# METHODS-Group/ProximalGalerkin

Measured on AMD Instinct MI355X. Metric: proximal-Newton iterations/sec, 2048^2 P1 obstacle (LVPP Newton inner loop), higher is better.
Workload: dtype f64; 1 GPU; 2048x2048 right-diagonal P1 obstacle problem on [-1,1]^2, phi_set obstacle, f=0, settings B: alpha double_exponential, alpha_max 100, tol 0.0001; snes_rtol 1e-6, Newton linear solves to true relative residual 1e-10; mixed_unknowns=8396802, step=one full LVPP solve from the zero state, parallelism=single

## Files before the change

include/pgx.h:

```cpp
#ifndef PGX_H
#define PGX_H

#include <stdint.h>

#ifdef __cplusplus
extern "C" {
#endif

#define PGX_OK 0
#define PGX_EINVAL (-1)
#define PGX_EHIP (-2)
#define PGX_ENODEV (-3)
#define PGX_ENOMEM (-4)
#define PGX_ESTATE (-5)
#define PGX_ECOMM (-6)

#define PGX_SNES_CONVERGED_FNORM_ABS 2
#define PGX_SNES_CONVERGED_FNORM_RELATIVE 3
#define PGX_SNES_CONVERGED_SNORM_RELATIVE 4
#define PGX_SNES_DIVERGED_LINEAR_SOLVE (-3)
#define PGX_SNES_DIVERGED_FNORM_NAN (-4)
#define PGX_SNES_DIVERGED_MAX_IT (-5)
#define PGX_SNES_DIVERGED_DTOL (-9)

typedef struct pgx_handle pgx_handle;

typedef struct {
  int32_t n_vertices;
  int32_t n_cells;
  const double* coords;
  const int32_t* cells;
  int32_t structured_nx;
  int32_t structured_ny;
  const int32_t* cell_dofs;
  int32_t n_dofs;
} pgx_mesh;

typedef struct {
  int32_t degree;
  int32_t nq;
  const double* qpts;
  const double* qwts;
  const double* phi_q;
  double f;
  int32_t n_bc;
  const int32_t* bc_dofs;
  const double* bc_vals;
} pgx_problem;

typedef struct {
  double snes_rtol;
  double snes_atol;
  double snes_stol;
  double snes_divtol;
  int32_t snes_max_it;
  double ksp_rtol;
  int32_t ksp_max_it;
  int32_t ksp_restart;
  int32_t mg_nu;
  double mg_omega;
  int32_t monitor;
  int32_t pc_type;
  int32_t linesearch;
} pgx_snes_opts;

void pgx_default_opts(pgx_snes_opts* o);

int pgx_create(const pgx_mesh* mesh, const pgx_problem* prob, int device, pgx_handle** out);
int pgx_create_curved(const pgx_mesh* mesh, const pgx_problem* prob, const double* geoq, int device, pgx_handle** out);
void pgx_destroy(pgx_handle* h);
const char* pgx_last_error(const pgx_handle* h);

int pgx_num_dofs(const pgx_handle* h, int64_t* ndofs);
int pgx_set_state(pgx_handle* h, const double* x);
int pgx_get_state(pgx_handle* h, double* x);
int pgx_set_prev(pgx_handle* h, const double* xk);
int pgx_get_prev(pgx_handle* h, double* xk);
int pgx_advance_prev(pgx_handle* h);
int pgx_zero_state(pgx_handle* h);
int pgx_set_alpha(pgx_handle* h, double alpha);

int pgx_residual(pgx_handle* h, const double* x, double* F, double* fnorm);
int pgx_jacobian_fill(pgx_handle* h, const double* x);

int pgx_csr_export(pgx_handle* h, int64_t* nrows, int64_t* nnz, int32_t* rowptr, int32_t* col,
                   double* K, double* M, double* D);

int pgx_spmv(pgx_handle* h, const double* x, double* y);
int pgx_spmv_bench(pgx_handle* h, int reps, double* avg_ms, double* algorithmic_bytes);
int pgx_spmv_bench_cold(pgx_handle* h, int reps, double* avg_ms, double* algorithmic_bytes);
int pgx_comm_counts(pgx_handle* h, int64_t out[4], int reset);
int pgx_spmv_select(pgx_handle* h, int kind, int* active);
int pgx_p2_stencil_info(pgx_handle* h, int32_t out[5]);
int pgx_smoother_bench(pgx_handle* h, int reps, double* avg_ms, double* algorithmic_bytes);

int pgx_tuning_set(const char* key, const char* value);
int pgx_vcycle_bench(pgx_handle* h, int level, int reps, double* avg_ms, int* n_level);

int pgx_mg_level_export(pgx_handle* h, int level, int32_t* nx, int32_t* ny, double* Dh4, float* Dq4, uint8_t* mask, int32_t* f32,
                        int32_t* dbf16);
int pgx_vcycle_apply(pgx_handle* h, int level, int nu, double omega, int in_form, int out_form, double scale, const double* b,
                     double* z);

int pgx_newton_solve(pgx_handle* h, const pgx_snes_opts* opts, int* reason, int* its, int* lin_its);
int pgx_observables(pgx_handle* h, double out[6]);

int pgx_profile_enable(pgx_handle* h, int on);
int pgx_profile_get(pgx_handle* h, double ms[8], int reset);

typedef struct pgx_comm pgx_comm;

typedef struct pgx_partition {
  int32_t rank, size;
  int32_t global_ny;
  int32_t dist_levels;
} pgx_partition;

int pgx_partition_rows(pgx_partition* part, int32_t* row0, int32_t* nrows, int32_t* own0, int32_t* nown);

int pgx_comm_rccl_unique_id(char id[128]);
int pgx_comm_rccl_init(const char id[128], int rank, int size, int device, pgx_comm** out);
int pgx_comm_local_group(int size, pgx_comm** out );
int pgx_comm_shm_init(const char* name, int rank, int size, uint64_t slot_bytes, int host_mode, pgx_comm** out);
int pgx_comm_allreduce(pgx_comm* c, double* buf, uint64_t n);
int pgx_comm_halo(pgx_comm* c, double* f0, double* f1, uint64_t send_lo, uint64_t n_send_lo, uint64_t recv_lo, uint64_t n_recv_lo,
                  uint64_t send_hi, uint64_t n_send_hi, uint64_t recv_hi, uint64_t n_recv_hi);
int pgx_comm_gather0(pgx_comm* c, const double* send, uint64_t n, double* recv0);
int pgx_comm_scatter0(pgx_comm* c, const double* send0, uint64_t n, double* recv);
int pgx_comm_selfcheck(pgx_comm* c, int host, double timeout_s);
void pgx_comm_free(pgx_comm* c);
const char* pgx_comm_last_error(void);

int pgx_create_sharded(const pgx_mesh* local_mesh, const pgx_problem* local_prob, const pgx_partition* part,
                       pgx_comm* comm, int device, pgx_handle** out);
int pgx_create_lu_dist(const pgx_mesh* mesh, const pgx_problem* prob, pgx_comm* comm, int device, pgx_handle** out);
int pgx_owned_range(const pgx_handle* h, int64_t* offset, int64_t* count);
int pgx_owned_edge_range(const pgx_handle* h, int64_t* offset, int64_t* count);
int pgx_sync_ghosts(pgx_handle* h);

#ifdef __cplusplus
}
#endif
#endif
```

proximalgalerkin_amd/_lib.py:

```python
from __future__ import annotations

import ctypes as C
import pathlib

import numpy as np

_HERE = pathlib.Path(__file__).resolve().parent
import os as _os

LIB_PATH = pathlib.Path(_os.environ.get("PGX_LIB", _HERE / "libpgx.so"))

c_double_p = C.POINTER(C.c_double)
c_int32_p = C.POINTER(C.c_int32)
c_int64_p = C.POINTER(C.c_int64)


class PgxError(RuntimeError):
    pass


class pgx_mesh(C.Structure):
    _fields_ = [
        ("n_vertices", C.c_int32),
        ("n_cells", C.c_int32),
# ... 264 lines not shown


class pgx_ma_problem(C.Structure):
    _fields_ = [
        ("nv", C.c_int32), ("nc", C.c_int32),
        ("coords", C.POINTER(C.c_double)),
        ("cells", C.POINTER(C.c_int32)),
        ("degree", C.c_int32),
        ("nu", C.c_int32), ("np", C.c_int32),
        ("cell_dofs_u", C.POINTER(C.c_int32)),
        ("cell_dofs_p", C.POINTER(C.c_int32)),
        ("nq", C.c_int32),
        ("qwts", C.POINTER(C.c_double)),
        ("tab_u", C.POINTER(C.c_double)),
        ("dtab_u", C.POINTER(C.c_double)),
        ("tab_p", C.POINTER(C.c_double)),
        ("dtab_p", C.POINTER(C.c_double)),
        ("ln_rho", C.POINTER(C.c_double)),
        ("n_bc", C.c_int32),
        ("bc_dofs", C.POINTER(C.c_int32)),
        ("g", C.POINTER(C.c_double)),
    ]


class pgx_ek_problem(C.Structure):
    _fields_ = [
        ("nc", C.c_int32),
        ("geo_order", C.c_int32),
        ("cell_nodes", c_double_p),
        ("n1", C.c_int32), ("n2", C.c_int32),
        ("cell_dofs_u", c_int32_p),
        ("cell_dofs_p", c_int32_p),
        ("nq", C.c_int32),
        ("qpts", c_double_p),
        ("qwts", c_double_p),
        ("f", C.c_double), ("phi", C.c_double),
    ]


class pgx_partition(C.Structure):
    _fields_ = [
        ("rank", C.c_int32),
        ("size", C.c_int32),
        ("global_ny", C.c_int32),
        ("dist_levels", C.c_int32),
    ]


_H = C.c_void_p
_COMM = C.c_void_p
SYMBOLS = [
    ("pgx_default_opts", None, [C.POINTER(pgx_snes_opts)]),
    ("pgx_create", C.c_int, [C.POINTER(pgx_mesh), C.POINTER(pgx_problem), C.c_int, C.POINTER(_H)]),
    ("pgx_create_curved", C.c_int, [C.POINTER(pgx_mesh), C.POINTER(pgx_problem), c_double_p, C.c_int, C.POINTER(_H)]),
    ("pgx_destroy", None, [_H]),
    ("pgx_last_error", C.c_char_p, [_H]),
    ("pgx_num_dofs", C.c_int, [_H, C.POINTER(C.c_int64)]),
    ("pgx_set_state", C.c_int, [_H, c_double_p]),
    ("pgx_get_state", C.c_int, [_H, c_double_p]),
    ("pgx_set_prev", C.c_int, [_H, c_double_p]),
    ("pgx_get_prev", C.c_int, [_H, c_double_p]),
    ("pgx_advance_prev", C.c_int, [_H]),
    ("pgx_zero_state", C.c_int, [_H]),
    ("pgx_set_alpha", C.c_int, [_H, C.c_double]),
    ("pgx_residual", C.c_int, [_H, c_double_p, c_double_p, c_double_p]),
    ("pgx_jacobian_fill", C.c_int, [_H, c_double_p]),
    ("pgx_csr_export", C.c_int,
     [_H, C.POINTER(C.c_int64), C.POINTER(C.c_int64), c_int32_p, c_int32_p, c_double_p, c_double_p, c_double_p]),
    ("pgx_spmv", C.c_int, [_H, c_double_p, c_double_p]),
    ("pgx_spmv_bench", C.c_int, [_H, C.c_int, c_double_p, c_double_p]),
    ("pgx_spmv_bench_cold", C.c_int, [_H, C.c_int, c_double_p, c_double_p]),
    ("pgx_tuning_set", C.c_int, [C.c_char_p, C.c_char_p]),
    ("pgx_smoother_bench", C.c_int, [_H, C.c_int, c_double_p, c_double_p]),
    ("pgx_vcycle_bench", C.c_int, [_H, C.c_int, C.c_int, c_double_p, C.POINTER(C.c_int)]),
    ("pgx_mg_level_export", C.c_int,
     [_H, C.c_int, c_int32_p, c_int32_p, c_double_p, C.POINTER(C.c_float), C.POINTER(C.c_uint8), c_int32_p, c_int32_p]),
    ("pgx_vcycle_apply", C.c_int, [_H, C.c_int, C.c_int, C.c_double, C.c_int, C.c_int, C.c_double, c_double_p, c_double_p]),
    ("pgx_spmv_select", C.c_int, [_H, C.c_int, C.POINTER(C.c_int)]),
    ("pgx_p2_stencil_info", C.c_int, [_H, C.POINTER(C.c_int32)]),
    ("pgx_comm_counts", C.c_int, [_H, C.POINTER(C.c_int64), C.c_int]),
    ("pgx_newton_solve", C.c_int,
     [_H, C.POINTER(pgx_snes_opts), C.POINTER(C.c_int), C.POINTER(C.c_int), C.POINTER(C.c_int)]),
    ("pgx_observables", C.c_int, [_H, c_double_p]),
    ("pgx_profile_enable", C.c_int, [_H, C.c_int]),
    ("pgx_profile_get", C.c_int, [_H, c_double_p, C.c_int]),
    ("pgx_partition_rows", C.c_int,
     [C.POINTER(pgx_partition), c_int32_p, c_int32_p, c_int32_p, c_int32_p]),
    ("pgx_comm_rccl_unique_id", C.c_int, [C.c_char_p]),
    ("pgx_comm_rccl_init", C.c_int, [C.c_char_p, C.c_int, C.c_int, C.c_int, C.POINTER(_COMM)]),
    ("pgx_comm_local_group", C.c_int, [C.c_int, C.POINTER(_COMM)]),
    ("pgx_comm_shm_init", C.c_int, [C.c_char_p, C.c_int, C.c_int, C.c_uint64, C.c_int, C.POINTER(_COMM)]),
    ("pgx_comm_allreduce", C.c_int, [_COMM, c_double_p, C.c_uint64]),
    ("pgx_comm_halo", C.c_int, [_COMM, c_double_p, c_double_p] + [C.c_uint64] * 8),
    ("pgx_comm_gather0", C.c_int, [_COMM, c_double_p, C.c_uint64, c_double_p]),
    ("pgx_comm_scatter0", C.c_int, [_COMM, c_double_p, C.c_uint64, c_double_p]),
    ("pgx_comm_selfcheck", C.c_int, [_COMM, C.c_int, C.c_double]),
    ("pgx_comm_free", None, [_COMM]),
    ("pgx_comm_last_error", C.c_char_p, []),
    ("pgx_create_sharded", C.c_int,
     [C.POINTER(pgx_mesh), C.POINTER(pgx_problem), C.POINTER(pgx_partition), _COMM, C.c_int, C.POINTER(_H)]),
    ("pgx_create_lu_dist", C.c_int, [C.POINTER(pgx_mesh), C.POINTER(pgx_problem), _COMM, C.c_int, C.POINTER(_H)]),
    ("pgx_owned_range", C.c_int, [_H, C.POINTER(C.c_int64), C.POINTER(C.c_int64)]),
    ("pgx_owned_edge_range", C.c_int, [_H, c_int64_p, c_int64_p]),
    ("pgx_sync_ghosts", C.c_int, [_H]),
    ("pgx_nd_create", C.c_int, [C.POINTER(pgx_nd_matrix), C.c_int, C.c_void_p, C.POINTER(_H)]),
    ("pgx_nd_create_dist", C.c_int, [C.POINTER(pgx_nd_matrix), _COMM, C.c_int, C.c_void_p, C.POINTER(_H)]),
    ("pgx_nd_create_symbolic_dist", C.c_int, [C.POINTER(pgx_nd_matrix), C.c_int, C.c_int, C.POINTER(_H)]),
    ("pgx_nd_export_dist", C.c_int, [_H, c_int32_p, c_int32_p, c_int32_p, c_int32_p]),
    ("pgx_nd_destroy", None, [_H]),
    ("pgx_nd_last_error", C.c_char_p, [_H]),
    ("pgx_nd_get_stats", C.c_int, [_H, C.POINTER(pgx_nd_stats)]),
    ("pgx_nd_factor", C.c_int, [_H, c_double_p, C.c_int]),
    ("pgx_nd_solve", C.c_int, [_H, c_double_p, c_double_p, C.c_int]),
    ("pgx_nd_timing", C.c_int, [_H, C.c_int, c_double_p, c_double_p]),
    ("pgx_nd_depth_profile", C.c_int, [_H, C.c_int, c_int32_p, c_double_p, c_double_p, c_double_p, c_int32_p]),
    ("pgx_nd_set_symmetric", C.c_int, [_H, C.c_int]),
    ("pgx_nd_is_symmetric", C.c_int, [_H]),
    ("pgx_nd_sym_tile_count", C.c_int, [C.c_int, C.c_int, C.c_int]),
    ("pgx_nd_sym_tile_at", None, [C.c_int, C.c_int, C.c_int, C.c_int, C.POINTER(C.c_int), C.POINTER(C.c_int)]),
    ("pgx_nd_export_levels", C.c_int, [_H, c_int64_p, c_int64_p, c_int32_p, c_int32_p, c_int64_p, c_int32_p]),
    ("pgx_nd_export_fronts", C.c_int,
     [_H, c_int64_p, c_int32_p, c_int32_p, c_int32_p, c_int32_p, c_int64_p, c_int32_p, c_int64_p, c_int32_p]),
    ("pgx_nd_export_dest", C.c_int, [_H, c_int64_p, c_int64_p]),
    ("pgx_dn_create", C.c_int, [C.c_int64, c_int32_p, c_int32_p, C.c_int, C.c_void_p, C.POINTER(_H)]),
    ("pgx_dn_destroy", None, [_H]),
    ("pgx_dn_last_error", C.c_char_p, [_H]),
    ("pgx_dn_get_stats", C.c_int, [_H, C.POINTER(pgx_dn_stats)]),
    ("pgx_dn_factor", C.c_int, [_H, c_double_p, C.c_int]),
    ("pgx_dn_solve", C.c_int, [_H, c_double_p, c_double_p, C.c_int]),
    ("pgx_dn_export_pivots", C.c_int, [_H, c_int32_p]),
    ("pgx_dn_timing", C.c_int, [_H, C.c_int, c_double_p, c_double_p]),
    ("pgx_gc_create", C.c_int, [C.POINTER(pgx_mesh), C.POINTER(pgx_gc_problem), C.c_int, C.POINTER(_H)]),
    ("pgx_gc_create_general", C.c_int, [C.POINTER(pgx_gc_spaces), C.POINTER(pgx_gc_problem), C.c_int, C.POINTER(_H)]),
    ("pgx_gc_create_dist", C.c_int, [C.POINTER(pgx_mesh), C.POINTER(pgx_gc_problem), _COMM, C.c_int, C.POINTER(_H)]),
    ("pgx_gc_lu_stats", C.c_int, [_H, C.POINTER(pgx_nd_stats)]),
    ("pgx_gc_lu_is_symmetric", C.c_int, [_H]),
    ("pgx_gc_num_dofs", C.c_int, [_H, c_int64_p]),
    ("pgx_gc_l2_increment", C.c_int, [_H, c_double_p]),
    ("pgx_gc_eval_cells", C.c_int,
     [_H, C.POINTER(pgx_gc_points), c_double_p, c_double_p, c_double_p, C.POINTER(C.c_uint8), C.POINTER(C.c_uint8)]),
    ("pgx_sg_create", C.c_int, [C.POINTER(pgx_sg_mesh), C.POINTER(pgx_sg_problem), C.c_int, C.POINTER(_H)]),
    ("pgx_sg_create_2d", C.c_int, [C.POINTER(pgx_sg_mesh2d), C.POINTER(pgx_sg_problem2d), C.c_int, C.POINTER(_H)]),
    ("pgx_sg_create_dist", C.c_int, [C.POINTER(pgx_sg_mesh), C.POINTER(pgx_sg_problem), _COMM, C.c_int, C.POINTER(_H)]),
    ("pgx_sg_create_curved", C.c_int, [C.POINTER(pgx_sg_mesh), C.POINTER(pgx_sg_problem), C.POINTER(pgx_sg_curved), C.c_int, C.POINTER(_H)]),
    ("pgx_sg_partition_info", C.c_int, [_H, c_int64_p, c_int64_p]),
    ("pgx_sg_lu_stats", C.c_int, [_H, C.POINTER(pgx_nd_stats)]),
    ("pgx_sg_lu_is_symmetric", C.c_int, [_H]),
    ("pgx_sg_num_dofs", C.c_int, [_H, c_int64_p, c_int64_p]),
    ("pgx_sg_contact_vertices", C.c_int, [_H, c_int32_p]),
    ("pgx_sg_u_increment", C.c_int, [_H, c_double_p]),
    ("pgx_sg_penetration", C.c_int, [_H, c_double_p]),
    ("pgx_sg_violation", C.c_int, [_H, c_double_p]),
    ("pgx_sg_von_mises", C.c_int, [_H, c_double_p]),
    ("pgx_qvi_create", C.c_int, [C.POINTER(pgx_mesh), C.POINTER(pgx_qvi_problem), C.c_int, C.POINTER(_H)]),
    ("pgx_qvi_num_dofs", C.c_int, [_H, c_int64_p]),
    ("pgx_qvi_h1_increment", C.c_int, [_H, c_double_p]),
    ("pgx_qmy_create", C.c_int, [C.POINTER(pgx_mesh), C.POINTER(pgx_qmy_problem), C.c_int, C.POINTER(_H)]),
    ("pgx_qmy_destroy", None, [_H]),
    ("pgx_qmy_last_error", C.c_char_p, [_H]),
    ("pgx_qmy_num_dofs", C.c_int, [_H, c_int64_p]),
    ("pgx_qmy_set_state", C.c_int, [_H, c_double_p]),
    ("pgx_qmy_get_state", C.c_int, [_H, c_double_p]),
    ("pgx_qmy_set_prev", C.c_int, [_H, c_double_p]),
    ("pgx_qmy_get_prev", C.c_int, [_H, c_double_p]),
    ("pgx_qmy_advance_prev", C.c_int, [_H]),
    ("pgx_qmy_set_gamma", C.c_int, [_H, C.c_double]),
# ... 157 lines not shown
```

proximalgalerkin_amd/csrc/pgx_api.hip:

```cpp
#include <algorithm>
#include <atomic>
#include <chrono>
#include <thread>
#include <cmath>
#include <cstdio>
#include <cstring>
#include <deque>
#include <map>
#include <mutex>
#include <string>
#include <vector>

#include "../../include/pgx.h"
#include "../../include/pgx_nd.h"
#include "pgx_comm.h"
#include "pgx_internal.h"

static thread_local std::string g_create_error;

struct DistLevel {
  int g, glo, H, ghi;
};
struct Dist {
  bool on = false;
// ... 14 lines not shown
struct pgx_handle {
  int device = 0;
  Dist dist;
  hipStream_t st = nullptr;
  std::string err;
  int n = 0, nc = 0, nx = 0, ny = 0, nnz = 0;
  int degree = 1;
  int nd = 0;
  bool structured = false;
  QuadTab q{};
  double f = 0.0, alpha = 1.0;
  double* coords = nullptr;
  int32_t* cells = nullptr;
  uint8_t* mask = nullptr;
  double *gbc = nullptr, *bphi = nullptr;
  int32_t *rowptr = nullptr, *colm = nullptr, *v2c_ptr = nullptr, *v2c_ent = nullptr, *v2c_pos = nullptr;
  std::vector<int32_t> h_rowptr, h_col;
  size_t fill_lds = 0;
  double *Kv = nullptr, *Mv = nullptr, *Dv = nullptr;
  bool jac_valid = false;
  double* geoq = nullptr;
  float2* zf_out = nullptr;
  int z_f32 = 1;
  int f32_dbf16 = 1;
  bool dv_lean = false;
  int32_t *s_rowptr = nullptr, *s_colm = nullptr;
  double *s_K = nullptr, *s_M = nullptr, *s_D = nullptr;
  int s_nnz = 0;
  size_t s_fill_lds = 0;
  int32_t* s_blk = nullptr;
  int s_nblk = 0, spmv_bal = 1;
  uint8_t* s_code = nullptr;
  double* s_tab = nullptr;
  int s_ntab = 0, spmv_dict = 1;
  std::vector<int32_t> s_h_rowptr, s_h_col;
  QuadTab2 q2{};
  int32_t *cdofs = nullptr, *p2_v2c_ptr = nullptr, *p2_v2c_ent = nullptr, *p2_v2c_pos = nullptr;
  int32_t *v2e_ptr = nullptr, *v2e = nullptr, *edge_ends = nullptr;
  double *p2_xu = nullptr, *p2_xp = nullptr, *p2_ru = nullptr, *p2_rp = nullptr;
  double* p2_stash = nullptr;
  double *c1_bu = nullptr, *c1_bp = nullptr, *c1_xu = nullptr, *c1_xp = nullptr;
  int patch_nn = 0, p2_patch = 1, patch_nu = 2;
  int p2_fallback_its = 60, p2_fallbacks = 0;
  double patch_omega = 0.8;
  bool patch_fresh = false;
  std::vector<int32_t> patch_dof_host;
  int32_t *pdof = nullptr, *ppos = nullptr;
  void* pinv = nullptr;
  int patch_f32 = 1;
  struct P2St {
    int state = 0, enable = 1, dist_enable = 1, select = 1, i0 = 0, ni = 0, j0 = 0, nj = 0, nframe = 0, ref_rows[4] = {0, 0, 0, 0};
    P2StTab tab;
    double K[46];
    double* Dst = nullptr;
    float* Dstf = nullptr;
    int32_t* frame = nullptr;
    bool fresh = false;
  } p2st;
  float* s_Df = nullptr;
  int p2_resid_f32 = 1;
  int patch_sym = 1;
  double *p2_su = nullptr, *p2_sp = nullptr;
  double *x = nullptr, *xk = nullptr, *F = nullptr, *dx = nullptr, *xw = nullptr, *rhs = nullptr;
  int restart = 0;
  double *V = nullptr, *Z = nullptr, *w = nullptr, *d_small = nullptr, *partials = nullptr, *partials2 = nullptr;
  double* h_small = nullptr;
  double* h_small_dev = nullptr;
  unsigned long long* h_seq = nullptr;
  unsigned long long* h_seq_dev = nullptr;
  unsigned long long seq = 0;
  int lean_d = 1;
  int spmv_d4 = 1;
  int lazy_norm = 1;
  double rhs_scale = 1.0;
  const float* rhs_f32 = nullptr;
  int v_f32 = 1;
  double v_f32_gain = 1e-4;
  double v_f32_max = 1e30;
  int v_f32_min = 1000000;
  bool v_f32_off = false;
  int host_poll = 1;
  int gs_wide = 16;
  int fused_publish = 1;
  int fused_resid = 1;
  int lean_rhs = 1;
  int fused_step = 1;
  std::vector<GridLevel> lev;
  double *tmp_u = nullptr, *tmp_p = nullptr, *res_u = nullptr, *res_p = nullptr;
  double omega_now = 0.0;
  int coarse_sweeps = 4;
  int tail_start = -1;
  int xcd_remap = 2;
  int tail_verts = 1100;
  int spmv_stream = 1;
  int nu_coarse = 0;
  int fused_k3 = 1;
  int fused_legs = 1;
  int fused_min = 4000;
  int cgs_selective = 1;
  long cgs_skipped = 0, cgs_total = 0;
  double cgs_eta2 = 1e-4;
  TailArgs tail{};
  pgx_nd* lu = nullptr;
  pgx_comm* lu_comm = nullptr;
  double* Jmix = nullptr;
  bool dh_interior = false;
  int d_direct = 1;
  int rap_lds_min = 60000;
  bool d0_direct = false;
  int stag_its = 12;
  double stag_gain = 1e-4;
  int smooth_d32 = 0;
  int k6_max = 0;
  int mg_f32 = 1;
  int f32_min = 4000;
  int f32_k6_max = 4300000;
  int f32_rr_max = 300000;
  int resid_grid = 1;
  int spmv_stencil = 1;
  bool lu_active = false;
  bool check_replicas = false;
  double *obs_partials = nullptr, *d_out6 = nullptr;
  int obs_blocks = 0;
  bool prof = false;
  double ms[8] = {0, 0, 0, 0, 0, 0, 0, 0};
  hipEvent_t e0 = nullptr, e1 = nullptr;
  std::vector<void*> allocs;
};

#define HIPCHK(call)                                                                            \
  do {                                                                                          \
    hipError_t e_ = (call);                                                                     \
    if (e_ != hipSuccess) {                                                                     \
      h->err = std::string(#call) + ": " + hipGetErrorString(e_);                               \
      return PGX_EHIP;                                                                          \
    }                                                                                           \
  } while (0)

template <typename T>
static int dalloc(pgx_handle* h, T** p, size_t count) {
  void* q = nullptr;
  hipError_t e = hipMalloc(&q, std::max<size_t>(count, 1) * sizeof(T));
  if (e != hipSuccess) {
    h->err = std::string("hipMalloc: ") + hipGetErrorString(e);
    return PGX_ENOMEM;
  }
  h->allocs.push_back(q);
  *p = (T*)q;
  return PGX_OK;
}
#define DALLOC(p, count)                         \
  do {                                           \
    int rc_ = dalloc(h, &(p), (size_t)(count));  \
    if (rc_) return rc_;                         \
  } while (0)

struct PhaseTimer {
  pgx_handle* h;
  int slot;
  PhaseTimer(pgx_handle* h_, int s) : h(h_), slot(s) {
    static const char* const names[8] = {"pgx:residual", "pgx:jacobian", "pgx:mg_setup/lu_factor", "pgx:spmv", "pgx:precond",
                                         "pgx:orthogonalise", "pgx:observables", "pgx:newton_solve"};
    pgx_roctx(names[s & 7]);
    if (h->prof) hipEventRecord(h->e0, h->st);
  }
  ~PhaseTimer() {
// ... 875 lines not shown
    HIPCHK(hipMemcpy(G.mask, gm.data(), G.n, hipMemcpyHostToDevice));
  }
  rc = detect_uniform(h, G);
  if (rc) return rc;
  D.view.interior_free = G.interior_free;
  h->lev.push_back(G);
  int nx = G.nx, ny = G.ny;
  const int min_nx = mg_min_nx();
  while (nx % 2 == 0 && ny % 2 == 0 && nx > min_nx && ny > min_nx) {
    nx /= 2;
    ny /= 2;
    GridLevel L{};
    L.nx = nx;
    L.ny = ny;
    L.n = (nx + 1) * (ny + 1);
    rc = alloc_level(h, L, false);
    if (rc) return rc;
    const GridLevel& Ff = h->lev.back();
    pgxk_coarse_mask(h->st, L, L.mask, Ff);
    pgxk_rap7(h->st, Ff, Ff.K, L, L.K);
    pgxk_rap7(h->st, Ff, Ff.M, L, L.M);
    rc = detect_uniform(h, L);
    if (rc) return rc;
    h->lev.push_back(L);
  }
  setup_tail(h, ld);
  rc = setup_f32(h);
  if (rc) return rc;
  HIPCHK(hipStreamSynchronize(h->st));
  return PGX_OK;
}

static thread_local const double* g_create_geoq = nullptr;

static int create_impl(const pgx_mesh* m, const pgx_problem* p, int device, const pgx_partition* part, pgx_comm* comm,
                       pgx_handle** out) {
  if (!m || !p || !out) {
    g_create_error = "null argument";
    return PGX_EINVAL;
  }
  *out = nullptr;
  int ndev = 0;
  if (hipGetDeviceCount(&ndev) != hipSuccess || ndev <= 0) {
    g_create_error = "no HIP device visible: libpgx has no CPU fallback";
    return PGX_ENODEV;
  }
  if (device < 0 || device >= ndev) {
    g_create_error = "device index out of range";
    return PGX_EINVAL;
  }
  pgx_handle* h = new pgx_handle();
  if (const char* e = pgx_tune("PGX_XCD_REMAP")) h->xcd_remap = atoi(e) ? 2 : 0;
  if (const char* e = pgx_tune("PGX_TAIL_VERTS")) h->tail_verts = atoi(e);
  if (const char* e = pgx_tune("PGX_P2_PATCH")) h->p2_patch = atoi(e);
  if (const char* e = pgx_tune("PGX_P2_PATCH_NU")) h->patch_nu = std::max(1, atoi(e));
  if (const char* e = pgx_tune("PGX_P2_PATCH_OMEGA")) h->patch_omega = atof(e);
  if (const char* e = pgx_tune("PGX_P2_PATCH_F32")) h->patch_f32 = atoi(e);
  if (const char* e = pgx_tune("PGX_P2_PATCH_SYM")) h->patch_sym = atoi(e);
  if (const char* e = pgx_tune("PGX_P2_RESID_F32")) h->p2_resid_f32 = atoi(e);
  if (const char* e = pgx_tune("PGX_P2_STENCIL")) h->p2st.enable = atoi(e);
  if (const char* e = pgx_tune("PGX_P2_STENCIL_DIST")) h->p2st.dist_enable = atoi(e);
  if (!h->patch_f32) h->patch_sym = 0;
  if (h->patch_f32 == 2 && !h->patch_sym) h->patch_f32 = 1;
  if (const char* e = pgx_tune("PGX_P2_FALLBACK_ITS")) h->p2_fallback_its = std::max(1, atoi(e));
  {
    const char* e = pgx_tune("PGX_TAIL2");
    pgxk_mg_tail_select(e ? atoi(e) : 1);
  }
  if (const char* e = pgx_tune("PGX_FUSED_LEGS")) h->fused_legs = atoi(e);
  if (const char* e = pgx_tune("PGX_FUSED_K3")) h->fused_k3 = atoi(e);
  if (const char* e = pgx_tune("PGX_NU_COARSE")) h->nu_coarse = atoi(e);
  if (const char* e = pgx_tune("PGX_SPMV_STREAM")) h->spmv_stream = atoi(e);
  if (const char* e = pgx_tune("PGX_SPMV_BAL")) h->spmv_bal = atoi(e);
  if (const char* e = pgx_tune("PGX_SPMV_DICT")) h->spmv_dict = atoi(e);
  if (const char* e = pgx_tune("PGX_SPMV_STENCIL")) h->spmv_stencil = atoi(e);
  if (const char* e = pgx_tune("PGX_RESID_GRID")) h->resid_grid = atoi(e);
  if (const char* e = pgx_tune("PGX_D_DIRECT")) h->d_direct = atoi(e);
  if (const char* e = pgx_tune("PGX_RAP_LDS_MIN")) h->rap_lds_min = atoi(e);
  if (const char* e = pgx_tune("PGX_K6_MAX")) h->k6_max = atoi(e);
  if (const char* e = pgx_tune("PGX_SMOOTH_D32")) h->smooth_d32 = atoi(e);
  if (const char* e = pgx_tune("PGX_HOST_POLL")) h->host_poll = atoi(e);
  if (const char* e = pgx_tune("PGX_GS_WIDE")) h->gs_wide = atoi(e) >= 16 ? 16 : 8;
  if (const char* e = pgx_tune("PGX_FUSED_PUBLISH")) h->fused_publish = atoi(e);
  if (const char* e = pgx_tune("PGX_FUSED_RESID")) h->fused_resid = atoi(e);
  if (const char* e = pgx_tune("PGX_LEAN_RHS")) h->lean_rhs = atoi(e);
  if (const char* e = pgx_tune("PGX_FUSED_STEP")) h->fused_step = atoi(e);
  if (const char* e = pgx_tune("PGX_LAZY_NORM")) h->lazy_norm = atoi(e);
  if (const char* e = pgx_tune("PGX_V_F32")) h->v_f32 = atoi(e);
  if (const char* e = pgx_tune("PGX_V_F32_GAIN")) h->v_f32_gain = atof(e);
  if (const char* e = pgx_tune("PGX_V_F32_MAX")) h->v_f32_max = atof(e);
  if (const char* e = pgx_tune("PGX_V_F32_MIN")) h->v_f32_min = atoi(e);
  if (const char* e = pgx_tune("PGX_Z_F32")) h->z_f32 = atoi(e);
  if (const char* e = pgx_tune("PGX_F32_DBF16")) h->f32_dbf16 = atoi(e);
  if (const char* e = pgx_tune("PGX_SPMV_D4")) h->spmv_d4 = atoi(e);
  if (const char* e = pgx_tune("PGX_LEAN_D")) h->lean_d = atoi(e);
  if (const char* e = pgx_tune("PGX_MG_F32")) h->mg_f32 = atoi(e);
  if (const char* e = pgx_tune("PGX_F32_MIN")) h->f32_min = atoi(e);
  if (const char* e = pgx_tune("PGX_F32_RR_MAX")) h->f32_rr_max = atoi(e);
  if (const char* e = pgx_tune("PGX_F32_K6_MAX")) h->f32_k6_max = atoi(e);
  if (const char* e = pgx_tune("PGX_STAG_ITS")) h->stag_its = std::max(2, atoi(e));
  if (const char* e = pgx_tune("PGX_STAG_GAIN")) h->stag_gain = atof(e);
  if (const char* e = pgx_tune("PGX_FUSED_MIN")) h->fused_min = atoi(e);
  if (const char* e = pgx_tune("PGX_CGS_SELECTIVE")) h->cgs_selective = atoi(e);
  if (const char* e = pgx_tune("PGX_CGS_ETA2")) h->cgs_eta2 = atof(e);
  if (const char* e = pgx_tune("PGX_COARSE_SWEEPS")) h->coarse_sweeps = atoi(e);
  auto fail = [&](int rc) {
    g_create_error = h->err;
    pgx_destroy(h);
    return rc;
  };
  h->device = device;
  if (p->degree != 1 && p->degree != 2) {
    h->err = "only Lagrange degree 1 and 2 are implemented";
    return fail(PGX_EINVAL);
  }
  h->degree = p->degree;
  if (p->degree == 2 && (!m->cell_dofs || m->n_dofs <= m->n_vertices)) {
    h->err = "degree 2 needs pgx_mesh.cell_dofs [n_cells][6] and n_dofs = n_vertices + n_edges";
    return fail(PGX_EINVAL);
  }
  if (p->nq < 1 || p->nq > PGX_MAX_NQ || !p->qpts || !p->qwts || !p->phi_q || m->n_vertices < 3 || m->n_cells < 1 ||
      !m->coords || !m->cells || (p->n_bc > 0 && !p->bc_dofs)) {
    h->err = "invalid mesh/problem description";
    return fail(PGX_EINVAL);
  }
  if (hipSetDevice(device) != hipSuccess || hipStreamCreate(&h->st) != hipSuccess) {
    h->err = "hipSetDevice/hipStreamCreate failed";
    return fail(PGX_EHIP);
  }
  hipEventCreate(&h->e0);
  hipEventCreate(&h->e1);
  const int n = h->n = m->n_vertices, nc = h->nc = m->n_cells;
  const int nd = h->nd = (p->degree == 2) ? m->n_dofs : n;
  h->f = p->f;
  if (m->structured_nx > 0 && m->structured_ny > 0) {
    if ((int64_t)(m->structured_nx + 1) * (m->structured_ny + 1) != n ||
        (int64_t)2 * m->structured_nx * m->structured_ny != nc) {
      h->err = "structured_nx/ny inconsistent with n_vertices/n_cells";
      return fail(PGX_EINVAL);
    }
    h->structured = true;
    h->nx = m->structured_nx;
    h->ny = m->structured_ny;
  }
  if (part) {
    pgx_partition pt = *part;
    int32_t row0 = 0, nrows = 0, own0 = 0, nown = 0;
    if (pgx_partition_rows(&pt, &row0, &nrows, &own0, &nown)) {
      h->err = g_create_error;
      return fail(PGX_EINVAL);
    }
    if (!comm || comm->rank != pt.rank || comm->size != pt.size) {
      h->err = "pgx_create_sharded: communicator rank/size differ from the partition's";
      return fail(PGX_EINVAL);
    }
    if (!h->structured || (p->degree != 1 && p->degree != 2)) {
      h->err = "pgx_create_sharded: structured P1 / P2 meshes are sharded (strip decomposition)";
      return fail(PGX_EINVAL);
    }
    if (h->ny + 1 != nrows || h->nx % (1 << pt.dist_levels)) {
      h->err = "pgx_create_sharded: local mesh must hold exactly the vertex rows of pgx_partition_rows, and nx must be "
               "divisible by 2^dist_levels";
      return fail(PGX_EINVAL);
    }
    for (int c = 0; c < nc; ++c) {
      const int v0 = std::min(m->cells[3 * c], std::min(m->cells[3 * c + 1], m->cells[3 * c + 2]));
// ... 107 lines not shown
    }
    double* phi_q = nullptr;
    const size_t nphi = (size_t)nc * p->nq;
    if (hipMalloc((void**)&phi_q, nphi * sizeof(double)) != hipSuccess) {
      h->err = "hipMalloc(phi_q)";
      return PGX_ENOMEM;
    }
    hipError_t e = hipMemcpy(phi_q, p->phi_q, nphi * sizeof(double), hipMemcpyHostToDevice);
    double* stash = nullptr;
    if (e == hipSuccess) e = hipMalloc((void**)&stash, sizeof(double) * 8 * (size_t)nc);
    if (e == hipSuccess) {
      if (p->degree == 2)
        pgxk_bphi_p2(h->st, nc, nd, h->cdofs, h->coords, phi_q, h->q2, h->p2_v2c_ptr, h->p2_v2c_ent, stash, h->bphi, h->geoq);
      else
        pgxk_bphi(h->st, nc, n, h->cells, h->coords, phi_q, h->q, h->v2c_ptr, h->v2c_ent, stash, h->bphi, h->geoq);
      e = hipStreamSynchronize(h->st);
    }
    hipFree(phi_q);
    if (stash) hipFree(stash);
    if (e != hipSuccess) {
      h->err = std::string("b_phi assembly: ") + hipGetErrorString(e);
      return PGX_EHIP;
    }
    DALLOC(h->Kv, h->nnz);
    DALLOC(h->Mv, h->nnz);
    DALLOC(h->Dv, h->nnz);
    const double* geo1 = p->degree == 1 ? h->geoq : nullptr;
    pgxk_fill_rows(h->st, 0, n, h->fill_lds, h->rowptr, h->v2c_ptr, h->v2c_ent, h->v2c_pos, h->cells, h->coords,
                   nullptr, h->q, h->Kv, geo1);
    pgxk_fill_rows(h->st, 1, n, h->fill_lds, h->rowptr, h->v2c_ptr, h->v2c_ent, h->v2c_pos, h->cells, h->coords,
                   nullptr, h->q, h->Mv, geo1);
    if (p->degree == 2) {
      DALLOC(h->s_K, h->s_nnz);
      DALLOC(h->s_M, h->s_nnz);
      DALLOC(h->s_D, h->s_nnz);
      pgxk_fill_rows_p2(h->st, 0, nd, h->s_fill_lds, h->s_rowptr, h->p2_v2c_ptr, h->p2_v2c_ent, h->p2_v2c_pos, h->cdofs,
                        h->coords, nullptr, h->q2, h->s_K, h->geoq);
      pgxk_fill_rows_p2(h->st, 1, nd, h->s_fill_lds, h->s_rowptr, h->p2_v2c_ptr, h->p2_v2c_ent, h->p2_v2c_pos, h->cdofs,
                        h->coords, nullptr, h->q2, h->s_M, h->geoq);
      if (h->spmv_dict && h->spmv_bal && h->s_blk) {
        const int rc = build_km_dictionary(h);
        if (rc) return rc;
      }
      DALLOC(h->p2_stash, (size_t)16 * nc);
      DALLOC(h->p2_xu, nd);
      DALLOC(h->p2_xp, nd);
      DALLOC(h->p2_ru, nd);
      DALLOC(h->p2_rp, nd);
      DALLOC(h->c1_bu, n);
      DALLOC(h->c1_bp, n);
      DALLOC(h->c1_xu, n);
      DALLOC(h->c1_xp, n);
    } else {
      h->s_rowptr = h->rowptr;
      h->s_colm = h->colm;
      h->s_K = h->Kv;
      h->s_M = h->Mv;
      h->s_D = h->Dv;
      h->s_nnz = h->nnz;
      h->s_fill_lds = h->fill_lds;
    }
    const size_t n2 = 2 * (size_t)nd;
    DALLOC(h->x, n2);
    DALLOC(h->xk, n2);
    DALLOC(h->F, n2);
    DALLOC(h->dx, n2);
    DALLOC(h->xw, n2);
    DALLOC(h->rhs, n2);
    HIPCHK(hipMemsetAsync(h->x, 0, n2 * sizeof(double), h->st));
    HIPCHK(hipMemsetAsync(h->xk, 0, n2 * sizeof(double), h->st));
    h->restart = 50;
    if (p->degree == 2) {
      double budget = 24e9;
      if (const char* e = pgx_tune("PGX_P2_BASIS_GB")) budget = 1e9 * atof(e);
      const double per_vec = 2.0 * (double)n2 * sizeof(double);
      h->restart = (int)std::max(50.0, std::min(300.0, budget / per_vec));
    }
    DALLOC(h->V, (size_t)(h->restart + 1) * n2);
    DALLOC(h->Z, (size_t)h->restart * n2);
    DALLOC(h->w, n2);
    DALLOC(h->d_small, 4 * (h->restart + 2));
    DALLOC(h->partials, (size_t)PGX_RED_BLOCKS * (h->restart + 2));
    DALLOC(h->partials2, ((n2 + PGX_BLOCK - 1) / PGX_BLOCK) * (size_t)62);
    {
      const size_t nsm = 4 * (size_t)(h->restart + 2);
      HIPCHK(hipHostMalloc((void**)&h->h_small, sizeof(double) * (nsm + 2), hipHostMallocMapped | hipHostMallocCoherent));
      memset(h->h_small, 0, sizeof(double) * (nsm + 2));
      HIPCHK(hipHostGetDevicePointer((void**)&h->h_small_dev, h->h_small, 0));
      h->h_seq = reinterpret_cast<unsigned long long*>(h->h_small + nsm);
      h->h_seq_dev = reinterpret_cast<unsigned long long*>(h->h_small_dev + nsm);
    }
    DALLOC(h->tmp_u, n);
    DALLOC(h->tmp_p, n);
    DALLOC(h->res_u, n);
    DALLOC(h->res_p, n);
    h->obs_blocks = pgxk_observables_blocks(nc);
    DALLOC(h->obs_partials, (size_t)h->obs_blocks * 6);
    DALLOC(h->d_out6, 6);
    if (h->dist.on) {
      DALLOC(h->dist.sb, n2);
      DALLOC(h->dist.wc, 2 * h->dist.nk_field() + 2);
    }
    const int r = h->dist.on ? build_multigrid_dist(h) : build_multigrid(h);
    if (r) return r;
    HIPCHK(hipStreamSynchronize(h->st));
    return PGX_OK;
  };
  rc = up();
  if (rc) return fail(rc);
  *out = h;
  return PGX_OK;
}

extern "C" int pgx_create(const pgx_mesh* m, const pgx_problem* p, int device, pgx_handle** out) {
  return create_impl(m, p, device, nullptr, nullptr, out);
}
extern "C" int pgx_create_curved(const pgx_mesh* m, const pgx_problem* p, const double* geoq, int device, pgx_handle** out) {
  if (!geoq) {
    g_create_error = "pgx_create_curved: null geometry table";
    return PGX_EINVAL;
  }
  g_create_geoq = geoq;
  const int rc = create_impl(m, p, device, nullptr, nullptr, out);
  g_create_geoq = nullptr;
  return rc;
}
extern "C" int pgx_create_lu_dist(const pgx_mesh* m, const pgx_problem* p, pgx_comm* comm, int device, pgx_handle** out) {
  if (!comm) {
    g_create_error = "pgx_create_lu_dist: null communicator";
    return PGX_EINVAL;
  }
  int rc = create_impl(m, p, device, nullptr, nullptr, out);
  if (rc) return rc;
  (*out)->lu_comm = comm;
  if (const char* e = pgx_tune("PGX_CHECK_REPLICAS")) (*out)->check_replicas = atoi(e) != 0;
  return PGX_OK;
}
extern "C" int pgx_create_sharded(const pgx_mesh* m, const pgx_problem* p, const pgx_partition* part, pgx_comm* comm,
                                  int device, pgx_handle** out) {
  if (!part || !comm) {
    g_create_error = "pgx_create_sharded: null partition / communicator";
    return PGX_EINVAL;
  }
  return create_impl(m, p, device, part, comm, out);
}

extern "C" void pgx_destroy(pgx_handle* h) {
  if (!h) return;
  hipSetDevice(h->device);
  if (h->st) hipStreamSynchronize(h->st);
  if (h->cgs_selective && pgx_tune("PGX_CGS_REPORT"))
    fprintf(stderr, "pgx: selective CGS2 skipped the second projection in %ld of %ld Krylov iterations\n", h->cgs_skipped, h->cgs_total);
  if (h->lu) pgx_nd_destroy(h->lu);
  for (void* p : h->allocs) hipFree(p);
  if (h->h_small) hipHostFree(h->h_small);
  if (h->e0) hipEventDestroy(h->e0);
  if (h->e1) hipEventDestroy(h->e1);
  if (h->st) hipStreamDestroy(h->st);
  delete h;
}

#define NEED(hh)          \
  if (!(hh)) return PGX_EINVAL; \
  hipSetDevice((hh)->device)

extern "C" int pgx_num_dofs(const pgx_handle* h, int64_t* nd) {
// ... 26 lines not shown
  if (!x) return PGX_EINVAL;
  return copy_in(h, h->xk, x);
}
extern "C" int pgx_get_prev(pgx_handle* h, double* x) {
  NEED(h);
  if (!x) return PGX_EINVAL;
  return copy_out(h, x, h->xk);
}
extern "C" int pgx_advance_prev(pgx_handle* h) {
  NEED(h);
  pgxk_scale_copy(h->st, 2 * (size_t)h->nd, 1.0, h->x, h->xk);
  HIPCHK(hipStreamSynchronize(h->st));
  return PGX_OK;
}
extern "C" int pgx_zero_state(pgx_handle* h) {
  NEED(h);
  HIPCHK(hipMemsetAsync(h->x, 0, sizeof(double) * 2 * (size_t)h->nd, h->st));
  HIPCHK(hipMemsetAsync(h->xk, 0, sizeof(double) * 2 * (size_t)h->nd, h->st));
  HIPCHK(hipStreamSynchronize(h->st));
  return PGX_OK;
}
extern "C" int pgx_owned_range(const pgx_handle* h, int64_t* offset, int64_t* count) {
  if (!h) return PGX_EINVAL;
  if (offset) *offset = h->dist.on ? (int64_t)h->dist.own_off : 0;
  if (count) *count = h->dist.on ? (int64_t)h->dist.own_cnt : (int64_t)(h->degree == 2 ? h->n : h->nd);
  return PGX_OK;
}
extern "C" int pgx_owned_edge_range(const pgx_handle* h, int64_t* offset, int64_t* count) {
  if (!h) return PGX_EINVAL;
  if (offset) *offset = (int64_t)h->n + (h->dist.on ? (int64_t)h->dist.eown_off : 0);
  if (count) *count = h->dist.on ? (int64_t)h->dist.eown_cnt : (int64_t)(h->nd - h->n);
  return PGX_OK;
}
extern "C" int pgx_sync_ghosts(pgx_handle* h) {
  NEED(h);
  if (!h->dist.on) return PGX_OK;
  int rc = halo_solution(h, h->x, h->x + h->nd);
  if (!rc) rc = halo_solution(h, h->xk, h->xk + h->nd);
  if (rc) return rc;
  HIPCHK(hipStreamSynchronize(h->st));
  return PGX_OK;
}
extern "C" int pgx_set_alpha(pgx_handle* h, double a) {
  if (!h || !(a > 0.0)) return PGX_EINVAL;
  h->alpha = a;
  return PGX_OK;
}

static int replica_agree(pgx_handle* h, double* dev, size_t n) {
  if (!h->lu_comm || h->lu_comm->size == 1) return PGX_OK;
  if (h->lu_comm->rank != 0) HIPCHK(hipMemsetAsync(dev, 0, n * sizeof(double), h->st));
  const int rc = h->lu_comm->allreduce(h->st, dev, n);
  if (rc) h->err = "replica agreement: " + h->lu_comm->err;
  return rc;
}

__global__ void __launch_bounds__(64) k_publish(int n, const double* __restrict__ src, double* dst, int n2, const double* __restrict__ src2,
                                                double* dst2, unsigned long long seq, unsigned long long* seqp) {
  for (int i = threadIdx.x; i < n; i += 64) __hip_atomic_store(dst + i, src[i], __ATOMIC_RELAXED, __HIP_MEMORY_SCOPE_SYSTEM);
  for (int i = threadIdx.x; i < n2; i += 64) __hip_atomic_store(dst2 + i, src2[i], __ATOMIC_RELAXED, __HIP_MEMORY_SCOPE_SYSTEM);
  __threadfence_system();
  if (threadIdx.x == 0) __hip_atomic_store(seqp, seq, __ATOMIC_RELEASE, __HIP_MEMORY_SCOPE_SYSTEM);
}
static int wait_published(pgx_handle* h, unsigned long long seq);
static int fetch_small(pgx_handle* h, const double* dsrc, size_t n, size_t hoff = 0, const double* dsrc2 = nullptr, size_t n2 = 0,
                       size_t hoff2 = 0) {
  if (!h->host_poll) {
    HIPCHK(hipMemcpyAsync(h->h_small + hoff, dsrc, sizeof(double) * n, hipMemcpyDeviceToHost, h->st));
    if (n2) HIPCHK(hipMemcpyAsync(h->h_small + hoff2, dsrc2, sizeof(double) * n2, hipMemcpyDeviceToHost, h->st));
    HIPCHK(hipStreamSynchronize(h->st));
    return PGX_OK;
  }
  const unsigned long long seq = ++h->seq;
  hipLaunchKernelGGL(k_publish, dim3(1), dim3(64), 0, h->st, (int)n, dsrc, h->h_small_dev + hoff, (int)n2, dsrc2, h->h_small_dev + hoff2,
                     seq, h->h_seq_dev);
  return wait_published(h, seq);
}
static bool fused_readback(const pgx_handle* h) { return h->fused_publish && h->host_poll && !h->dist.on && !h->lu_comm; }
static int reduce_fetch(pgx_handle* h, int nb, const double* partials, int nrows, double* dout, size_t hoff_r, const double* dsrc1 = nullptr,
                        size_t n1 = 0, size_t hoff1 = 0) {
  const unsigned long long seq = ++h->seq;
  pgxk_reduce_publish(h->st, nb, partials, nrows, dout, h->h_small_dev + hoff_r, (int)n1, dsrc1, h->h_small_dev + hoff1, seq, h->h_seq_dev);
  return wait_published(h, seq);
}
static int wait_published(pgx_handle* h, unsigned long long seq) {
  static const double limit_s = [] {
    const char* t = getenv("PGX_COMM_TIMEOUT");
    return t ? std::max(1.0, atof(t)) : 120.0;
  }();
  std::chrono::steady_clock::time_point t0;
  bool timed = false;
  for (unsigned long spins = 1;; ++spins) {
    if (__atomic_load_n(h->h_seq, __ATOMIC_ACQUIRE) == seq) return PGX_OK;
    __builtin_ia32_pause();
    if (spins > 0x2000 && (spins & 0xff) == 0) std::this_thread::yield();
    if ((spins & 0x3fff) == 0) {
      if (!timed) {
        t0 = std::chrono::steady_clock::now();
        timed = true;
      } else if (std::chrono::duration<double>(std::chrono::steady_clock::now() - t0).count() > limit_s) {
        h->err = "fetch_small: the device did not publish within PGX_COMM_TIMEOUT (" + std::to_string((int)limit_s) +
                 " s): a kernel or a collective ahead of it on the stream does not complete" + (h->dist.on || h->lu_comm ? " (a peer rank is missing?)" : "");
        return (h->dist.on || h->lu_comm) ? PGX_ECOMM : PGX_EHIP;
      }
      const hipError_t e = hipStreamQuery(h->st);
      if (e == hipSuccess) {
        if (__atomic_load_n(h->h_seq, __ATOMIC_ACQUIRE) == seq) return PGX_OK;
        h->err = "fetch_small: the stream drained without publishing (launch failure)";
        return PGX_EHIP;
      }
      if (e != hipErrorNotReady) {
        h->err = std::string("fetch_small: ") + hipGetErrorString(e);
        return PGX_EHIP;
      }
    }
  }
}

static int dev_norm(pgx_handle* h, const double* v, double* out, size_t len = 0) {
  if (fused_readback(h)) {
    const size_t l = len ? len : 2 * (size_t)h->nd;
    pgxk_multidot(h->st, l, 1, v, 0, v, h->partials, nullptr);
    const int rc = reduce_fetch(h, pgxk_multidot_blocks(l), h->partials, 1, h->d_small, 0);
    if (rc) return rc;
    *out = std::sqrt(h->h_small[0]);
    return PGX_OK;
  }
  pgxk_multidot(h->st, len ? len : 2 * (size_t)h->nd, 1, v, 0, v, h->partials, h->d_small);
  if (h->dist.on) {
    const int rc = allreduce_dev(h, h->d_small, 1);
    if (rc) return rc;
  }
  {
    const int rc = replica_agree(h, h->d_small, 1);
    if (rc) return rc;
  }
  {
    const int rc = fetch_small(h, h->d_small, 1);
    if (rc) return rc;
  }
  *out = std::sqrt(h->h_small[0]);
  return PGX_OK;
}

static bool d_direct_on(const pgx_handle* h) {
  return h->d_direct && !h->dist.on && h->degree == 1 && h->structured && h->resid_grid && !h->lev.empty() && h->lev[0].uniform &&
         sizeof(dsten_t) == 8 && !h->lev[0].Dh32;
}

static void residual_dev(pgx_handle* h, const double* x, double* F, int with_d = 0) {
  PhaseTimer t(h, 0);
  if (h->degree == 2) {
    pgxk_residual_p2_cells(h->st, h->nc, h->nd, h->cdofs, h->coords, h->mask, h->gbc, x, h->xk, h->alpha, h->f, h->q2,
                           h->p2_v2c_ptr, h->p2_v2c_ent, h->p2_stash, F, h->geoq);
    pgxk_residual_final(h->st, h->nd, h->mask, h->gbc, h->bphi, x, F);
    return;
  }
  if (h->resid_grid && h->structured && !h->lev.empty() && h->lev[0].uniform) {
    pgxk_resid_fill_grid(h->st, with_d ? 1 : 0, h->lev[0], h->fill_lds, h->rowptr, h->v2c_ptr, h->v2c_ent, h->v2c_pos, h->cells,
                         h->coords, h->mask, h->gbc, h->bphi, x, h->xk, h->alpha, h->f, h->q, F, h->Dv, with_d, d_direct_on(h), h->colm);
    h->dh_interior = with_d != 0;
    h->d0_direct = with_d != 0 && d_direct_on(h);
    if (with_d == 2) h->dv_lean = true;
    if (with_d == 1) h->dv_lean = false;
    return;
  }
  pgxk_resid_fill_p1(h->st, with_d, h->n, h->fill_lds, h->rowptr, h->v2c_ptr, h->v2c_ent, h->v2c_pos, h->cells,
                     h->coords, h->mask, h->gbc, h->bphi, x, h->xk, h->alpha, h->f, h->q, F, h->Dv, h->geoq);
}

static int jacobian_dev(pgx_handle* h, const double* x, bool have_d = false) {
  if (!(have_d && h->degree == 1)) {
    PhaseTimer t(h, 1);
    if (h->degree == 2) {
      pgxk_fill_rows_p2(h->st, 2, h->nd, h->s_fill_lds, h->s_rowptr, h->p2_v2c_ptr, h->p2_v2c_ent, h->p2_v2c_pos,
                        h->cdofs, h->coords, x + h->nd, h->q2, h->s_D, h->geoq);
      pgxk_fill_rows_p1_Dp2(h->st, h->n, h->fill_lds, h->rowptr, h->v2c_ptr, h->v2c_ent, h->v2c_pos, h->cdofs, h->coords,
                            x + h->nd, h->q2, h->Dv, h->geoq);
    } else if (h->resid_grid && h->structured && !h->lev.empty() && h->lev[0].uniform) {
      pgxk_resid_fill_grid(h->st, 1, h->lev[0], h->fill_lds, h->rowptr, h->v2c_ptr, h->v2c_ent, h->v2c_pos, h->cells, h->coords,
                           h->mask, h->gbc, h->bphi, x, h->xk, h->alpha, h->f, h->q, h->w, h->Dv, 1, d_direct_on(h), h->colm);
      h->dh_interior = true;
      h->d0_direct = d_direct_on(h);
      h->dv_lean = false;
      have_d = true;
    } else {
      pgxk_fill_rows(h->st, 2, h->n, h->fill_lds, h->rowptr, h->v2c_ptr, h->v2c_ent, h->v2c_pos, h->cells, h->coords,
                     x + h->n, h->q, h->Dv, h->geoq);
    }
  }
  if (h->structured) {
    PhaseTimer t(h, 2);
    const bool direct = d_direct_on(h);
    const bool d0 = direct && have_d && h->dh_interior && h->d0_direct;
    if (!d0)
      pgxk_csr_to_stencil_h(h->st, h->n, h->nx + 1, h->rowptr, h->colm, h->Dv, h->lev[0].Dh,
                            (have_d && h->degree == 1 && h->dh_interior) ? h->lev[0].ny : 0);
    h->dh_interior = false;
    h->d0_direct = false;
    if (h->lev[0].Dh32) pgxk_to_float(h->st, (size_t)4 * h->n, h->lev[0].Dh, h->lev[0].Dh32);
    if (h->lev[0].f32 && !d0) pgxk_f_pack_d(h->st, h->lev[0]);
    if (h->lev[0].Dd4 && !d0) pgxk_pack_d4(h->st, h->lev[0]);
    const int ld = h->dist.on ? h->dist.ldist : 0;
    for (size_t l = 1; l < h->lev.size(); ++l) {
      if (h->dist.on && (int)l == ld) {
        const Dist& D = h->dist;
// ... 764 lines not shown
  const bool vf32_ok = h->v_f32 && lean && lazy && zf32 && h->nd >= h->v_f32_min;
  float* const Vf = reinterpret_cast<float*>(h->V);
  const size_t ldvf = (nk + 3) & ~(size_t)3;
  while (true) {
    double beta;
    const bool vf32 = vf32_ok && !h->v_f32_off;
    if (first_cycle && its >= o->ksp_max_it) break;
    if (first_cycle) {
      beta = bnorm;
      if (vf32)
        pgxk_scale_copy_f32(h->st, nk, bsign * (1.0 / beta), b, Vf);
      else
        pgxk_scale_copy(h->st, nk, bsign * (1.0 / beta), b, h->V);
    } else {
      PhaseTimer t(h, 3);
      if (lean && h->fused_resid) {
        pgxk_st_spmv(h->st, h->lev[0], h->alpha, x, x + h->nd, h->xcd_remap ? 1 : 0, h->w, h->w + h->nd, nullptr, b, b + h->nd, bsign);
      } else {
        spmv_dev(h, x, h->w);
        if (dist) gather_owned(h, h->w, wk);
        pgxk_scale_copy(h->st, nk, -1.0, wk, wk);
        pgxk_axpy(h->st, nk, bsign, b, wk);
      }
      rc = dev_norm(h, wk, &beta, nk);
      if (rc) return rc;
      res = beta;
      if (o->monitor > 1) printf("      ksp true residual after cycle: %.6e (rel %.3e)\n", beta, beta / bnorm);
      if (!redo && beta <= target) break;
      if (!redo && beta > 0.1 * prev_cycle_res && beta <= 1e-7 * bnorm) break;
      if (its >= o->ksp_max_it) break;
      prev_cycle_res = beta;
      if (vf32)
        pgxk_scale_copy_f32(h->st, nk, 1.0 / beta, wk, Vf);
      else
        pgxk_scale_copy(h->st, nk, 1.0 / beta, wk, h->V);
    }
    const bool was_first = first_cycle;
    first_cycle = false;
    redo = false;
    bool abandoned = false;
    double hn_bad = 0.0;
    const double cycle_target = vf32 ? std::max(target, h->v_f32_gain * beta) : target;
    std::fill(g.begin(), g.end(), 0.0);
    g[0] = beta;
    float2* const Zf = reinterpret_cast<float2*>(h->Z);
    PgxDotScale sc2;
    std::vector<double> sv((size_t)m + 2, 1.0);
    for (int i = 0; i < PGX_DOT_SCALE_MAX; ++i) sc2.s[i] = 1.0;
    int j = 0;
    for (; j < m && its < o->ksp_max_it; ++j) {
      double* vj = h->V + (size_t)j * nk;
      double* zj = h->Z + (size_t)j * n2;
      {
        PhaseTimer t(h, 4);
        h->rhs_scale = lazy ? sv[j] : 1.0;
        h->zf_out = zf32 ? Zf + (size_t)j * h->nd : nullptr;
        h->rhs_f32 = vf32 ? Vf + (size_t)j * ldvf : nullptr;
        rc = precond(h, vj, zj, o->mg_nu, omega);
        h->rhs_f32 = nullptr;
        h->zf_out = nullptr;
        h->rhs_scale = 1.0;
        if (rc) return rc;
      }
      {
        PhaseTimer t(h, 3);
        if (dist) {
          spmv_dev(h, zj, h->w);
          gather_owned(h, h->w, h->V + (size_t)(j + 1) * nk);
        } else if (zf32) {
          double* const wn = vf32 ? h->w : h->V + (size_t)(j + 1) * n2;
          pgxk_st_spmv(h->st, h->lev[0], h->alpha, nullptr, nullptr, h->xcd_remap ? 1 : 0, wn, wn + h->nd, Zf + (size_t)j * h->nd);
        } else {
          spmv_dev(h, zj, h->V + (size_t)(j + 1) * n2);
        }
      }
      double* wj = h->V + (size_t)(j + 1) * nk;
      float* const vnext = Vf + (size_t)(j + 1) * ldvf;
      double hn = 0.0;
      {
        PhaseTimer t(h, 5);
        double* d_h1 = h->d_small;
        double* d_h2 = h->d_small + (m + 2);
        const PgxDotScale* const dsc = lazy ? &sc2 : nullptr;
        if (vf32)
          pgxk_multidot_f32(h->st, nk, j + 1, Vf, ldvf, h->w, nullptr, h->partials, d_h1, dsc, h->gs_wide);
        else
          pgxk_multidot(h->st, nk, j + 1, h->V, nk, wj, h->partials, d_h1, dsc, h->gs_wide);
        if (dist && (rc = allreduce_dev(h, d_h1, j + 1))) return rc;
        double wp2, h1h1 = 0.0, hh = 0.0;
        bool second;
        if (h->cgs_selective) {
          if (fused_readback(h)) {
            if (vf32)
              pgxk_multiaxpy_norm_f32(h->st, nk, j + 1, Vf, ldvf, d_h1, 0, h->w, vnext, h->partials, nullptr, h->gs_wide);
            else
              pgxk_multiaxpy_norm(h->st, nk, j + 1, h->V, nk, d_h1, wj, h->partials, nullptr, h->gs_wide);
            if ((rc = reduce_fetch(h, pgxk_stream_blocks(nk), h->partials, 1, d_h2 + j + 1, (size_t)(m + 2) + j + 1, d_h1, (size_t)(j + 1), 0)))
              return rc;
          } else {
            if (vf32)
              pgxk_multiaxpy_norm_f32(h->st, nk, j + 1, Vf, ldvf, d_h1, 0, h->w, vnext, h->partials, d_h2 + j + 1, h->gs_wide);
            else
              pgxk_multiaxpy_norm(h->st, nk, j + 1, h->V, nk, d_h1, wj, h->partials, d_h2 + j + 1, h->gs_wide);
            if (dist && (rc = allreduce_dev(h, d_h2 + j + 1, 1))) return rc;
            if ((rc = replica_agree(h, h->d_small, 2 * (size_t)(m + 2)))) return rc;
            if ((rc = fetch_small(h, d_h1, (size_t)(j + 1), 0, d_h2 + j + 1, 1, (size_t)(m + 2) + j + 1))) return rc;
          }
          for (int i = 0; i <= j; ++i) {
            h->h_small[i] /= sv[i];
            h1h1 += h->h_small[i] * h->h_small[i];
          }
          wp2 = h->h_small[(m + 2) + j + 1];
          second = wp2 < h->cgs_eta2 * (wp2 + h1h1);
          if (second) {
            if (vf32)
              pgxk_multidot_f32(h->st, nk, j + 1, Vf, ldvf, nullptr, vnext, h->partials, d_h2, dsc, h->gs_wide);
            else
              pgxk_multidot(h->st, nk, j + 1, h->V, nk, wj, h->partials, d_h2, dsc, h->gs_wide);
            if (dist && (rc = allreduce_dev(h, d_h2, j + 1))) return rc;
            if ((rc = replica_agree(h, d_h2, (size_t)(j + 1)))) return rc;
            if ((rc = fetch_small(h, d_h2, (size_t)(j + 1), (size_t)(m + 2)))) return rc;
            for (int i = 0; i <= j; ++i) h->h_small[(m + 2) + i] /= sv[i];
          }
        } else {
          if (j + 1 <= 60) {
            pgxk_axpy_dot(h->st, nk, j + 1, h->V, nk, d_h1, wj, h->partials2, d_h2);
          } else {
            pgxk_multiaxpy(h->st, nk, j + 1, h->V, nk, d_h1, wj);
            pgxk_multidot(h->st, nk, j + 2, h->V, nk, wj, h->partials, d_h2);
          }
          if (dist && (rc = allreduce_dev(h, d_h2, j + 2))) return rc;
          if ((rc = replica_agree(h, h->d_small, 2 * (size_t)(m + 2)))) return rc;
          if ((rc = fetch_small(h, h->d_small, 2 * (size_t)(m + 2)))) return rc;
          wp2 = h->h_small[(m + 2) + j + 1];
          second = true;
        }
        for (int i = 0; i <= j; ++i) {
          const double h2 = second ? h->h_small[(m + 2) + i] : 0.0;
          H[(size_t)i * m + j] = h->h_small[i] + h2;
          hh += h2 * h2;
        }
        if (second && vf32) {
          double* const d_n2 = d_h2 + j + 1;
          if (fused_readback(h)) {
            pgxk_multiaxpy_norm_f32(h->st, nk, j + 1, Vf, ldvf, d_h2, 1, h->w, vnext, h->partials, nullptr, h->gs_wide);
            if ((rc = reduce_fetch(h, pgxk_stream_blocks(nk), h->partials, 1, d_n2, (size_t)(m + 2) + j + 1))) return rc;
          } else {
            pgxk_multiaxpy_norm_f32(h->st, nk, j + 1, Vf, ldvf, d_h2, 1, h->w, vnext, h->partials, d_n2, h->gs_wide);
            if ((rc = fetch_small(h, d_n2, 1, (size_t)(m + 2) + j + 1))) return rc;
          }
          hn = std::sqrt(std::max(h->h_small[(m + 2) + j + 1], 0.0));
        } else if (second) {
          hn = std::sqrt(std::max(wp2 - hh, 0.0));
          if (hn > 0.0) {
            if (lazy)
              pgxk_multiaxpy(h->st, nk, j + 1, h->V, nk, d_h2, wj);
            else
              pgxk_multiaxpy_scale(h->st, nk, j + 1, h->V, nk, d_h2, 1.0 / hn, wj);
          }
        } else {
          hn = std::sqrt(std::max(wp2, 0.0));
          if (hn > 0.0 && !lazy) pgxk_scale_copy(h->st, nk, 1.0 / hn, wj, wj);
          ++h->cgs_skipped;
        }
        if (vf32 && (!std::isfinite(hn) || hn > h->v_f32_max)) {
          ++its;
          ++h->cgs_total;
          hn_bad = hn;
          abandoned = true;
          break;
        }
        if (lazy && hn > 0.0) {
          sv[j + 1] = 1.0 / hn;
          sc2.s[j + 1] = sv[j + 1] * sv[j + 1];
        }
        ++h->cgs_total;
      }
      H[(size_t)(j + 1) * m + j] = hn;
      for (int i = 0; i < j; ++i) {
        const double t1 = cs[i] * H[(size_t)i * m + j] + sn[i] * H[(size_t)(i + 1) * m + j];
        H[(size_t)(i + 1) * m + j] = -sn[i] * H[(size_t)i * m + j] + cs[i] * H[(size_t)(i + 1) * m + j];
        H[(size_t)i * m + j] = t1;
      }
      const double a = H[(size_t)j * m + j], bb = H[(size_t)(j + 1) * m + j];
      const double rr = std::hypot(a, bb);
      cs[j] = rr == 0.0 ? 1.0 : a / rr;
      sn[j] = rr == 0.0 ? 0.0 : bb / rr;
      H[(size_t)j * m + j] = rr;
      H[(size_t)(j + 1) * m + j] = 0.0;
      g[j + 1] = -sn[j] * g[j];
      g[j] = cs[j] * g[j];
      res = std::fabs(g[j + 1]);
      ++its;
      if (dist) ++h->dist.n_krylov;
      if (o->monitor > 1) printf("      ksp %3d  rnorm %.6e  rel %.3e\n", its, res, res / bnorm);
      if (!std::isfinite(res)) {
        if (x_unset) pgxk_set(h->st, n2, 0.0, x);
        *its_out = its;
        *relres = res / bnorm;
        return PGX_OK;
      }
      if (res <= cycle_target || hn == 0.0) {
        ++j;
        break;
      }
      if (omega > omega_safe && j + 1 == std::min(m, h->stag_its) && res > h->stag_gain * beta) {
        h->omega_now = omega = omega_safe;
        if (o->monitor > 1) printf("      ksp stagnates: smoother damping -> %.2f for the rest of this Newton solve\n", omega);
      }
    }
    if (abandoned) {
      h->v_f32_off = true;
      if (o->monitor > 1) printf("      ksp: basis vector outside the float range (norm %.3e): this cycle again, with the fp64 basis\n", hn_bad);
      res = beta;
      first_cycle = was_first;
      redo = !was_first;
      continue;
    }
    for (int i = j - 1; i >= 0; --i) {
      double s = g[i];
      for (int k = i + 1; k < j; ++k) s -= H[(size_t)i * m + k] * y[k];
      y[i] = s / H[(size_t)i * m + i];
    }
    for (int i = 0; i < j; ++i) h->h_small[i] = y[i];
    HIPCHK(hipMemcpyAsync(h->d_small, h->h_small, sizeof(double) * j, hipMemcpyHostToDevice, h->st));
    if (zf32)
      pgxk_lincomb_f2(h->st, (size_t)h->nd, j, Zf, (size_t)h->nd, h->d_small, x, x + h->nd, x_unset ? 0 : 1);
    else
      pgxk_lincomb(h->st, n2, j, h->Z, n2, h->d_small, x, x_unset ? 0 : 1);
    x_unset = false;
  }
  if (x_unset) pgxk_set(h->st, n2, 0.0, x);
  *its_out = its;
  *relres = res / bnorm;
  return PGX_OK;
}

extern "C" int pgx_residual(pgx_handle* h, const double* x, double* F, double* fnorm) {
  NEED(h);
  const double* xd = h->x;
  if (x) {
    int rc = copy_in(h, h->xw, x);
    if (rc) return rc;
    xd = h->xw;
  }
  residual_dev(h, xd, h->F);
  if (fnorm) {
    int rc;
    if (h->dist.on) {
      gather_owned(h, h->F, h->dist.wc);
      rc = dev_norm(h, h->dist.wc, fnorm, 2 * h->dist.nk_field());
    } else {
      rc = dev_norm(h, h->F, fnorm);
    }
    if (rc) return rc;
  }
  if (F) return copy_out(h, F, h->F);
  HIPCHK(hipStreamSynchronize(h->st));
  return PGX_OK;
}

extern "C" int pgx_jacobian_fill(pgx_handle* h, const double* x) {
  NEED(h);
  const double* xd = h->x;
  if (x) {
    int rc = copy_in(h, h->xw, x);
    if (rc) return rc;
    xd = h->xw;
  }
  {
    const int rc = jacobian_dev(h, xd);
    if (rc) return rc;
  }
  HIPCHK(hipStreamSynchronize(h->st));
  HIPCHK(hipGetLastError());
  return PGX_OK;
}

extern "C" int pgx_csr_export(pgx_handle* h, int64_t* nrows, int64_t* nnz, int32_t* rowptr, int32_t* col, double* K,
                              double* M, double* D) {
  NEED(h);
  const std::vector<int32_t>& hr = (h->degree == 2) ? h->s_h_rowptr : h->h_rowptr;
  const std::vector<int32_t>& hc = (h->degree == 2) ? h->s_h_col : h->h_col;
  if (nrows) *nrows = h->nd;
  if (nnz) *nnz = h->s_nnz;
  if (rowptr) memcpy(rowptr, hr.data(), sizeof(int32_t) * (h->nd + 1));
  if (col) memcpy(col, hc.data(), sizeof(int32_t) * h->s_nnz);
  if (K) HIPCHK(hipMemcpy(K, h->s_K, sizeof(double) * h->s_nnz, hipMemcpyDeviceToHost));
  if (M) HIPCHK(hipMemcpy(M, h->s_M, sizeof(double) * h->s_nnz, hipMemcpyDeviceToHost));
  if (D) {
    if (!h->jac_valid) {
      h->err = "pgx_csr_export(D) before pgx_jacobian_fill";
      return PGX_ESTATE;
    }
    HIPCHK(hipMemcpy(D, h->s_D, sizeof(double) * h->s_nnz, hipMemcpyDeviceToHost));
  }
  return PGX_OK;
}

extern "C" int pgx_spmv(pgx_handle* h, const double* x, double* y) {
  NEED(h);
  if (!x || !y) return PGX_EINVAL;
  if (!h->jac_valid) {
    h->err = "pgx_spmv before pgx_jacobian_fill";
    return PGX_ESTATE;
  }
  int rc = copy_in(h, h->V, x);
  if (rc) return rc;
  if (h->dist.on && (rc = halo_solution(h, h->V, h->V + h->nd))) return rc;
  spmv_dev(h, h->V, h->w);
  return copy_out(h, y, h->w);
}

extern "C" int pgx_smoother_bench(pgx_handle* h, int reps, double* avg_ms, double* bytes) {
  NEED(h);
  if (reps < 1 || !avg_ms) return PGX_EINVAL;
  if (!h->jac_valid || !h->structured || h->lev.size() < 2 || h->dist.on) {
    h->err = "pgx_smoother_bench needs a structured single-GPU handle with a grid hierarchy and a filled Jacobian";
    return PGX_ESTATE;
  }
  if (h->degree == 2) {
    if (!h->patch_nn || !h->p2_patch) {
      h->err = "pgx_smoother_bench (P2): no patch smoother on this handle";
      return PGX_ESTATE;
    }
    const int rcp = ensure_patches(h);
    if (rcp) return rcp;
    const int nd = h->nd, nv = h->n, NN = h->patch_nn, P = 2 * NN;
    pgxk_set(h->st, 2 * (size_t)nd, 1.0, h->rhs);
    HIPCHK(hipMemsetAsync(h->w, 0, sizeof(double) * 2 * nd, h->st));
    auto sweep = [&]() {
      pgxk_patch_sweep(h->st, nv, NN, nv, nd, h->pdof, h->edge_ends, h->pinv, h->patch_f32, h->patch_sym, h->rhs, h->rhs + nd, h->patch_omega,
                       h->w, h->w + nd, h->p2_su, h->p2_sp);
    };
    for (int k = 0; k < 3; ++k) sweep();
    HIPCHK(hipEventRecord(h->e0, h->st));
    for (int k = 0; k < reps; ++k) sweep();
    HIPCHK(hipEventRecord(h->e1, h->st));
    HIPCHK(hipEventSynchronize(h->e1));
    float msp = 0;
    HIPCHK(hipEventElapsedTime(&msp, h->e0, h->e1));
// ... 415 lines not shown
  const size_t n2 = 2 * (size_t)h->nd;
  PgxSolveScope scope(h->st, h->prof, &h->lu_active);
  struct JacStale {
    pgx_handle* h;
    ~JacStale() {
      if (h->dh_interior || h->dv_lean) h->jac_valid = false;
    }
  } jac_stale{h};
  PgxRange range("pgx:newton_solve");
  int its = 0, lin = 0, rsn = 0;
  double fnorm = 0, fnorm0 = 0, ttol = 0;
  h->omega_now = 0.0;
  h->v_f32_off = false;
  int rc = PGX_OK;
  const bool dist = h->dist.on;
  const size_t nk = dist ? 2 * h->dist.nk_field() : n2;
  auto owned_norm = [&](const double* v, double* out) -> int {
    if (!dist) return dev_norm(h, v, out);
    gather_owned(h, v, h->dist.wc);
    return dev_norm(h, h->dist.wc, out, nk);
  };
  const int with_d = (!use_lu && !mg_first && h->degree == 1 && h->structured && h->spmv_stencil == 1 && h->lean_d) ? 2 : 1;
  pgxk_scale_copy(h->st, n2, 1.0, h->x, h->xw);
  residual_dev(h, h->xw, h->F, with_d);
  if ((rc = replica_check(h, h->F, n2, "the residual"))) return rc;
  if (dist) {
    gather_owned(h, h->F, h->rhs);
    rc = dev_norm(h, h->rhs, &fnorm, nk);
  } else {
    rc = dev_norm(h, h->F, &fnorm);
  }
  if (rc) return rc;
  fnorm0 = fnorm;
  if (opts->monitor) printf("  0 SNES Function norm %.12e\n", fnorm);
  if (!std::isfinite(fnorm))
    rsn = PGX_SNES_DIVERGED_FNORM_NAN;
  else if (fnorm < opts->snes_atol)
    rsn = PGX_SNES_CONVERGED_FNORM_ABS;
  ttol = fnorm * opts->snes_rtol;
  while (rsn == 0) {
    if (its >= opts->snes_max_it) {
      rsn = PGX_SNES_DIVERGED_MAX_IT;
      break;
    }
    rc = jacobian_dev(h, h->xw, true);
    if (rc) return rc;
    if (use_lu) {
      if ((rc = lu_factor(h))) return rc;
      h->lu_active = true;
    }
    const bool lean_rhs = h->lean_rhs && !use_lu && !mg_first && krylov_lean(h);
    if (!lean_rhs) pgxk_scale_copy(h->st, nk, -1.0, dist ? h->rhs : h->F, h->rhs);
    int kits = 0;
    double relres = 0;
    if (mg_first && !use_lu) {
      pgx_snes_opts ol = optv;
      ol.ksp_max_it = std::min(optv.ksp_max_it, h->p2_fallback_its);
      rc = fgmres(h, h->rhs, h->dx, &ol, &kits, &relres, fnorm);
      if (rc) return rc;
      if (kits >= ol.ksp_max_it && !(relres <= 10.0 * optv.ksp_rtol)) {
        if (opts->monitor) printf("    KSP (patch multigrid) %d its, rel residual %.3e: sparse LU for the rest of this solve\n", kits, relres);
        lin += kits;
        if ((rc = ensure_lu(h))) return rc;
        if ((rc = lu_factor(h))) return rc;
        h->lu_active = true;
        use_lu = true;
        ++h->p2_fallbacks;
        rc = fgmres(h, h->rhs, h->dx, opts, &kits, &relres, fnorm);
        if (rc) return rc;
      }
    } else {
      rc = lean_rhs ? fgmres(h, h->F, h->dx, opts, &kits, &relres, fnorm, -1.0) : fgmres(h, h->rhs, h->dx, opts, &kits, &relres, fnorm);
      if (rc) return rc;
    }
    lin += kits;
    ++its;
    if (opts->monitor) printf("    KSP its %d  rel residual %.3e\n", kits, relres);
    if (!(relres <= std::max(opts->ksp_rtol, 1e-7)) || !std::isfinite(relres)) {
      rsn = PGX_SNES_DIVERGED_LINEAR_SOLVE;
      break;
    }
    const bool fstep = h->fused_step && fused_readback(h) && !use_lu && !mg_first && krylov_lean(h);
    int step_nb = 0;
    if (fstep)
      step_nb = pgxk_axpy_norms(h->st, n2, h->dx, h->xw, h->partials2);
    else
      pgxk_axpy(h->st, n2, 1.0, h->dx, h->xw);
    if (dist && (rc = halo_solution(h, h->xw, h->xw + h->nd))) return rc;
    residual_dev(h, h->xw, h->F, with_d);
    if ((rc = replica_check(h, h->F, n2, "the residual"))) return rc;
    if (dist) {
      gather_owned(h, h->F, h->rhs);
      rc = dev_norm(h, h->rhs, &fnorm, nk);
    } else {
      rc = dev_norm(h, h->F, &fnorm);
    }
    if (rc) return rc;
    if (opts->monitor) printf("  %d SNES Function norm %.12e\n", its, fnorm);
    if (!std::isfinite(fnorm)) {
      rsn = PGX_SNES_DIVERGED_FNORM_NAN;
    } else if (fnorm < opts->snes_atol) {
      rsn = PGX_SNES_CONVERGED_FNORM_ABS;
    } else if (fnorm <= ttol) {
      rsn = PGX_SNES_CONVERGED_FNORM_RELATIVE;
    } else {
      double snorm, xnorm;
      if (fstep) {
        if ((rc = reduce_fetch(h, step_nb, h->partials2, 2, h->d_small, 0))) return rc;
        snorm = std::sqrt(h->h_small[0]);
        xnorm = std::sqrt(h->h_small[1]);
      } else {
        rc = owned_norm(h->dx, &snorm);
        if (rc) return rc;
        rc = owned_norm(h->xw, &xnorm);
        if (rc) return rc;
      }
      if (snorm < opts->snes_stol * xnorm)
        rsn = PGX_SNES_CONVERGED_SNORM_RELATIVE;
      else if (fnorm > opts->snes_divtol * fnorm0)
        rsn = PGX_SNES_DIVERGED_DTOL;
    }
  }
  h->lu_active = false;
  if (rsn > 0) pgxk_scale_copy(h->st, n2, 1.0, h->xw, h->x);
  if (h->dh_interior || h->dv_lean) h->jac_valid = false;
  HIPCHK(hipStreamSynchronize(h->st));
  HIPCHK(hipGetLastError());
  if (h->prof) h->ms[7] += scope.stop();
  *reason = rsn;
  if (its_out) *its_out = its;
  if (lin_out) *lin_out = lin;
  return PGX_OK;
}
```

proximalgalerkin_amd/csrc/pgx_internal.h:

```cpp
#pragma once
#include <hip/hip_runtime.h>
#include <stdint.h>
#include <stddef.h>

#include "pgx_scope.h"

#ifdef PGX_DSTEN_FLOAT
typedef float dsten_t;
#else
typedef double dsten_t;
#endif

#define PGX_MAX_NQ 16
#define PGX_BLOCK 256
#ifndef PGX_TILE_X
#define PGX_TILE_X 32
#define PGX_TILE_Y 16
#endif
#ifndef PGX_ROWMAP_TY
#define PGX_ROWMAP_TY 16
#endif
#ifndef PGX_ROWMAP_BLOCK
#define PGX_ROWMAP_BLOCK 512
#endif
// ... 4 lines not shown
  double Mref[3][3];
  double mref[3];
  int nq;
};

struct GridLevel {
  int nx, ny, n;
  double *K, *M;
  dsten_t* Dh;
  float* Dh32;
  int uniform;
  int interior_free;
  double Kc[7], Mc[7];
  uint8_t* mask;
  double *xu, *xp, *xu2, *xp2;
  double *bu, *bp;
  double *ru, *rp;
  int f32;
  double4* Dd4;
  void* Dq;
  int dbf16;
  float2 *xf, *xf2, *bf;
};

struct StConst {
  double K[7], M[7];
  int uniform;
};

typedef float f_v2f __attribute__((ext_vector_type(2)));
typedef __bf16 f_v2bf __attribute__((ext_vector_type(2)));
__device__ __forceinline__ uint32_t f_pack_bf16x2(float lo, float hi) {
  const f_v2f f = {lo, hi};
  return __builtin_bit_cast(uint32_t, __builtin_convertvector(f, f_v2bf));
}
__device__ __forceinline__ void f_pack_d(float4 q, float4& out) { out = q; }
__device__ __forceinline__ void f_pack_d(float4 q, uint2& out) { out = make_uint2(f_pack_bf16x2(q.x, q.y), f_pack_bf16x2(q.z, q.w)); }
template <class DT>
__device__ __forceinline__ void f_pack_dq(dsten_t d0, dsten_t d1, dsten_t d2, dsten_t d3, DT& out) {
  const float big = 1e30f;
  f_pack_d(make_float4(fminf((float)d0, big), fminf((float)d1, big), fminf((float)d2, big), fminf((float)d3, big)), out);
}

#define PGX_TAIL_MAX 8
#define PGX_TAIL_VERTS 17000
struct TailLevel {
  int nx, ny, n;
  int interior_free;
  double ic[8];
  const double *K, *M;
  const dsten_t* Dh;
  StConst sc;
  const uint8_t* mask;
  double *xu, *xp, *xu2, *xp2, *bu, *bp, *ru, *rp;
};
struct TailArgs {
  int nlev, nu, coarse_sweeps;
  double alpha, omega;
  TailLevel L[PGX_TAIL_MAX];
};
void pgxk_mg_tail(hipStream_t st, const TailArgs& A);
void pgxk_mg_tail_select(int v);

void pgxk_bphi(hipStream_t st, int nc, int n, const int32_t* cells, const double* coords, const double* phi_q,
               QuadTab q, const int32_t* v2c_ptr, const int32_t* v2c_ent, double* stash, double* bphi,
               const double* geo = nullptr );
void pgxk_gather_ent(hipStream_t st, int n, const int32_t* ptr, const int32_t* ent, const double* stash, double* out);
void pgxk_fill_rows(hipStream_t st, int mode, int n, size_t lds_bytes, const int32_t* rowptr, const int32_t* v2c_ptr,
                    const int32_t* v2c_ent, const int32_t* v2c_pos, const int32_t* cells, const double* coords,
                    const double* psi, QuadTab q, double* out, const double* geo = nullptr);
void pgxk_bspmv(hipStream_t st, int mode, int n, const int32_t* rowptr, const int32_t* colm, const double* K,
                const double* M, const double* D, double alpha, const double* xu, const double* xp, const double* bu,
                const double* bp, double omega, int first, double* yu, double* yp);
void pgxk_observables(hipStream_t st, int nc, int n, const int32_t* cells, const double* coords, const double* x,
                      const double* xk, double alpha, double f, QuadTab q, double* partials, int nblocks, double* out6,
                      int raw = 0, const double* geo = nullptr);
int pgxk_observables_blocks(int nc);

void pgxk_axpy(hipStream_t st, size_t len, double a, const double* x, double* y);
void pgxk_scale_copy(hipStream_t st, size_t len, double a, const double* x, double* y);
void pgxk_scale_copy_f32(hipStream_t st, size_t len, double a, const double* x, float* y);
void pgxk_set(hipStream_t st, size_t len, double a, double* y);
void pgxk_to_float(hipStream_t st, size_t len, const double* x, float* y);
#define PGX_RED_BLOCKS 1024
#define PGX_DOT_SCALE_MAX 64
struct PgxDotScale {
  double s[PGX_DOT_SCALE_MAX];
};
void pgxk_multidot(hipStream_t st, size_t len, int nv, const double* V, size_t ldv, const double* w, double* partials,
                   double* out, const PgxDotScale* scale = nullptr, int wide = 8);
void pgxk_multidot_f32(hipStream_t st, size_t len, int nv, const float* V, size_t ldv, const double* w, const float* wf, double* partials,
                       double* out, const PgxDotScale* scale = nullptr, int wide = 8);
int pgxk_multidot_blocks(size_t len);
int pgxk_stream_blocks(size_t len);
void pgxk_reduce_publish(hipStream_t st, int nb, const double* partials, int nrows, double* out, double* hout, int n1, const double* src1,
                         double* dst1, unsigned long long seq, unsigned long long* seqp);
int pgxk_axpy_norms(hipStream_t st, size_t len, const double* x, double* y, double* partials);
void pgxk_multiaxpy(hipStream_t st, size_t len, int nv, const double* V, size_t ldv, const double* h, double* w);
void pgxk_lincomb(hipStream_t st, size_t len, int nv, const double* Z, size_t ldz, const double* y, double* x,
                  int accumulate);

void pgxk_csr_to_stencil(hipStream_t st, int n, int sx, const int32_t* rowptr, const int32_t* colm, const double* vals,
                         double* S);
void pgxk_csr_to_stencil_h(hipStream_t st, int n, int sx, const int32_t* rowptr, const int32_t* colm,
                           const double* vals, dsten_t* Sh, int frame_ny = 0);
void pgxk_rap7(hipStream_t st, const GridLevel& f, const double* Sf, const GridLevel& c, double* Sc);
void pgxk_rap7h(hipStream_t st, const GridLevel& f, const dsten_t* Sfh, const GridLevel& c, dsten_t* Sch, int pack = 0, int staged = 0);
void pgxk_st_apply(hipStream_t st, int mode, const GridLevel& L, double alpha, const double* xu, const double* xp,
                   const double* bu, const double* bp, double omega, int first, double* yu, double* yp);
void pgxk_restrict(hipStream_t st, const GridLevel& f, const double* ru, const double* rp, const GridLevel& c,
                   double* bu, double* bp);
void pgxk_prolong_add(hipStream_t st, const GridLevel& c, const double* cu, const double* cp, const GridLevel& f,
                      double* xu, double* xp);
void pgxk_coarse_mask(hipStream_t st, const GridLevel& c, uint8_t* mask_c, const GridLevel& f);
void pgxk_view_to_global(hipStream_t st, int ns, int n_view, int n_glob, int sx, int row0, int own0, int nown,
                         const double* in, double* out);
void pgxk_st_smooth2(hipStream_t st, int post, const GridLevel& L, double alpha, const double* xu, const double* xp,
                     const GridLevel* C, const double* cu, const double* cp, const double* bu, const double* bp,
                     double omega, int remap, double* yu, double* yp);
void pgxk_st_spmv(hipStream_t st, const GridLevel& L, double alpha, const double* xu, const double* xp, int remap, double* yu,
                  double* yp, const float2* xf = nullptr ,
                  const double* bu = nullptr, const double* bp = nullptr, double s = 1.0 );
void pgxk_lincomb_f2(hipStream_t st, size_t n, int nv, const float2* Zf, size_t ldz, const double* y, double* xu, double* xp,
                     int accumulate = 1);
void pgxk_pack_d4(hipStream_t st, const GridLevel& L);
void pgxk_st_resid_restrict(hipStream_t st, const GridLevel& L, double alpha, const double* xu, const double* xp,
                            const double* bu, const double* bp, const GridLevel& C, int remap, double* cbu,
                            double* cbp);
#ifndef PGX_BAL_CAP
#define PGX_BAL_CAP 1536
#endif
void pgxk_bspmv_bal(hipStream_t st, int n, int nblk, const int32_t* blk, const int32_t* rowptr, const int32_t* colm,
                    const double* K, const double* M, const uint8_t* code, const double* table, const double* D, double alpha,
                    const uint8_t* mask, const double* xu, const double* xp, const double* bu, const double* bp, int remap,
                    double* yu, double* yp, const float* Df = nullptr);
void pgxk_dict_assign(hipStream_t st, int64_t nnz, const double* K, const double* M, int ntab, const double* table, double tk,
                      double tm, uint8_t* code, int* fail, int cap, double* fail_v);
void pgxk_bspmv_stream(hipStream_t st, int n, size_t fill_lds_bytes, const int32_t* rowptr, const int32_t* colm,
                       const double* K, const double* M, const double* D, double alpha, const uint8_t* mask,
                       const double* xu, const double* xp, int remap, double* yu, double* yp);

struct QuadTab2 {
  double L[PGX_MAX_NQ][3];
  double N[PGX_MAX_NQ][6];
  double dN[PGX_MAX_NQ][6][2];
  double w[PGX_MAX_NQ];
  int nq;
};
void pgxk_bphi_p2(hipStream_t st, int nc, int n, const int32_t* cdofs, const double* coords, const double* phi_q,
                  QuadTab2 q, const int32_t* v2c_ptr, const int32_t* v2c_ent, double* stash, double* bphi,
                  const double* geo = nullptr );
void pgxk_residual_p2_cells(hipStream_t st, int nc, int n, const int32_t* cdofs, const double* coords,
                            const uint8_t* mask, const double* gbc, const double* x, const double* xk, double alpha,
                            double f, QuadTab2 q, const int32_t* v2c_ptr, const int32_t* v2c_ent, double* stash, double* F,
                            const double* geo = nullptr);
void pgxk_residual_final(hipStream_t st, int n, const uint8_t* mask, const double* gbc, const double* bphi,
                         const double* x, double* F);
void pgxk_fill_rows_p2(hipStream_t st, int mode, int n, size_t lds_bytes, const int32_t* rowptr,
                       const int32_t* v2c_ptr, const int32_t* v2c_ent, const int32_t* v2c_pos, const int32_t* cdofs,
                       const double* coords, const double* psi, QuadTab2 q, double* out, const double* geo = nullptr);
void pgxk_fill_rows_p1_Dp2(hipStream_t st, int nv, size_t lds_bytes, const int32_t* rowptr, const int32_t* v2c_ptr,
                           const int32_t* v2c_ent, const int32_t* v2c_pos, const int32_t* cdofs, const double* coords,
                           const double* psi, QuadTab2 q, double* out, const double* geo = nullptr);
void pgxk_p2_restrict(hipStream_t st, int nv, int n2, const int32_t* v2e_ptr, const int32_t* v2e, const uint8_t* mask1,
                      const double* ru2, const double* rp2, double* bu1, double* bp1);
void pgxk_p2_prolong_add(hipStream_t st, int nv, int n2, const int32_t* edge_ends, const double* cu, const double* cp,
                         double* xu, double* xp);
void pgxk_observables_p2_cells(hipStream_t st, int nc, int n, const int32_t* cdofs, const double* coords,
                               const double* x, const double* xk, double alpha, double f, QuadTab2 q, double* partials,
                               int nblocks, const double* geo = nullptr);
void pgxk_observables_final(hipStream_t st, int nblocks, const double* partials, double* out6);
void pgxk_observables_final_raw(hipStream_t st, int nblocks, const double* partials, double* out6);
void pgxk_patch_positions(hipStream_t st, int np, int NN, const int32_t* pdof, const int32_t* rowptr, const int32_t* colm,
                          int32_t* ppos);
void pgxk_patch_invert(hipStream_t st, int np, int NN, const int32_t* pdof, const int32_t* ppos, const double* K, const double* M,
                       const double* D, const uint8_t* mask, double alpha, void* pinv, int f32, int sym);
void pgxk_patch_sweep(hipStream_t st, int np, int NN, int nv, int nd, const int32_t* pdof, const int32_t* edge_ends,
                      const void* pinv, int f32, int sym, const double* ru, const double* rp, double omega, double* xu, double* xp,
                      double* su, double* sp);
size_t pgxk_patch_inverse_bytes(int np, int NN, int f32, int sym);
struct P2StTab {
  int delta[46];
  unsigned char isedge[46];
  int lofs[46];
  int lds;
  double aK[46], M[46];
  double kmax, mmax;
};
#define PGX_P2ST_BW 128
void pgxk_p2st_apply(hipStream_t st, const P2StTab& S, int nx, int nv, int i0, int ni, int j0, int nj, size_t G, const void* Dst, int f32,
                     const double* xu, const double* xp, const double* bu, const double* bp, double* yu, double* yp);
void pgxk_p2st_pack(hipStream_t st, int nx, int nv, int i0, int ni, int j0, int nj, size_t G, const int32_t* rowptr, const double* D,
                    void* Dst, int f32);
void pgxk_p2st_check(hipStream_t st, const P2StTab& S, int nx, int nv, int i0, int ni, int j0, int nj, double alpha_ref, double tol,
                     const int32_t* rowptr, const double* K, const double* M, int* fail);
void pgxk_p2_rows_csr(hipStream_t st, int nrows, const int32_t* rows, const int32_t* rowptr, const int32_t* colm, const double* K,
                      const double* M, const double* D, double alpha, const uint8_t* mask, const double* xu, const double* xp,
                      const double* bu, const double* bp, double* yu, double* yp);
void pgxk_resid_fill_p1(hipStream_t st, int write_d, int n, size_t lds_bytes, const int32_t* rowptr,
                        const int32_t* v2c_ptr, const int32_t* v2c_ent, const int32_t* v2c_pos, const int32_t* cells,
                        const double* coords, const uint8_t* mask, const double* gbc, const double* bphi,
                        const double* x, const double* xk, double alpha, double f, QuadTab q, double* F, double* Dout,
                        const double* geo = nullptr);
void pgxk_resid_fill_grid(hipStream_t st, int write_d, const GridLevel& L, size_t lds_bytes, const int32_t* rowptr,
                          const int32_t* v2c_ptr, const int32_t* v2c_ent, const int32_t* v2c_pos, const int32_t* cells,
                          const double* coords, const uint8_t* mask, const double* gbc, const double* bphi, const double* x,
                          const double* xk, double alpha, double f, QuadTab q, double* F, double* Dout, int write_sh,
                          int direct = 0, const int32_t* colm = nullptr);
void pgxk_axpy_dot(hipStream_t st, size_t len, int nv, const double* V, size_t ldv, const double* h1, double* w,
                   double* partials, double* out);
void pgxk_multiaxpy_scale(hipStream_t st, size_t len, int nv, const double* V, size_t ldv, const double* h,
                          double scale, double* w);
void pgxk_multiaxpy_norm(hipStream_t st, size_t len, int nv, const double* V, size_t ldv, const double* h, double* w,
                         double* partials, double* out, int wide = 8);
void pgxk_multiaxpy_norm_f32(hipStream_t st, size_t len, int nv, const float* V, size_t ldv, const double* h, int from_vnext, double* w,
                             float* vnext, double* partials, double* out, int wide = 8);
void pgxk_f_pack_d(hipStream_t st, const GridLevel& L);
void pgxk_f_smooth(hipStream_t st, int K, int first, const GridLevel& L, double alpha, const float2* xf, const double* b64u,
                   const double* b64p, const GridLevel* C, const float2* cf, const double* cdu, const double* cdp, double omega,
                   int remap, float2* yf, double* y64u, double* y64p, float2* cbf = nullptr, double* cb64u = nullptr,
                   double* cb64p = nullptr, double bscale = 1.0,
                   const float* b32u = nullptr, const float* b32p = nullptr);
void pgxk_f_resid_restrict(hipStream_t st, const GridLevel& L, double alpha, const float2* xf, const GridLevel& C, int remap,
                           float2* cbf, double* cb64u, double* cb64p);
int pgxk_st_smooth6_ok(const GridLevel& L);
void pgxk_st_smoothK(hipStream_t st, int K, int post, const GridLevel& L, double alpha, const double* xu,
                     const double* xp, const GridLevel* C, const double* cu, const double* cp, const double* bu,
                     const double* bp, double omega, int remap, double* yu, double* yp);
```

proximalgalerkin_amd/csrc/pgx_kernels.hip:

```cpp
#include "pgx_internal.h"
#include "pgx_stencil.h"
#include <algorithm>
#include <type_traits>

#define WAVE 64

static bool first_use_on_device(int slot) {
  static bool done[4][64] = {};
  int dev = 0;
  if (hipGetDevice(&dev) != hipSuccess || dev < 0 || dev >= 64) return true;
  if (done[slot][dev]) return false;
  done[slot][dev] = true;
  return true;
}

__device__ __forceinline__ double wave_sum(double v) {
#pragma unroll
  for (int o = WAVE / 2; o > 0; o >>= 1) v += __shfl_xor(v, o, WAVE);
  return v;
}

__device__ __forceinline__ double2 ldnt2(const double2* p) {
  typedef double v2d __attribute__((ext_vector_type(2)));
  const v2d v = __builtin_nontemporal_load((const v2d*)p);
// ... 1142 lines not shown
  if (tail && i == ng) {
    const double2 x0 = x[2 * i];
    *(float2*)(y + 4 * i) = make_float2((float)(x0.x * a), (float)(x0.y * a));
  }
}
void pgxk_scale_copy_f32(hipStream_t st, size_t len, double a, const double* x, float* y) {
  const size_t ng = len / 4;
  hipLaunchKernelGGL(k_scale_copy_f32, stream_grid(ng + 1), dim3(PGX_BLOCK), 0, st, ng, (int)(len - 4 * ng), a, (const double2*)x, y);
}

__global__ void __launch_bounds__(PGX_BLOCK) k_set(size_t len, double a, double* __restrict__ y) {
  for (size_t i = blockIdx.x * (size_t)blockDim.x + threadIdx.x; i < len; i += (size_t)gridDim.x * blockDim.x)
    y[i] = a;
}
void pgxk_set(hipStream_t st, size_t len, double a, double* y) {
  hipLaunchKernelGGL(k_set, stream_grid(len), dim3(PGX_BLOCK), 0, st, len, a, y);
}

__global__ void __launch_bounds__(PGX_BLOCK) k_to_float(size_t len, const double* __restrict__ x, float* __restrict__ y) {
  for (size_t i = blockIdx.x * (size_t)blockDim.x + threadIdx.x; i < len; i += (size_t)gridDim.x * blockDim.x) y[i] = (float)x[i];
}
void pgxk_to_float(hipStream_t st, size_t len, const double* x, float* y) {
  hipLaunchKernelGGL(k_to_float, stream_grid(len), dim3(PGX_BLOCK), 0, st, len, x, y);
}

template <class T>
struct GsLane;
template <>
struct GsLane<double> {
  static constexpr int G = 2;
};
template <>
struct GsLane<float> {
  static constexpr int G = 4;
};
template <int G>
__device__ __forceinline__ void gs_ld_basis(const double* p, double* a) {
  static_assert(G == 2, "fp64 basis: two elements per lane");
  const double2 v = ldnt2((const double2*)p);
  a[0] = v.x, a[1] = v.y;
}
template <int G>
__device__ __forceinline__ void gs_ld_basis(const float* p, double* a) {
  typedef float vf __attribute__((ext_vector_type(G)));
  const vf v = __builtin_nontemporal_load((const vf*)p);
#pragma unroll
  for (int k = 0; k < G; ++k) a[k] = (double)v[k];
}
template <int G>
__device__ __forceinline__ void gs_ld(const double* p, double* a) {
#pragma unroll
  for (int k = 0; k < G; k += 2) {
    const double2 v = *(const double2*)(p + k);
    a[k] = v.x, a[k + 1] = v.y;
  }
}
template <int G>
__device__ __forceinline__ void gs_ld(const float* p, double* a) {
  typedef float vf __attribute__((ext_vector_type(G)));
  const vf v = *(const vf*)p;
#pragma unroll
  for (int k = 0; k < G; ++k) a[k] = (double)v[k];
}
template <int G>
__device__ __forceinline__ void gs_st(double* p, const double* a, double* s) {
#pragma unroll
  for (int k = 0; k < G; k += 2) {
    *(double2*)(p + k) = make_double2(a[k], a[k + 1]);
    s[k] = a[k], s[k + 1] = a[k + 1];
  }
}
template <int G>
__device__ __forceinline__ void gs_st(float* p, const double* a, double* s) {
  typedef float vf __attribute__((ext_vector_type(G)));
  vf v;
#pragma unroll
  for (int k = 0; k < G; ++k) {
    v[k] = (float)a[k];
    s[k] = (double)v[k];
  }
  *(vf*)p = v;
}

template <int NV, class VT, class WT>
__global__ void __launch_bounds__(PGX_BLOCK) k_multidot(size_t ng, int tail, const VT* __restrict__ V, size_t ldv,
                                                        const WT* __restrict__ w,
                                                        double* __restrict__ partials, int pstride, int poff) {
  constexpr int G = GsLane<VT>::G;
  __shared__ double sm[PGX_BLOCK / WAVE];
  double acc[NV];
#pragma unroll
  for (int v = 0; v < NV; ++v) acc[v] = 0.0;
  size_t i = blockIdx.x * (size_t)blockDim.x + threadIdx.x;
  for (; i < ng; i += (size_t)gridDim.x * blockDim.x) {
    double wv[G];
    gs_ld<G>(w + G * i, wv);
#pragma unroll
    for (int v = 0; v < NV; ++v) {
      double a[G];
      gs_ld_basis<G>(V + v * ldv + G * i, a);
#pragma unroll
      for (int k = 0; k < G; k += 2) acc[v] += fma(a[k], wv[k], a[k + 1] * wv[k + 1]);
    }
  }
  if (G == 4 && tail && i == ng) {
    double wv[2];
    gs_ld<2>(w + G * i, wv);
#pragma unroll
    for (int v = 0; v < NV; ++v) {
      double a[2];
      gs_ld<2>(V + v * ldv + G * i, a);
      acc[v] += fma(a[0], wv[0], a[1] * wv[1]);
    }
  }
#pragma unroll
  for (int v = 0; v < NV; ++v) {
    const double r = block_sum(acc[v], sm);
    if (threadIdx.x == 0) partials[(size_t)blockIdx.x * pstride + poff + v] = r;
  }
}

__global__ void __launch_bounds__(PGX_BLOCK) k_reduce_partials(int nblocks, int nv, const double* __restrict__ p,
                                                               double* __restrict__ out) {
  __shared__ double sm[PGX_BLOCK / WAVE];
  const int v = blockIdx.x;
  double s = 0.0;
  for (int b = threadIdx.x; b < nblocks; b += blockDim.x) s += p[(size_t)b * nv + v];
  const double r = block_sum(s, sm);
  if (threadIdx.x == 0) out[v] = r;
}
__global__ void __launch_bounds__(PGX_BLOCK) k_reduce_partials_scaled(int nblocks, int nv, const double* __restrict__ p, PgxDotScale sc,
                                                                      double* __restrict__ out) {
  __shared__ double sm[PGX_BLOCK / WAVE];
  const int v = blockIdx.x;
  double s = 0.0;
  for (int b = threadIdx.x; b < nblocks; b += blockDim.x) s += p[(size_t)b * nv + v];
  const double r = block_sum(s, sm);
  if (threadIdx.x == 0) out[v] = r * sc.s[v];
}

int pgxk_multidot_blocks(size_t len) {
  size_t nb = (len / 2 + PGX_BLOCK - 1) / PGX_BLOCK;
  if (nb > PGX_RED_BLOCKS) nb = PGX_RED_BLOCKS;
  return nb == 0 ? 1 : (int)nb;
}

template <class VT, class WT>
static void multidot_t(hipStream_t st, size_t len, int nv, const VT* V, size_t ldv, const WT* w, double* partials, double* out,
                       const PgxDotScale* scale, int wide) {
  constexpr int G = GsLane<VT>::G;
  const size_t ng = len / G;
  const int tail = (int)(len - G * ng);
  const size_t nb = (size_t)pgxk_multidot_blocks(len);
  dim3 grid((unsigned)nb), block(PGX_BLOCK);
  const int cap = wide > 16 ? 16 : wide < 1 ? 1 : wide;
  int done = 0;
  while (done < nv) {
    const int rem = nv - done;
    const VT* Vp = V + (size_t)done * ldv;
#define PGX_MD(N)                                                                                                          \
  case N:                                                                                                                  \
    hipLaunchKernelGGL((k_multidot<N, VT, WT>), grid, block, 0, st, ng, tail, Vp, ldv, w, partials, nv, done);             \
    break
    const int take = rem >= cap ? cap : rem;
    switch (take) {
      PGX_MD(1);
      PGX_MD(2);
      PGX_MD(3);
      PGX_MD(4);
      PGX_MD(5);
      PGX_MD(6);
      PGX_MD(7);
      PGX_MD(8);
      PGX_MD(9);
      PGX_MD(10);
      PGX_MD(11);
      PGX_MD(12);
      PGX_MD(13);
      PGX_MD(14);
      PGX_MD(15);
      PGX_MD(16);
    }
#undef PGX_MD
    done += take;
  }
  if (!out) return;
  if (scale)
    hipLaunchKernelGGL(k_reduce_partials_scaled, dim3(nv), block, 0, st, (int)nb, nv, partials, *scale, out);
  else
    hipLaunchKernelGGL(k_reduce_partials, dim3(nv), block, 0, st, (int)nb, nv, partials, out);
}
void pgxk_multidot(hipStream_t st, size_t len, int nv, const double* V, size_t ldv, const double* w, double* partials,
                   double* out, const PgxDotScale* scale, int wide) {
  multidot_t(st, len, nv, V, ldv, w, partials, out, scale, wide);
}
void pgxk_multidot_f32(hipStream_t st, size_t len, int nv, const float* V, size_t ldv, const double* w, const float* wf,
                       double* partials, double* out, const PgxDotScale* scale, int wide) {
  if (w)
    multidot_t(st, len, nv, V, ldv, w, partials, out, scale, wide);
  else
    multidot_t(st, len, nv, V, ldv, wf, partials, out, scale, wide);
}

__global__ void __launch_bounds__(PGX_BLOCK) k_reduce_publish(int nb, const double* __restrict__ p, int nrows, double* out, double* hout,
                                                              int n1, const double* src1, double* dst1, unsigned long long seq,
                                                              unsigned long long* seqp) {
  __shared__ double sm[PGX_BLOCK / WAVE];
  for (int r = 0; r < nrows; ++r) {
    const double* row = p + (size_t)r * nb;
    double s = 0.0;
    for (int b = threadIdx.x; b < nb; b += blockDim.x) s += row[b];
    const double t = block_sum(s, sm);
    if (threadIdx.x == 0) {
      out[r] = t;
      __hip_atomic_store(hout + r, t, __ATOMIC_RELAXED, __HIP_MEMORY_SCOPE_SYSTEM);
    }
  }
  if (threadIdx.x >= WAVE) return;
  for (int i = threadIdx.x; i < n1; i += WAVE) __hip_atomic_store(dst1 + i, src1[i], __ATOMIC_RELAXED, __HIP_MEMORY_SCOPE_SYSTEM);
  __threadfence_system();
  if (threadIdx.x == 0) __hip_atomic_store(seqp, seq, __ATOMIC_RELEASE, __HIP_MEMORY_SCOPE_SYSTEM);
}
void pgxk_reduce_publish(hipStream_t st, int nb, const double* partials, int nrows, double* out, double* hout, int n1, const double* src1,
                         double* dst1, unsigned long long seq, unsigned long long* seqp) {
  hipLaunchKernelGGL(k_reduce_publish, dim3(1), dim3(PGX_BLOCK), 0, st, nb, partials, nrows, out, hout, n1, src1, dst1, seq, seqp);
}

__global__ void __launch_bounds__(PGX_BLOCK) k_axpy_norms(size_t len2, double a, const double2* __restrict__ x, double2* __restrict__ y,
                                                          double* __restrict__ partials) {
  __shared__ double sm[PGX_BLOCK / WAVE];
  double accx = 0.0, accy = 0.0;
  for (size_t i = blockIdx.x * (size_t)blockDim.x + threadIdx.x; i < len2; i += (size_t)gridDim.x * blockDim.x) {
    double2 xv = x[i], yv = y[i];
    yv.x += a * xv.x;
    yv.y += a * xv.y;
    y[i] = yv;
    accx += xv.x * xv.x + xv.y * xv.y;
    accy += yv.x * yv.x + yv.y * yv.y;
  }
  const double rx = block_sum(accx, sm);
  const double ry = block_sum(accy, sm);
  if (threadIdx.x == 0) {
    partials[blockIdx.x] = rx;
    partials[gridDim.x + blockIdx.x] = ry;
  }
}
int pgxk_axpy_norms(hipStream_t st, size_t len, const double* x, double* y, double* partials) {
  const int nb = pgxk_multidot_blocks(len);
  hipLaunchKernelGGL(k_axpy_norms, dim3(nb), dim3(PGX_BLOCK), 0, st, len / 2, 1.0, (const double2*)x, (double2*)y, partials);
  return nb;
}

template <int NV>
__global__ void __launch_bounds__(PGX_BLOCK) k_multiaxpy(size_t len2, const double2* __restrict__ V, size_t ldv2,
                                                         const double* __restrict__ h, double2* __restrict__ w) {
  double hv[NV];
#pragma unroll
  for (int v = 0; v < NV; ++v) hv[v] = h[v];
  for (size_t i = blockIdx.x * (size_t)blockDim.x + threadIdx.x; i < len2; i += (size_t)gridDim.x * blockDim.x) {
    double2 wv = w[i];
#pragma unroll
    for (int v = 0; v < NV; ++v) {
      const double2 a = V[v * ldv2 + i];
      wv.x -= hv[v] * a.x;
      wv.y -= hv[v] * a.y;
    }
    w[i] = wv;
  }
}

__global__ void __launch_bounds__(PGX_BLOCK) k_axpy_dot(size_t len, int nv, const double* __restrict__ V, size_t ldv,
                                                        const double* __restrict__ h1, double* __restrict__ w,
                                                        double* __restrict__ partials) {
  extern __shared__ double sh[];
  double* hs = sh + (size_t)(nv + 1) * PGX_BLOCK;
  const int t = threadIdx.x;
  const int lane = t & (WAVE - 1), wid = t / WAVE;
  if (t < nv) hs[t] = h1[t];
  constexpr int NW = PGX_BLOCK / WAVE;
  constexpr int MAXA = 16;
  double acc[MAXA];
#pragma unroll
  for (int k = 0; k < MAXA; ++k) acc[k] = 0.0;
  const size_t nchunks = (len + PGX_BLOCK - 1) / PGX_BLOCK;
  for (size_t chunk = blockIdx.x; chunk < nchunks; chunk += gridDim.x) {
    __syncthreads();
    const size_t i = chunk * PGX_BLOCK + t;
    const bool live = i < len;
    double wv = live ? w[i] : 0.0;
#pragma unroll 8
    for (int v = 0; v < nv; ++v) {
      const double a = live ? __builtin_nontemporal_load(V + (size_t)v * ldv + i) : 0.0;
      sh[v * PGX_BLOCK + t] = a;
      wv -= hs[v] * a;
    }
    if (live) w[i] = wv;
    sh[nv * PGX_BLOCK + t] = wv;
    __syncthreads();
    const double* wl = sh + (size_t)nv * PGX_BLOCK;
    double wr[NW];
#pragma unroll
    for (int r = 0; r < NW; ++r) wr[r] = wl[lane + WAVE * r];
#pragma unroll
    for (int k = 0; k < MAXA; ++k) {
      const int v = wid + NW * k;
      if (v <= nv) {
        const double* sv = sh + (size_t)v * PGX_BLOCK;
#pragma unroll
        for (int r = 0; r < NW; ++r) acc[k] += sv[lane + WAVE * r] * wr[r];
      }
    }
  }
#pragma unroll
  for (int k = 0; k < MAXA; ++k) {
    const int v = wid + NW * k;
    if (v <= nv) {
      const double r = wave_sum(acc[k]);
      if (lane == 0) partials[(size_t)v * gridDim.x + blockIdx.x] = r;
    }
  }
}

__global__ void __launch_bounds__(PGX_BLOCK) k_reduce_rows(int nb, const double* __restrict__ p,
                                                           double* __restrict__ out) {
  __shared__ double sm[PGX_BLOCK / WAVE];
  const double* row = p + (size_t)blockIdx.x * nb;
  double s = 0.0;
  for (int b = threadIdx.x; b < nb; b += blockDim.x) s += row[b];
  const double r = block_sum(s, sm);
  if (threadIdx.x == 0) out[blockIdx.x] = r;
}

void pgxk_axpy_dot(hipStream_t st, size_t len, int nv, const double* V, size_t ldv, const double* h1, double* w,
                   double* partials, double* out) {
  size_t nchunks = (len + PGX_BLOCK - 1) / PGX_BLOCK;
  const unsigned nb = (unsigned)std::min<size_t>(nchunks, 4096);
  const size_t lds = ((size_t)(nv + 1) * PGX_BLOCK + nv) * sizeof(double);
  if (first_use_on_device(1))
    hipFuncSetAttribute((const void*)k_axpy_dot, hipFuncAttributeMaxDynamicSharedMemorySize, 128 * 1024);
  hipLaunchKernelGGL(k_axpy_dot, dim3(nb), dim3(PGX_BLOCK), lds, st, len, nv, V, ldv, h1, w, partials);
  hipLaunchKernelGGL(k_reduce_rows, dim3(nv + 1), dim3(PGX_BLOCK), 0, st, (int)nb, partials, out);
}

template <int NV>
__global__ void __launch_bounds__(PGX_BLOCK) k_multiaxpy_scale(size_t len2, const double2* __restrict__ V, size_t ldv2,
                                                               const double* __restrict__ h, double scale, int last,
                                                               double2* __restrict__ w) {
  double hv[NV];
#pragma unroll
  for (int v = 0; v < NV; ++v) hv[v] = h[v];
  for (size_t i = blockIdx.x * (size_t)blockDim.x + threadIdx.x; i < len2; i += (size_t)gridDim.x * blockDim.x) {
    double2 wv = w[i];
#pragma unroll
    for (int v = 0; v < NV; ++v) {
      const double2 a = ldnt2(V + v * ldv2 + i);
      wv.x -= hv[v] * a.x;
      wv.y -= hv[v] * a.y;
    }
    if (last) {
      wv.x *= scale;
      wv.y *= scale;
    }
    w[i] = wv;
  }
}

void pgxk_multiaxpy_scale(hipStream_t st, size_t len, int nv, const double* V, size_t ldv, const double* h,
                          double scale, double* w) {
  const size_t len2 = len / 2, ldv2 = ldv / 2;
  dim3 grid = stream_grid(len2), block(PGX_BLOCK);
  int done = 0;
  while (done < nv) {
    const int rem = nv - done;
    const double2* Vp = (const double2*)(V + (size_t)done * ldv);
    const int step = rem >= 8 ? 8 : rem >= 4 ? 4 : rem >= 2 ? 2 : 1;
    const int last = (done + step == nv);
    if (step == 8)
      hipLaunchKernelGGL(k_multiaxpy_scale<8>, grid, block, 0, st, len2, Vp, ldv2, h + done, scale, last, (double2*)w);
    else if (step == 4)
      hipLaunchKernelGGL(k_multiaxpy_scale<4>, grid, block, 0, st, len2, Vp, ldv2, h + done, scale, last, (double2*)w);
    else if (step == 2)
      hipLaunchKernelGGL(k_multiaxpy_scale<2>, grid, block, 0, st, len2, Vp, ldv2, h + done, scale, last, (double2*)w);
    else
      hipLaunchKernelGGL(k_multiaxpy_scale<1>, grid, block, 0, st, len2, Vp, ldv2, h + done, scale, last, (double2*)w);
    done += step;
  }
}

template <int NV, bool NORM, class VT, class WT>
__global__ void __launch_bounds__(PGX_BLOCK) k_multiaxpy_norm(size_t ng, int tail, const VT* __restrict__ V, size_t ldv,
                                                              const double* __restrict__ h, const WT* __restrict__ win,
                                                              typename std::conditional<NORM && std::is_same<VT, float>::value, float, double>::type* __restrict__ wout,
                                                              double* __restrict__ partials) {
  typedef typename std::conditional<NORM && std::is_same<VT, float>::value, float, double>::type OT;
  constexpr int G = GsLane<VT>::G;
  const WT* const wi = std::is_same<WT, OT>::value ? (const WT*)wout : win;
  __shared__ double sm[PGX_BLOCK / WAVE];
  double hv[NV];
#pragma unroll
  for (int v = 0; v < NV; ++v) hv[v] = h[v];
  double acc = 0.0;
  size_t i = blockIdx.x * (size_t)blockDim.x + threadIdx.x;
  for (; i < ng; i += (size_t)gridDim.x * blockDim.x) {
    double wv[G], s[G];
    gs_ld<G>(wi + G * i, wv);
#pragma unroll
    for (int v = 0; v < NV; ++v) {
      double a[G];
      gs_ld_basis<G>(V + v * ldv + G * i, a);
#pragma unroll
      for (int k = 0; k < G; ++k) wv[k] -= hv[v] * a[k];
    }
    gs_st<G>(wout + G * i, wv, s);
    if (NORM) {
#pragma unroll
      for (int k = 0; k < G; k += 2) acc += fma(s[k + 1], s[k + 1], s[k] * s[k]);
    }
  }
  if (G == 4 && tail && i == ng) {
    double wv[2], s[2];
    gs_ld<2>(wi + G * i, wv);
#pragma unroll
    for (int v = 0; v < NV; ++v) {
      double a[2];
      gs_ld<2>(V + v * ldv + G * i, a);
      wv[0] -= hv[v] * a[0];
      wv[1] -= hv[v] * a[1];
    }
    gs_st<2>(wout + G * i, wv, s);
    if (NORM) acc += fma(s[1], s[1], s[0] * s[0]);
  }
  if (NORM) {
    const double r = block_sum(acc, sm);
    if (threadIdx.x == 0) partials[blockIdx.x] = r;
  }
}
int pgxk_stream_blocks(size_t len) { return (int)stream_grid(len / 2).x; }
template <int N, class VT>
static void launch_multiaxpy_norm(hipStream_t st, dim3 grid, size_t ng, int tail, const VT* Vp, size_t ldv, const double* h, bool last,
                                  bool inf, double* w, float* wf, double* partials) {
  const dim3 block(PGX_BLOCK);
  if constexpr (std::is_same<VT, double>::value) {
    if (last)
      hipLaunchKernelGGL((k_multiaxpy_norm<N, true, double, double>), grid, block, 0, st, ng, tail, Vp, ldv, h, (const double*)nullptr, w, partials);
    else
      hipLaunchKernelGGL((k_multiaxpy_norm<N, false, double, double>), grid, block, 0, st, ng, tail, Vp, ldv, h, (const double*)nullptr, w, partials);
  } else {
    if (last && inf)
      hipLaunchKernelGGL((k_multiaxpy_norm<N, true, float, float>), grid, block, 0, st, ng, tail, Vp, ldv, h, (const float*)nullptr, wf, partials);
    else if (last)
      hipLaunchKernelGGL((k_multiaxpy_norm<N, true, float, double>), grid, block, 0, st, ng, tail, Vp, ldv, h, (const double*)w, wf, partials);
    else if (inf)
      hipLaunchKernelGGL((k_multiaxpy_norm<N, false, float, float>), grid, block, 0, st, ng, tail, Vp, ldv, h, (const float*)wf, w, partials);
    else
      hipLaunchKernelGGL((k_multiaxpy_norm<N, false, float, double>), grid, block, 0, st, ng, tail, Vp, ldv, h, (const double*)nullptr, w, partials);
  }
}
template <class VT>
static void multiaxpy_norm_t(hipStream_t st, size_t len, int nv, const VT* V, size_t ldv, const double* h, bool inf, double* w, float* wf,
                             double* partials, double* out, int wide) {
  constexpr int G = GsLane<VT>::G;
  const size_t ng = len / G;
  const int tail = (int)(len - G * ng);
  dim3 grid = stream_grid(len / 2);
  const int cap = wide > 16 ? 16 : wide < 1 ? 1 : wide;
  int done = 0;
  while (done < nv) {
    const int step = std::min(cap, nv - done);
    const bool last = done + step == nv;
    const VT* Vp = V + (size_t)done * ldv;
#define PGX_MAN(N)                                                                                                     \
  case N:                                                                                                              \
    launch_multiaxpy_norm<N>(st, grid, ng, tail, Vp, ldv, h + done, last, inf && done == 0, w, wf, partials);          \
    break
    switch (step) {
      PGX_MAN(16);
      PGX_MAN(15);
      PGX_MAN(14);
      PGX_MAN(13);
      PGX_MAN(12);
      PGX_MAN(11);
      PGX_MAN(10);
      PGX_MAN(9);
      PGX_MAN(8);
      PGX_MAN(7);
      PGX_MAN(6);
      PGX_MAN(5);
      PGX_MAN(4);
      PGX_MAN(3);
      PGX_MAN(2);
      default: launch_multiaxpy_norm<1>(st, grid, ng, tail, Vp, ldv, h + done, last, inf && done == 0, w, wf, partials); break;
    }
#undef PGX_MAN
    done += step;
  }
  if (out) hipLaunchKernelGGL(k_reduce_rows, dim3(1), dim3(PGX_BLOCK), 0, st, (int)grid.x, partials, out);
}
void pgxk_multiaxpy_norm(hipStream_t st, size_t len, int nv, const double* V, size_t ldv, const double* h, double* w,
                         double* partials, double* out, int wide) {
  multiaxpy_norm_t(st, len, nv, V, ldv, h, false, w, nullptr, partials, out, wide);
}
void pgxk_multiaxpy_norm_f32(hipStream_t st, size_t len, int nv, const float* V, size_t ldv, const double* h, int from_vnext, double* w,
                             float* vnext, double* partials, double* out, int wide) {
  multiaxpy_norm_t(st, len, nv, V, ldv, h, from_vnext != 0, w, vnext, partials, out, wide);
}

void pgxk_multiaxpy(hipStream_t st, size_t len, int nv, const double* V, size_t ldv, const double* h, double* w) {
  const size_t len2 = len / 2, ldv2 = ldv / 2;
  dim3 grid = stream_grid(len2), block(PGX_BLOCK);
  int done = 0;
  while (done < nv) {
    const int rem = nv - done;
    const double2* Vp = (const double2*)(V + (size_t)done * ldv);
    if (rem >= 8) {
      hipLaunchKernelGGL(k_multiaxpy<8>, grid, block, 0, st, len2, Vp, ldv2, h + done, (double2*)w);
      done += 8;
    } else if (rem >= 4) {
      hipLaunchKernelGGL(k_multiaxpy<4>, grid, block, 0, st, len2, Vp, ldv2, h + done, (double2*)w);
      done += 4;
    } else if (rem >= 2) {
      hipLaunchKernelGGL(k_multiaxpy<2>, grid, block, 0, st, len2, Vp, ldv2, h + done, (double2*)w);
      done += 2;
    } else {
      hipLaunchKernelGGL(k_multiaxpy<1>, grid, block, 0, st, len2, Vp, ldv2, h + done, (double2*)w);
      done += 1;
    }
  }
}

__global__ void __launch_bounds__(PGX_BLOCK) k_lincomb(size_t len2, int nv, const double2* __restrict__ Z,
                                                       size_t ldz2, const double* __restrict__ y,
                                                       double2* __restrict__ x, int accumulate) {
  for (size_t i = blockIdx.x * (size_t)blockDim.x + threadIdx.x; i < len2; i += (size_t)gridDim.x * blockDim.x) {
    double2 s = accumulate ? x[i] : make_double2(0.0, 0.0);
    for (int v = 0; v < nv; ++v) {
      const double2 a = Z[v * ldz2 + i];
      const double yv = y[v];
      s.x += yv * a.x;
      s.y += yv * a.y;
    }
    x[i] = s;
  }
}
__global__ void __launch_bounds__(PGX_BLOCK) k_lincomb_f2(size_t n, int nv, const float2* __restrict__ Zf, size_t ldz,
                                                          const double* __restrict__ y, double* __restrict__ xu, double* __restrict__ xp,
                                                          int accumulate) {
  for (size_t i = blockIdx.x * (size_t)blockDim.x + threadIdx.x; i < n; i += (size_t)gridDim.x * blockDim.x) {
    double su = accumulate ? xu[i] : 0.0, sp = accumulate ? xp[i] : 0.0;
    for (int v = 0; v < nv; ++v) {
      const float2 a = Zf[v * ldz + i];
      const double yv = y[v];
      su += yv * (double)a.x;
      sp += yv * (double)a.y;
    }
    xu[i] = su;
    xp[i] = sp;
  }
}
void pgxk_lincomb_f2(hipStream_t st, size_t n, int nv, const float2* Zf, size_t ldz, const double* y, double* xu, double* xp,
                     int accumulate) {
  const unsigned grid = (unsigned)std::min<size_t>((n + PGX_BLOCK - 1) / PGX_BLOCK, 256 * 32);
  hipLaunchKernelGGL(k_lincomb_f2, dim3(grid), dim3(PGX_BLOCK), 0, st, n, nv, Zf, ldz, y, xu, xp, accumulate);
}

void pgxk_lincomb(hipStream_t st, size_t len, int nv, const double* Z, size_t ldz, const double* y, double* x,
                  int accumulate) {
  hipLaunchKernelGGL(k_lincomb, stream_grid(len / 2), dim3(PGX_BLOCK), 0, st, len / 2, nv, (const double2*)Z,
                     ldz / 2, y, (double2*)x, accumulate);
}

__device__ __forceinline__ constexpr double pw(int dx, int dy) {
  return (dx == 0 && dy == 0) ? 1.0
         : ((dx == 1 && dy == 0) || (dx == -1 && dy == 0) || (dx == 0 && dy == 1) || (dx == 0 && dy == -1) ||
            (dx == 1 && dy == 1) || (dx == -1 && dy == -1))
             ? 0.5
             : 0.0;
}

__global__ void __launch_bounds__(PGX_BLOCK) k_csr_to_stencil(int n, int sx, const int32_t* __restrict__ rowptr,
                                                              const int32_t* __restrict__ colm,
                                                              const double* __restrict__ vals,
                                                              double* __restrict__ S) {
  const int i = blockIdx.x * blockDim.x + threadIdx.x;
  if (i >= n) return;
  double s[7] = {0, 0, 0, 0, 0, 0, 0};
  for (int k = rowptr[i]; k < rowptr[i + 1]; ++k) {
    const int o = (colm[k] & 0x7fffffff) - i;
    const double v = vals[k];
    if (o == 0) s[0] = v;
    else if (o == 1) s[1] = v;
    else if (o == -1) s[2] = v;
    else if (o == sx) s[3] = v;
    else if (o == -sx) s[4] = v;
    else if (o == sx + 1) s[5] = v;
    else if (o == -sx - 1) s[6] = v;
  }
#pragma unroll
  for (int k = 0; k < 7; ++k) S[(size_t)k * n + i] = s[k];
}
void pgxk_csr_to_stencil(hipStream_t st, int n, int sx, const int32_t* rowptr, const int32_t* colm, const double* vals,
                         double* S) {
  hipLaunchKernelGGL(k_csr_to_stencil, dim3((n + PGX_BLOCK - 1) / PGX_BLOCK), dim3(PGX_BLOCK), 0, st, n, sx, rowptr,
                     colm, vals, S);
}

__global__ void __launch_bounds__(PGX_BLOCK) k_rap7(int nxf, int nyf, int nf, const double* __restrict__ Sf, int nxc,
                                                    int nyc, int ncv, double* __restrict__ Sc) {
  const int C = blockIdx.x * blockDim.x + threadIdx.x;
  if (C >= ncv) return;
  constexpr int OX[7] = {0, 1, -1, 0, 0, 1, -1};
  constexpr int OY[7] = {0, 0, 0, 1, -1, 1, -1};
  const int sxc = nxc + 1, sxf = nxf + 1;
  const int I = C % sxc, Jc = C / sxc;
  double out[7] = {0, 0, 0, 0, 0, 0, 0};
#pragma unroll
  for (int oa = 0; oa < 7; ++oa) {
    const int ax = 2 * I + OX[oa], ay = 2 * Jc + OY[oa];
    if (ax < 0 || ax > nxf || ay < 0 || ay > nyf) continue;
    const double wa = pw(OX[oa], OY[oa]);
    const size_t a = (size_t)ay * sxf + ax;
#pragma unroll
    for (int os = 0; os < 7; ++os) {
      const double coef = wa * Sf[(size_t)os * nf + a];
      const int dx = OX[oa] + OX[os], dy = OY[oa] + OY[os];
#pragma unroll
      for (int oc = 0; oc < 7; ++oc) {
        const double w2 = pw(dx - 2 * OX[oc], dy - 2 * OY[oc]);
        if (w2 != 0.0) out[oc] += coef * w2;
      }
    }
  }
#pragma unroll
  for (int oc = 0; oc < 7; ++oc) {
    const int nx_ = I + OX[oc], ny_ = Jc + OY[oc];
    const bool ok = nx_ >= 0 && nx_ <= nxc && ny_ >= 0 && ny_ <= nyc;
    Sc[(size_t)oc * ncv + C] = ok ? out[oc] : 0.0;
  }
}
void pgxk_rap7(hipStream_t st, const GridLevel& f, const double* Sf, const GridLevel& c, double* Sc) {
  hipLaunchKernelGGL(k_rap7, dim3((c.n + PGX_BLOCK - 1) / PGX_BLOCK), dim3(PGX_BLOCK), 0, st, f.nx, f.ny, f.n, Sf, c.nx,
                     c.ny, c.n, Sc);
}

__device__ __forceinline__ void ld7h(const dsten_t* __restrict__ Sh, int n, int sx, int v, int i, int j, int nx,
                                     int ny, double d[7]) {
  d[0] = Sh[v];
  d[1] = (i < nx) ? Sh[(size_t)n + v] : 0.0;
  d[2] = (i > 0) ? Sh[(size_t)n + v - 1] : 0.0;
  d[3] = (j < ny) ? Sh[(size_t)2 * n + v] : 0.0;
  d[4] = (j > 0) ? Sh[(size_t)2 * n + v - sx] : 0.0;
  d[5] = (i < nx && j < ny) ? Sh[(size_t)3 * n + v] : 0.0;
// ... 1992 lines not shown
```

proximalgalerkin_amd/csrc/pgx_mg32.hip:

```cpp
#include <algorithm>

#include "pgx_internal.h"
#include "pgx_stencil.h"

#define F32_BLOCK 512
#ifndef F32_LEAN
#define F32_LEAN 0
#endif
#ifndef F32_WAVES_EU
#define F32_WAVES_EU 2
#endif
#ifndef F32_K6_SPLIT
#define F32_K6_SPLIT 0
#endif
#ifndef F32_K6_TY_TOP
#define F32_K6_TY_TOP 20
#endif
#ifndef F32_LDS_SINGLE
#define F32_LDS_SINGLE 1
#endif
#define F32_RR_CYB 2
#define F32_TB 2
__host__ __device__ constexpr int f32_tb(int K, int RR) { return (K == 6 && !RR) ? 4 : F32_TB; }

// ... 906 lines not shown
    if (ty == 4)
      launch_f_smooth<4, 3>(st, first, A, L.interior_free);
    else if (ty == 8)
      launch_f_smooth<8, 3>(st, first, A, L.interior_free);
    else
      launch_f_smooth<16, 3>(st, first, A, L.interior_free);
  } else {
    if (ty == 4)
      launch_f_smooth<4, 2>(st, first, A, L.interior_free);
    else if (ty == 8)
      launch_f_smooth<8, 2>(st, first, A, L.interior_free);
    else
      launch_f_smooth<16, 2>(st, first, A, L.interior_free);
  }
}

struct FRrArgs {
  int nx, ny, n, nbnd, nxc, nyc, remap;
  RrGrid g;
  const double *K, *M;
  const void* Dq;
  int dbf16;
  const uint8_t *mask, *mask_c;
  const float2 *xf, *bf;
  float2* cbf;
  double *cb64u, *cb64p;
  float alpha;
  FConst sc;
};

template <class DT, bool CB64>
__device__ __forceinline__ void f_rr_fast(int tx, int ty, const FRrArgs& A, float2* ximg, float2* rimg, float2* exch) {
  constexpr int W = 64, CX = 30, CY = 8, HX = 2 * CY + 3, HR = 2 * CY + 1, NW = F32_BLOCK / 64, R = (HX + NW - 1) / NW;
  const int sx = A.nx + 1, sxc = A.nxc + 1;
  const int I0 = tx * CX, J0 = ty * CY;
  const int i0 = 2 * I0 - 2, j0 = 2 * J0 - 2;
  const int lane = threadIdx.x & 63;
  const int wave = __builtin_amdgcn_readfirstlane(threadIdx.x >> 6);
  const int gi = i0 + lane;
  const bool act = lane >= 1 && lane < W - 1;
  const DT* const Dq = static_cast<const DT*>(A.Dq);
  float2 xa[R], rb[R];
  DT dw[R];
  float4 dq[R];
#pragma unroll
  for (int k = 0; k < R; ++k) {
    const int lj = wave + NW * k;
    if (lj < HX) {
      const unsigned v = (unsigned)((j0 + lj) * sx + gi);
      xa[k] = A.xf[v];
      if (lj <= HR) dw[k] = Dq[v];
      if (lj >= 1 && lj <= HR) rb[k] = A.bf[v];
    }
  }
#pragma unroll
  for (int k = 0; k < R; ++k) {
    const int lj = wave + NW * k;
    if (lj < HX) ximg[lj * W + lane] = xa[k];
    if (lj <= HR) {
      dq[k] = f_unpack_d(dw[k]);
      exch[lj * W + lane] = make_float2(dq[k].z, dq[k].w);
    }
  }
  __syncthreads();
  const float k0 = A.sc.k0, k1 = A.sc.k1, k3 = A.sc.k3, k5 = A.sc.k5, m0 = A.sc.m0, m1 = A.sc.m1, m3 = A.sc.m3, m5 = A.sc.m5;
#pragma unroll
  for (int k = 0; k < R; ++k) {
    const int lj = wave + NW * k;
    if (lj < 1 || lj > HR) continue;
    const float d2 = lane_shr1f(dq[k].y), d4 = exch[(lj - 1) * W + lane].x, d6 = exch[(lj - 1) * W + lane - 1].y;
    const int q = lj * W + lane;
    const float2 x0 = ximg[q], x1 = ximg[q + 1], x2 = ximg[q - 1], x3 = ximg[q + W], x4 = ximg[q - W], x5 = ximg[q + W + 1],
                 x6 = ximg[q - W - 1];
    const float u12 = x1.x + x2.x, u34 = x3.x + x4.x, u56 = x5.x + x6.x;
    const float p12 = x1.y + x2.y, p34 = x3.y + x4.y, p56 = x5.y + x6.y;
    const float au = (k0 * x0.x + k1 * u12) + (k3 * u34 + k5 * u56) + ((m0 * x0.y + m1 * p12) + (m3 * p34 + m5 * p56));
    const float ap = ((m0 * x0.x + m1 * u12) + (m3 * u34 + m5 * u56)) -
                     (((dq[k].x * x0.y + dq[k].y * x1.y) + (d2 * x2.y + dq[k].z * x3.y)) + ((d4 * x4.y + dq[k].w * x5.y) + d6 * x6.y));
    if (act) rimg[(lj - 1) * W + lane] = make_float2(rb[k].x - au, rb[k].y - ap);
  }
  __syncthreads();
  if (wave < CY && lane < CX) {
    const int q = (2 * wave + 1) * W + 2 * lane + 2;
    F_LDS7(rimg, q, W, r0, r1, r2, r3, r4, r5, r6)
    const float su = r0.x + 0.5f * (((r1.x + r2.x) + (r3.x + r4.x)) + (r5.x + r6.x));
    const float sp = r0.y + 0.5f * (((r1.y + r2.y) + (r3.y + r4.y)) + (r5.y + r6.y));
    const int C = (J0 + wave) * sxc + I0 + lane;
    if (CB64) {
      A.cb64u[C] = (double)su;
      A.cb64p[C] = (double)sp;
    } else {
      A.cbf[C] = make_float2(su, sp);
    }
  }
}

template <class DT, bool CB64>
__device__ __forceinline__ void f_rr_bnd(int tx, int ty, int sub, const FRrArgs& A, float2* ximg, float2* rimg, float2* exch) {
  constexpr int W = 64, CX = 30, CY = 8, CYB = F32_RR_CYB, HX = 2 * CYB + 3, HR = 2 * CYB + 1, NW = F32_BLOCK / 64;
  static_assert(HX <= NW && CY % CYB == 0, "one image row per wave");
  const int nx = A.nx, ny = A.ny, sx = nx + 1, sxc = A.nxc + 1;
  const int I0 = tx * CX, J0 = ty * CY + sub * CYB;
  const int i0 = 2 * I0 - 2, j0 = 2 * J0 - 2;
  const int lane = threadIdx.x & 63;
  const int wave = __builtin_amdgcn_readfirstlane(threadIdx.x >> 6);
  const int gi = i0 + lane, lj = wave, gj = j0 + lj;
  const bool in = lj < HX && gi >= 0 && gi <= nx && gj >= 0 && gj <= ny;
  const bool act = lane >= 1 && lane < W - 1;
  DT dw;
  f_zero_d(dw);
  float2 rb = make_float2(0.f, 0.f), xa = make_float2(0.f, 0.f);
  float kv[7], mv[7];
  bool bc = false;
#pragma unroll
  for (int t = 0; t < 7; ++t) {
    kv[t] = A.sc.kc[t];
    mv[t] = A.sc.mc[t];
  }
  if (in) {
    const int v = gj * sx + gi;
    xa = A.xf[v];
    bc = A.mask[v] != 0;
    if (lj <= HR) dw = static_cast<const DT*>(A.Dq)[v];
    if (lj >= 1 && lj <= HR) {
      rb = A.bf[v];
      if (!(A.sc.uniform && gi > 0 && gi < nx && gj > 0 && gj < ny)) {
#pragma unroll
        for (int t = 0; t < 7; ++t) {
          kv[t] = A.alpha * (float)A.K[(size_t)t * A.n + v];
          mv[t] = (float)A.M[(size_t)t * A.n + v];
        }
      }
    }
  }
  const float4 dq = f_unpack_d(dw);
  if (lj < HX) {
    ximg[lj * W + lane] = make_float2(bc ? 0.f : xa.x, xa.y);
    exch[lj * W + lane] = make_float2(dq.z, dq.w);
  }
  __syncthreads();
  if (lj >= 1 && lj <= HR) {
    const float d2 = lane_shr1f(dq.y), d4 = exch[(lj - 1) * W + lane].x, d6 = exch[(lj - 1) * W + lane - 1].y;
    const int q = lj * W + lane;
    const float2 x0 = ximg[q], x1 = ximg[q + 1], x2 = ximg[q - 1], x3 = ximg[q + W], x4 = ximg[q - W], x5 = ximg[q + W + 1],
                 x6 = ximg[q - W - 1];
    float au = ((kv[0] * x0.x + kv[1] * x1.x) + (kv[2] * x2.x + kv[3] * x3.x)) + ((kv[4] * x4.x + kv[5] * x5.x) + kv[6] * x6.x) +
               (((mv[0] * x0.y + mv[1] * x1.y) + (mv[2] * x2.y + mv[3] * x3.y)) + ((mv[4] * x4.y + mv[5] * x5.y) + mv[6] * x6.y));
    const float ap = (((mv[0] * x0.x + mv[1] * x1.x) + (mv[2] * x2.x + mv[3] * x3.x)) + ((mv[4] * x4.x + mv[5] * x5.x) + mv[6] * x6.x)) -
                     (((dq.x * x0.y + dq.y * x1.y) + (d2 * x2.y + dq.z * x3.y)) + ((d4 * x4.y + dq.w * x5.y) + d6 * x6.y));
    if (bc) au = xa.x;
    if (act) rimg[(lj - 1) * W + lane] = in ? make_float2(rb.x - au, rb.y - ap) : make_float2(0.f, 0.f);
  }
  __syncthreads();
  if (wave < CYB && lane < CX) {
    const int I = I0 + lane, J = J0 + wave;
    if (I <= A.nxc && J <= A.nyc) {
      const int q = (2 * wave + 1) * W + 2 * lane + 2;
      F_LDS7(rimg, q, W, r0, r1, r2, r3, r4, r5, r6)
      float su = r0.x + 0.5f * (((r1.x + r2.x) + (r3.x + r4.x)) + (r5.x + r6.x));
      const float sp = r0.y + 0.5f * (((r1.y + r2.y) + (r3.y + r4.y)) + (r5.y + r6.y));
      const int C = J * sxc + I;
      if (A.mask_c[C]) su = 0.f;
      if (CB64) {
        A.cb64u[C] = (double)su;
        A.cb64p[C] = (double)sp;
      } else {
        A.cbf[C] = make_float2(su, sp);
      }
    }
  }
}

template <class DT, bool CB64>
__global__ void __launch_bounds__(F32_BLOCK) k_f_resid_restrict(const FRrArgs A) {
  constexpr int W = 64, CY = 8, HX = 2 * CY + 3, HR = 2 * CY + 1, PAD = W + 1;
  __shared__ float2 ximg_[HX * W + 2 * PAD], rimg_[HR * W + 2 * PAD], exch_[HX * W + 2 * PAD];
  int b = blockIdx.x;
  if (b < A.nbnd) {
    constexpr int NSUB = 8 / F32_RR_CYB;
    const int sub = b % NSUB;
    b /= NSUB;
    int tx, ty;
    const RrGrid& g = A.g;
    const int side = g.ntx - g.nfx;
    if (b < g.ntx) {
      tx = b;
      ty = 0;
    } else if ((b -= g.ntx) < g.nfy * side) {
      ty = 1 + b / side;
      const int r = b % side;
      tx = r == 0 ? 0 : g.nfx + r;
    } else {
      b -= g.nfy * side;
      ty = g.nfy + 1 + b / g.ntx;
      tx = b % g.ntx;
    }
    f_rr_bnd<DT, CB64>(tx, ty, sub, A, ximg_ + PAD, rimg_ + PAD, exch_ + PAD);
  } else {
    b = xcd_block(b - A.nbnd, gridDim.x - A.nbnd, A.remap);
    f_rr_fast<DT, CB64>(1 + b % A.g.nfx, 1 + b / A.g.nfx, A, ximg_ + PAD, rimg_ + PAD, exch_ + PAD);
  }
}

void pgxk_f_resid_restrict(hipStream_t st, const GridLevel& L, double alpha, const float2* xf, const GridLevel& C, int remap,
                           float2* cbf, double* cb64u, double* cb64p) {
  constexpr int CX = 30, CY = 8;
  FRrArgs A;
  A.nx = L.nx;
  A.ny = L.ny;
  A.n = L.n;
  A.nxc = C.nx;
  A.nyc = C.ny;
  A.remap = remap;
  A.K = L.K;
  A.M = L.M;
  A.Dq = L.Dq;
  A.dbf16 = L.dbf16;
  A.mask = L.mask;
  A.mask_c = C.mask;
  A.xf = xf;
  A.bf = L.bf;
  A.cbf = cbf;
  A.cb64u = cb64u;
  A.cb64p = cb64p;
  A.alpha = (float)alpha;
  A.sc = make_fconst(L, alpha);
  RrGrid& g = A.g;
  g.ntx = (C.nx + CX) / CX;
  g.nty = (C.ny + CY) / CY;
  g.nfx = (L.nx - 62) >= 2 * CX ? (L.nx - 62) / (2 * CX) : 0;
  g.nfy = (L.ny - 1 - 2 * CY) >= 2 * CY ? (L.ny - 1 - 2 * CY) / (2 * CY) : 0;
  g.nfx = std::min(g.nfx, g.ntx - 1);
  g.nfy = std::min(g.nfy, g.nty - 1);
  if (!L.interior_free || !C.interior_free || g.nfx <= 0 || g.nfy <= 0) g.nfx = g.nfy = 0;
  const int nfast = g.nfx * g.nfy;
  A.nbnd = (g.ntx * g.nty - nfast) * (CY / F32_RR_CYB);
  const dim3 grid(A.nbnd + nfast), block(F32_BLOCK);
  if (L.dbf16) {
    if (cb64u)
      hipLaunchKernelGGL((k_f_resid_restrict<uint2, true>), grid, block, 0, st, A);
    else
// ... 9 lines not shown
```

proximalgalerkin_amd/problem.py:

```python
from __future__ import annotations

import ctypes as C
import warnings
from dataclasses import dataclass

import numpy as np

from . import _lib
from .fem import Constant, DirichletBC, Function, QuadratureFunction

SNES_CONVERGED_FNORM_ABS = 2
SNES_CONVERGED_FNORM_RELATIVE = 3
SNES_CONVERGED_SNORM_RELATIVE = 4
SNES_DIVERGED_LINEAR_SOLVE = -3
SNES_DIVERGED_FNORM_NAN = -4
SNES_DIVERGED_MAX_IT = -5
SNES_DIVERGED_DTOL = -9


class ConvergenceError(RuntimeError):
    """Raised for snes_error_if_not_converged / ksp_error_if_not_converged (obstacle_pg.py:132,135)."""


@dataclass
# ... 254 lines not shown
        return ms.value, by.value

    def spmv_bench_cold(self, reps=20):
        ms, by = C.c_double(0), C.c_double(0)
        _lib.check(self._lib, self._h, self._lib.pgx_spmv_bench_cold(self._h, int(reps), C.byref(ms), C.byref(by)),
                   "pgx_spmv_bench_cold")
        return ms.value, by.value

    def spmv_select(self, kind=-1):
        act = C.c_int(0)
        _lib.check(self._lib, self._h, self._lib.pgx_spmv_select(self._h, int(kind), C.byref(act)), "pgx_spmv_select")
        return act.value

    def p2_stencil_info(self):
        out = (C.c_int32 * 5)()
        _lib.check(self._lib, self._h, self._lib.pgx_p2_stencil_info(self._h, out), "pgx_p2_stencil_info")
        return tuple(int(v) for v in out)

    def comm_counts(self, reset=False):
        out = (C.c_int64 * 4)()
        _lib.check(self._lib, self._h, self._lib.pgx_comm_counts(self._h, out, int(reset)), "pgx_comm_counts")
        return dict(zip(("halo_exchanges", "allreduces", "vcycles", "krylov_iterations"), (int(v) for v in out)))

    def smoother_bench(self, reps=20):
        ms, by = C.c_double(0), C.c_double(0)
        _lib.check(self._lib, self._h, self._lib.pgx_smoother_bench(self._h, int(reps), C.byref(ms), C.byref(by)),
                   "pgx_smoother_bench")
        return ms.value, by.value

    def vcycle_bench(self, level, reps=50):
        ms, nl = C.c_double(0), C.c_int(0)
        _lib.check(self._lib, self._h, self._lib.pgx_vcycle_bench(self._h, int(level), int(reps), C.byref(ms), C.byref(nl)),
                   "pgx_vcycle_bench")
        return ms.value, nl.value

    def _check_code(self, rc, what):
        try:
            _lib.check(self._lib, self._h, rc, what)
        except _lib.PgxError as e:
            e.code = rc
            raise

    def mg_levels(self):
        nx, ny, f, d = C.c_int32(0), C.c_int32(0), C.c_int32(0), C.c_int32(0)
        l = 0
        while self._lib.pgx_mg_level_export(self._h, l, C.byref(nx), C.byref(ny), None, None, None, C.byref(f), C.byref(d)) == 0:
            l += 1
        if l == 0:
            self.mg_level_export(0)
        return l

    def mg_level_export(self, level):
        lib = self._lib
        nx, ny, f, d = C.c_int32(0), C.c_int32(0), C.c_int32(0), C.c_int32(0)
        self._check_code(lib.pgx_mg_level_export(self._h, int(level), C.byref(nx), C.byref(ny), None, None, None, C.byref(f), C.byref(d)),
                         "pgx_mg_level_export")
        n = (nx.value + 1) * (ny.value + 1)
        Dh = np.empty((4, n))
        Dq = np.zeros((n, 4), dtype=np.float32) if f.value else None
        mask = np.empty(n, dtype=np.uint8)
        self._check_code(lib.pgx_mg_level_export(self._h, int(level), C.byref(nx), C.byref(ny), _lib.dptr(Dh),
                                                 None if Dq is None else Dq.ctypes.data_as(C.POINTER(C.c_float)),
                                                 mask.ctypes.data_as(C.POINTER(C.c_uint8)), C.byref(f), C.byref(d)), "pgx_mg_level_export")
        return dict(nx=nx.value, ny=ny.value, Dh=Dh, Dq=Dq, mask=mask.astype(bool), f32=f.value, dbf16=d.value)

    def vcycle_apply(self, level, b, nu=6, omega=0.75, in_form=0, out_form=0, scale=1.0):
        b = np.ascontiguousarray(b, dtype=np.float64)
        z = np.empty_like(b)
        nx, ny = C.c_int32(0), C.c_int32(0)
        self._check_code(self._lib.pgx_mg_level_export(self._h, int(level), C.byref(nx), C.byref(ny), None, None, None, None, None),
                         "pgx_vcycle_apply")
        if b.shape != (2 * (nx.value + 1) * (ny.value + 1),):
            raise ValueError(f"b must hold [u | psi] of level {level}: {2 * (nx.value + 1) * (ny.value + 1)} entries")
        self._check_code(self._lib.pgx_vcycle_apply(self._h, int(level), int(nu), float(omega), int(in_form), int(out_form), float(scale),
                                                    _lib.dptr(b), _lib.dptr(z)), "pgx_vcycle_apply")
        return z

    def observables(self):
        self._sync_inputs()
        out = np.empty(6)
        _lib.check(self._lib, self._h, self._lib.pgx_observables(self._h, _lib.dptr(out)), "pgx_observables")
        return out

    def owned_edge_range(self):
        off, cnt = C.c_int64(0), C.c_int64(0)
        _lib.check(self._lib, self._h, self._lib.pgx_owned_edge_range(self._h, C.byref(off), C.byref(cnt)),
                   "pgx_owned_edge_range")
        return off.value, cnt.value

    def owned_range(self):
        off, cnt = C.c_int64(0), C.c_int64(0)
        _lib.check(self._lib, self._h, self._lib.pgx_owned_range(self._h, C.byref(off), C.byref(cnt)),
                   "pgx_owned_range")
        return off.value, cnt.value

    def profile(self, enable=None, reset=False):
        if enable is not None:
            self._lib.pgx_profile_enable(self._h, int(enable))
        ms = np.empty(8)
        self._lib.pgx_profile_get(self._h, _lib.dptr(ms), int(reset))
        keys = ["residual", "jacobian_fill", "mg_setup", "spmv", "vcycle", "orthogonalisation", "observables",
                "newton_total"]
        return dict(zip(keys, ms.tolist()))

    def close(self):
        if getattr(self, "_h", None):
            self._lib.pgx_destroy(self._h)
            self._h = None

    def __del__(self):
        try:
            self.close()
        except Exception:
            pass


class SNESProblem:

    def __init__(self, F, u, J=None, bcs=None, form_compiler_options=None, jit_options=None, device=0):
        self.L = F
        self.a = J if J is not None else derivative(F, u)
        self.bcs = bcs
        self.u = u
        self._backend = NonlinearProblem(F, u, bcs=bcs, J=self.a, device=device)

    @staticmethod
    def _arr(v):
        return v.array if hasattr(v, "array") else v

    def F(self, snes, x, F):
        out, _ = self._backend.residual(self._arr(x))
        self._arr(F)[:] = out

    def J(self, snes, x, J, P):
        self._backend.assemble_jacobian(self._arr(x))


class SNESSolver:

    def __init__(self, problem: SNESProblem, options: dict):
        self.problem = problem
        self.options = options
        b = problem._backend
        b._opts, b._flags = _parse_options(b._lib, options)
        b.solver = _SNES(b._opts)
        self._snes = b.solver

    def solve(self):
        b = self.problem._backend
        b.solve()
        return self._snes.getConvergedReason(), self._snes.getIterationNumber()
```

Baseline: 158.1 Newton iterations/s.

## Fuse reductions into last-block ticketed second stage that publishes to host

Adds a device ticket counter so the last block of the multidot, multiaxpy-norm and axpy-norms kernels does the final cross-block reduction and writes the result straight to mapped host memory. This removes the separate k_reduce_rows / reduce-publish launch per GMRES orthogonalisation step and per Newton step norm. It also passes small solution coefficients by value into the lincomb kernels, which drops a host-to-device copy. It adds atomics and a fallback path, plus a self-check API that compares the ticketed reduction bitwise against the old path.

```diff
diff --git a/include/pgx.h b/include/pgx.h
--- a/include/pgx.h
+++ b/include/pgx.h
@@ -105,6 +105,8 @@
 int pgx_newton_solve(pgx_handle* h, const pgx_snes_opts* opts, int* reason, int* its, int* lin_its);
 int pgx_observables(pgx_handle* h, double out[6]);
 
+int pgx_reduce_selfcheck(pgx_handle* h, int nv, int64_t len, int basis_f32, int reps, uint64_t seed, int64_t* mismatches);
+
 int pgx_profile_enable(pgx_handle* h, int on);
 int pgx_profile_get(pgx_handle* h, double ms[8], int reset);
 
diff --git a/proximalgalerkin_amd/_lib.py b/proximalgalerkin_amd/_lib.py
--- a/proximalgalerkin_amd/_lib.py
+++ b/proximalgalerkin_amd/_lib.py
@@ -370,6 +370,7 @@
     ("pgx_newton_solve", C.c_int,
      [_H, C.POINTER(pgx_snes_opts), C.POINTER(C.c_int), C.POINTER(C.c_int), C.POINTER(C.c_int)]),
     ("pgx_observables", C.c_int, [_H, c_double_p]),
+    ("pgx_reduce_selfcheck", C.c_int, [_H, C.c_int, C.c_int64, C.c_int, C.c_int, C.c_uint64, c_int64_p]),
     ("pgx_profile_enable", C.c_int, [_H, C.c_int]),
     ("pgx_profile_get", C.c_int, [_H, c_double_p, C.c_int]),
     ("pgx_partition_rows", C.c_int,
diff --git a/proximalgalerkin_amd/csrc/pgx_api.hip b/proximalgalerkin_amd/csrc/pgx_api.hip
--- a/proximalgalerkin_amd/csrc/pgx_api.hip
+++ b/proximalgalerkin_amd/csrc/pgx_api.hip
@@ -120,6 +120,8 @@
   int host_poll = 1;
   int gs_wide = 16;
   int fused_publish = 1;
+  int ticket_reduce = 1;
+  unsigned long long* d_ticket = nullptr;
   int fused_resid = 1;
   int lean_rhs = 1;
   int fused_step = 1;
@@ -1161,6 +1163,7 @@
   if (const char* e = pgx_tune("PGX_HOST_POLL")) h->host_poll = atoi(e);
   if (const char* e = pgx_tune("PGX_GS_WIDE")) h->gs_wide = atoi(e) >= 16 ? 16 : 8;
   if (const char* e = pgx_tune("PGX_FUSED_PUBLISH")) h->fused_publish = atoi(e);
+  if (const char* e = pgx_tune("PGX_TICKET_REDUCE")) h->ticket_reduce = atoi(e);
   if (const char* e = pgx_tune("PGX_FUSED_RESID")) h->fused_resid = atoi(e);
   if (const char* e = pgx_tune("PGX_LEAN_RHS")) h->lean_rhs = atoi(e);
   if (const char* e = pgx_tune("PGX_FUSED_STEP")) h->fused_step = atoi(e);
@@ -1434,6 +1437,8 @@
     DALLOC(h->d_small, 4 * (h->restart + 2));
     DALLOC(h->partials, (size_t)PGX_RED_BLOCKS * (h->restart + 2));
     DALLOC(h->partials2, ((n2 + PGX_BLOCK - 1) / PGX_BLOCK) * (size_t)62);
+    DALLOC(h->d_ticket, PGX_TK_WORDS);
+    HIPCHK(hipMemsetAsync(h->d_ticket, 0, sizeof(unsigned long long) * PGX_TK_WORDS, h->st));
     {
       const size_t nsm = 4 * (size_t)(h->restart + 2);
       HIPCHK(hipHostMalloc((void**)&h->h_small, sizeof(double) * (nsm + 2), hipHostMallocMapped | hipHostMallocCoherent));
@@ -1626,6 +1631,24 @@
   const unsigned long long seq = ++h->seq;
   pgxk_reduce_publish(h->st, nb, partials, nrows, dout, h->h_small_dev + hoff_r, (int)n1, dsrc1, h->h_small_dev + hoff1, seq, h->h_seq_dev);
   return wait_published(h, seq);
+}
+static bool ticketed(const pgx_handle* h) { return h->ticket_reduce && fused_readback(h); }
+static PgxTicket ticket_publish(pgx_handle* h, unsigned long long* seq, size_t hoff_r, const double* dsrc1 = nullptr, size_t n1 = 0,
+                                size_t hoff1 = 0) {
+  PgxTicket t;
+  t.ctr = h->d_ticket;
+  t.hout = h->h_small_dev + hoff_r;
+  t.n1 = (int)n1;
+  t.src1 = dsrc1;
+  t.dst1 = h->h_small_dev + hoff1;
+  t.seq = *seq = ++h->seq;
+  t.seqp = h->h_seq_dev;
+  return t;
+}
+static PgxTicket ticket_device(pgx_handle* h) {
+  PgxTicket t;
+  t.ctr = h->d_ticket;
+  return t;
 }
 static int wait_published(pgx_handle* h, unsigned long long seq) {
   static const double limit_s = [] {
@@ -1664,8 +1687,17 @@
 static int dev_norm(pgx_handle* h, const double* v, double* out, size_t len = 0) {
   if (fused_readback(h)) {
     const size_t l = len ? len : 2 * (size_t)h->nd;
-    pgxk_multidot(h->st, l, 1, v, 0, v, h->partials, nullptr);
-    const int rc = reduce_fetch(h, pgxk_multidot_blocks(l), h->partials, 1, h->d_small, 0);
+    int rc;
+    if (ticketed(h)) {
+      unsigned long long seq;
+      PgxTicket tk = ticket_publish(h, &seq, 0);
+      const bool done = pgxk_multidot(h->st, l, 1, v, 0, v, h->partials, h->d_small, nullptr, 8, &tk);
+      if (!done) h->err = "dev_norm: k_multidot<1> without its second stage";
+      rc = done ? wait_published(h, seq) : PGX_EHIP;
+    } else {
+      pgxk_multidot(h->st, l, 1, v, 0, v, h->partials, nullptr);
+      rc = reduce_fetch(h, pgxk_multidot_blocks(l), h->partials, 1, h->d_small, 0);
+    }
     if (rc) return rc;
     *out = std::sqrt(h->h_small[0]);
     return PGX_OK;
@@ -2596,15 +2628,30 @@
         double* d_h1 = h->d_small;
         double* d_h2 = h->d_small + (m + 2);
         const PgxDotScale* const dsc = lazy ? &sc2 : nullptr;
+        PgxTicket tkd = ticket_device(h);
+        PgxTicket* const tk1 = ticketed(h) ? &tkd : nullptr;
         if (vf32)
-          pgxk_multidot_f32(h->st, nk, j + 1, Vf, ldvf, h->w, nullptr, h->partials, d_h1, dsc, h->gs_wide);
+          pgxk_multidot_f32(h->st, nk, j + 1, Vf, ldvf, h->w, nullptr, h->partials, d_h1, dsc, h->gs_wide, tk1);
         else
-          pgxk_multidot(h->st, nk, j + 1, h->V, nk, wj, h->partials, d_h1, dsc, h->gs_wide);
+          pgxk_multidot(h->st, nk, j + 1, h->V, nk, wj, h->partials, d_h1, dsc, h->gs_wide, tk1);
         if (dist && (rc = allreduce_dev(h, d_h1, j + 1))) return rc;
         double wp2, h1h1 = 0.0, hh = 0.0;
         bool second;
         if (h->cgs_selective) {
-          if (fused_readback(h)) {
+          if (ticketed(h)) {
+            unsigned long long seq;
+            const unsigned long long seq0 = h->seq;
+            PgxTicket tk = ticket_publish(h, &seq, (size_t)(m + 2) + j + 1, d_h1, (size_t)(j + 1), 0);
+            const bool done = vf32 ? pgxk_multiaxpy_norm_f32(h->st, nk, j + 1, Vf, ldvf, d_h1, 0, h->w, vnext, h->partials, d_h2 + j + 1, h->gs_wide, &tk)
+                                   : pgxk_multiaxpy_norm(h->st, nk, j + 1, h->V, nk, d_h1, wj, h->partials, d_h2 + j + 1, h->gs_wide, &tk);
+            if (done) {
+              rc = wait_published(h, seq);
+            } else {
+              h->seq = seq0;
+              rc = reduce_fetch(h, pgxk_stream_blocks(nk), h->partials, 1, d_h2 + j + 1, (size_t)(m + 2) + j + 1, d_h1, (size_t)(j + 1), 0);
+            }
+            if (rc) return rc;
+          } else if (fused_readback(h)) {
             if (vf32)
               pgxk_multiaxpy_norm_f32(h->st, nk, j + 1, Vf, ldvf, d_h1, 0, h->w, vnext, h->partials, nullptr, h->gs_wide);
             else
@@ -2627,10 +2674,12 @@
           wp2 = h->h_small[(m + 2) + j + 1];
           second = wp2 < h->cgs_eta2 * (wp2 + h1h1);
           if (second) {
+            PgxTicket tkd2 = ticket_device(h);
+            PgxTicket* const tk2 = ticketed(h) ? &tkd2 : nullptr;
             if (vf32)
-              pgxk_multidot_f32(h->st, nk, j + 1, Vf, ldvf, nullptr, vnext, h->partials, d_h2, dsc, h->gs_wide);
+              pgxk_multidot_f32(h->st, nk, j + 1, Vf, ldvf, nullptr, vnext, h->partials, d_h2, dsc, h->gs_wide, tk2);
             else
-              pgxk_multidot(h->st, nk, j + 1, h->V, nk, wj, h->partials, d_h2, dsc, h->gs_wide);
+              pgxk_multidot(h->st, nk, j + 1, h->V, nk, wj, h->partials, d_h2, dsc, h->gs_wide, tk2);
             if (dist && (rc = allreduce_dev(h, d_h2, j + 1))) return rc;
             if ((rc = replica_agree(h, d_h2, (size_t)(j + 1)))) return rc;
             if ((rc = fetch_small(h, d_h2, (size_t)(j + 1), (size_t)(m + 2)))) return rc;
@@ -2656,7 +2705,18 @@
         }
         if (second && vf32) {
           double* const d_n2 = d_h2 + j + 1;
-          if (fused_readback(h)) {
+          if (ticketed(h)) {
+            unsigned long long seq;
+            const unsigned long long seq0 = h->seq;
+            PgxTicket tk = ticket_publish(h, &seq, (size_t)(m + 2) + j + 1);
+            if (pgxk_multiaxpy_norm_f32(h->st, nk, j + 1, Vf, ldvf, d_h2, 1, h->w, vnext, h->partials, d_n2, h->gs_wide, &tk)) {
+              rc = wait_published(h, seq);
+            } else {
+              h->seq = seq0;
+              rc = reduce_fetch(h, pgxk_stream_blocks(nk), h->partials, 1, d_n2, (size_t)(m + 2) + j + 1);
+            }
+            if (rc) return rc;
+          } else if (fused_readback(h)) {
             pgxk_multiaxpy_norm_f32(h->st, nk, j + 1, Vf, ldvf, d_h2, 1, h->w, vnext, h->partials, nullptr, h->gs_wide);
             if ((rc = reduce_fetch(h, pgxk_stream_blocks(nk), h->partials, 1, d_n2, (size_t)(m + 2) + j + 1))) return rc;
           } else {
@@ -2736,12 +2796,15 @@
       for (int k = i + 1; k < j; ++k) s -= H[(size_t)i * m + k] * y[k];
       y[i] = s / H[(size_t)i * m + i];
     }
-    for (int i = 0; i < j; ++i) h->h_small[i] = y[i];
-    HIPCHK(hipMemcpyAsync(h->d_small, h->h_small, sizeof(double) * j, hipMemcpyHostToDevice, h->st));
+    const double* const y_arg = j <= PGX_DOT_SCALE_MAX ? y.data() : nullptr;
+    if (!y_arg) {
+      for (int i = 0; i < j; ++i) h->h_small[i] = y[i];
+      HIPCHK(hipMemcpyAsync(h->d_small, h->h_small, sizeof(double) * j, hipMemcpyHostToDevice, h->st));
+    }
     if (zf32)
-      pgxk_lincomb_f2(h->st, (size_t)h->nd, j, Zf, (size_t)h->nd, h->d_small, x, x + h->nd, x_unset ? 0 : 1);
+      pgxk_lincomb_f2(h->st, (size_t)h->nd, j, Zf, (size_t)h->nd, h->d_small, x, x + h->nd, x_unset ? 0 : 1, y_arg);
     else
-      pgxk_lincomb(h->st, n2, j, h->Z, n2, h->d_small, x, x_unset ? 0 : 1);
+      pgxk_lincomb(h->st, n2, j, h->Z, n2, h->d_small, x, x_unset ? 0 : 1, y_arg);
     x_unset = false;
   }
   if (x_unset) pgxk_set(h->st, n2, 0.0, x);
@@ -2771,6 +2834,106 @@
   }
   if (F) return copy_out(h, F, h->F);
   HIPCHK(hipStreamSynchronize(h->st));
+  return PGX_OK;
+}
+
+extern "C" int pgx_reduce_selfcheck(pgx_handle* h, int nv, int64_t len, int basis_f32, int reps, uint64_t seed, int64_t* mismatches) {
+  NEED(h);
+  if (!mismatches) return PGX_EINVAL;
+  const size_t n2 = 2 * (size_t)h->nd;
+  if (h->dist.on || h->lu_comm || !h->host_poll) {
+    h->err = "pgx_reduce_selfcheck: single handles with the polled read-back only";
+    return PGX_EINVAL;
+  }
+  if (nv < 1 || nv > std::min(h->restart - 1, PGX_DOT_SCALE_MAX) || len < 2 || (len & 1) || (size_t)len > n2 || reps < 1) {
+    h->err = "pgx_reduce_selfcheck: 1 <= nv <= min(restart - 1, " + std::to_string(PGX_DOT_SCALE_MAX) + "), len even, 2 <= len <= 2 nd, reps >= 1";
+    return PGX_EINVAL;
+  }
+  const size_t l = (size_t)len;
+  const size_t ldvf = (l + 3) & ~(size_t)3, ldv = basis_f32 ? ldvf : l;
+  float* const Vf = reinterpret_cast<float*>(h->V);
+  float* const vnext = Vf + (size_t)nv * ldvf;
+  double* const wsave = h->Z;
+  double* const wkeep = h->Z + n2;
+  const size_t wwords = basis_f32 ? l / 2 : l;
+  const int m2 = h->restart + 2;
+  double* const d_a = h->d_small;
+  double* const d_b = h->d_small + m2;
+  std::vector<double> ha(nv + 1), hb(nv + 1), pa(nv + 1), pb(nv + 1), wa(wwords), wb(wwords);
+  int64_t bad = 0;
+  auto differ = [](const double* a, const double* b, size_t n) {
+    int64_t d = 0;
+    for (size_t i = 0; i < n; ++i) {
+      uint64_t x, y;
+      memcpy(&x, a + i, 8);
+      memcpy(&y, b + i, 8);
+      d += x != y;
+    }
+    return d;
+  };
+  auto project = [&](double* out, PgxTicket* tk) {
+    return basis_f32 ? pgxk_multiaxpy_norm_f32(h->st, l, nv, Vf, ldvf, d_a, 0, h->w, vnext, h->partials, out, h->gs_wide, tk)
+                     : pgxk_multiaxpy_norm(h->st, l, nv, h->V, ldv, d_a, h->w, h->partials, out, h->gs_wide, tk);
+  };
+  double* const wres = basis_f32 ? reinterpret_cast<double*>(vnext) : h->w;
+  for (int rep = 0; rep < reps; ++rep) {
+    const unsigned long long sd = (unsigned long long)seed * 1000003ull + (unsigned long long)rep * 65ull;
+    for (int i = 0; i < nv; ++i) {
+      if (basis_f32)
+        pgxk_fill_hash(h->st, l, sd + 1 + i, nullptr, Vf + (size_t)i * ldvf);
+      else
+        pgxk_fill_hash(h->st, l, sd + 1 + i, h->V + (size_t)i * ldv, nullptr);
+    }
+    pgxk_fill_hash(h->st, l, sd, h->w, nullptr);
+    pgxk_scale_copy(h->st, l, 1.0, h->w, wsave);
+    PgxDotScale sc;
+    for (int i = 0; i < PGX_DOT_SCALE_MAX; ++i) sc.s[i] = 1.0 + (double)((i * 7 + rep) % 13) / 16.0;
+    const PgxDotScale* const scp = (rep & 1) ? &sc : nullptr;
+    HIPCHK(hipMemsetAsync(h->d_small, 0xff, sizeof(double) * 2 * (size_t)m2, h->st));
+    if (basis_f32)
+      pgxk_multidot_f32(h->st, l, nv, Vf, ldvf, h->w, nullptr, h->partials, d_a, scp, h->gs_wide);
+    else
+      pgxk_multidot(h->st, l, nv, h->V, ldv, h->w, h->partials, d_a, scp, h->gs_wide);
+    PgxTicket tkd = ticket_device(h);
+    const bool dot_tk = basis_f32 ? pgxk_multidot_f32(h->st, l, nv, Vf, ldvf, h->w, nullptr, h->partials, d_b, scp, h->gs_wide, &tkd)
+                                  : pgxk_multidot(h->st, l, nv, h->V, ldv, h->w, h->partials, d_b, scp, h->gs_wide, &tkd);
+    (void)dot_tk;
+    project(nullptr, nullptr);
+    int rc = reduce_fetch(h, pgxk_stream_blocks(l), h->partials, 1, d_a + nv, (size_t)m2 + nv, d_a, (size_t)nv, 0);
+    if (rc) return rc;
+    for (int i = 0; i < nv; ++i) pa[i] = h->h_small[i];
+    pa[nv] = h->h_small[(size_t)m2 + nv];
+    HIPCHK(hipMemcpyAsync(wa.data(), wres, sizeof(double) * wwords, hipMemcpyDeviceToHost, h->st));
+    HIPCHK(hipMemcpyAsync(ha.data(), d_a, sizeof(double) * (nv + 1), hipMemcpyDeviceToHost, h->st));
+    HIPCHK(hipStreamSynchronize(h->st));
+    for (int i = 0; i <= nv; ++i) h->h_small[i] = h->h_small[(size_t)m2 + i] = 0.0;
+    pgxk_scale_copy(h->st, l, 1.0, wsave, h->w);
+    HIPCHK(hipMemsetAsync(wkeep, 0, sizeof(double) * wwords, h->st));
+    if (basis_f32) HIPCHK(hipMemsetAsync(vnext, 0, sizeof(float) * ldvf, h->st));
+    {
+      unsigned long long seq;
+      const unsigned long long seq0 = h->seq;
+      PgxTicket tk = ticket_publish(h, &seq, (size_t)m2 + nv, d_a, (size_t)nv, 0);
+      if (project(d_b + nv, &tk)) {
+        rc = wait_published(h, seq);
+      } else {
+        h->seq = seq0;
+        rc = reduce_fetch(h, pgxk_stream_blocks(l), h->partials, 1, d_b + nv, (size_t)m2 + nv, d_a, (size_t)nv, 0);
+      }
+      if (rc) return rc;
+    }
+    for (int i = 0; i < nv; ++i) pb[i] = h->h_small[i];
+    pb[nv] = h->h_small[(size_t)m2 + nv];
+    HIPCHK(hipMemcpyAsync(wb.data(), wres, sizeof(double) * wwords, hipMemcpyDeviceToHost, h->st));
+    HIPCHK(hipMemcpyAsync(hb.data(), d_b, sizeof(double) * (nv + 1), hipMemcpyDeviceToHost, h->st));
+    HIPCHK(hipStreamSynchronize(h->st));
+    bad += differ(ha.data(), hb.data(), (size_t)nv + 1);
+    bad += differ(pa.data(), pb.data(), (size_t)nv + 1);
+    bad += differ(pa.data(), ha.data(), (size_t)nv + 1);
+    bad += differ(wa.data(), wb.data(), wwords);
+  }
+  HIPCHK(hipGetLastError());
+  *mismatches = bad;
   return PGX_OK;
 }
 
@@ -3352,7 +3515,12 @@
     }
     const bool fstep = h->fused_step && fused_readback(h) && !use_lu && !mg_first && krylov_lean(h);
     int step_nb = 0;
-    if (fstep)
+    const bool fstep_tk = fstep && ticketed(h);
+    if (fstep_tk) {
+      unsigned long long seq;
+      PgxTicket tk = ticket_publish(h, &seq, 2);
+      step_nb = pgxk_axpy_norms(h->st, n2, h->dx, h->xw, h->partials2, h->d_small + 2, &tk);
+    } else if (fstep)
       step_nb = pgxk_axpy_norms(h->st, n2, h->dx, h->xw, h->partials2);
     else
       pgxk_axpy(h->st, n2, 1.0, h->dx, h->xw);
@@ -3375,7 +3543,10 @@
       rsn = PGX_SNES_CONVERGED_FNORM_RELATIVE;
     } else {
       double snorm, xnorm;
-      if (fstep) {
+      if (fstep_tk) {
+        snorm = std::sqrt(h->h_small[2]);
+        xnorm = std::sqrt(h->h_small[3]);
+      } else if (fstep) {
         if ((rc = reduce_fetch(h, step_nb, h->partials2, 2, h->d_small, 0))) return rc;
         snorm = std::sqrt(h->h_small[0]);
         xnorm = std::sqrt(h->h_small[1]);
diff --git a/proximalgalerkin_amd/csrc/pgx_internal.h b/proximalgalerkin_amd/csrc/pgx_internal.h
--- a/proximalgalerkin_amd/csrc/pgx_internal.h
+++ b/proximalgalerkin_amd/csrc/pgx_internal.h
@@ -110,23 +110,36 @@
 void pgxk_scale_copy_f32(hipStream_t st, size_t len, double a, const double* x, float* y);
 void pgxk_set(hipStream_t st, size_t len, double a, double* y);
 void pgxk_to_float(hipStream_t st, size_t len, const double* x, float* y);
+void pgxk_fill_hash(hipStream_t st, size_t len, unsigned long long seed, double* y, float* yf);
 #define PGX_RED_BLOCKS 1024
 #define PGX_DOT_SCALE_MAX 64
 struct PgxDotScale {
   double s[PGX_DOT_SCALE_MAX];
 };
-void pgxk_multidot(hipStream_t st, size_t len, int nv, const double* V, size_t ldv, const double* w, double* partials,
-                   double* out, const PgxDotScale* scale = nullptr, int wide = 8);
-void pgxk_multidot_f32(hipStream_t st, size_t len, int nv, const float* V, size_t ldv, const double* w, const float* wf, double* partials,
-                       double* out, const PgxDotScale* scale = nullptr, int wide = 8);
+#define PGX_TK_SHARDS 64
+#define PGX_TK_STRIDE 16
+#define PGX_TK_WORDS ((PGX_TK_SHARDS + 1) * PGX_TK_STRIDE)
+struct PgxTicket {
+  unsigned long long* ctr = nullptr;
+  double* hout = nullptr;
+  int n1 = 0;
+  const double* src1 = nullptr;
+  double* dst1 = nullptr;
+  unsigned long long seq = 0;
+  unsigned long long* seqp = nullptr;
+};
+bool pgxk_multidot(hipStream_t st, size_t len, int nv, const double* V, size_t ldv, const double* w, double* partials,
+                   double* out, const PgxDotScale* scale = nullptr, int wide = 8, PgxTicket* tk = nullptr);
+bool pgxk_multidot_f32(hipStream_t st, size_t len, int nv, const float* V, size_t ldv, const double* w, const float* wf, double* partials,
+                       double* out, const PgxDotScale* scale = nullptr, int wide = 8, PgxTicket* tk = nullptr);
 int pgxk_multidot_blocks(size_t len);
 int pgxk_stream_blocks(size_t len);
 void pgxk_reduce_publish(hipStream_t st, int nb, const double* partials, int nrows, double* out, double* hout, int n1, const double* src1,
                          double* dst1, unsigned long long seq, unsigned long long* seqp);
-int pgxk_axpy_norms(hipStream_t st, size_t len, const double* x, double* y, double* partials);
+int pgxk_axpy_norms(hipStream_t st, size_t len, const double* x, double* y, double* partials, double* out = nullptr, PgxTicket* tk = nullptr);
 void pgxk_multiaxpy(hipStream_t st, size_t len, int nv, const double* V, size_t ldv, const double* h, double* w);
 void pgxk_lincomb(hipStream_t st, size_t len, int nv, const double* Z, size_t ldz, const double* y, double* x,
-                  int accumulate);
+                  int accumulate, const double* yhost = nullptr);
 
 void pgxk_csr_to_stencil(hipStream_t st, int n, int sx, const int32_t* rowptr, const int32_t* colm, const double* vals,
                          double* S);
@@ -150,7 +163,7 @@
                   double* yp, const float2* xf = nullptr ,
                   const double* bu = nullptr, const double* bp = nullptr, double s = 1.0 );
 void pgxk_lincomb_f2(hipStream_t st, size_t n, int nv, const float2* Zf, size_t ldz, const double* y, double* xu, double* xp,
-                     int accumulate = 1);
+                     int accumulate = 1, const double* yhost = nullptr);
 void pgxk_pack_d4(hipStream_t st, const GridLevel& L);
 void pgxk_st_resid_restrict(hipStream_t st, const GridLevel& L, double alpha, const double* xu, const double* xp,
                             const double* bu, const double* bp, const GridLevel& C, int remap, double* cbu,
@@ -239,10 +252,10 @@
                    double* partials, double* out);
 void pgxk_multiaxpy_scale(hipStream_t st, size_t len, int nv, const double* V, size_t ldv, const double* h,
                           double scale, double* w);
-void pgxk_multiaxpy_norm(hipStream_t st, size_t len, int nv, const double* V, size_t ldv, const double* h, double* w,
-                         double* partials, double* out, int wide = 8);
-void pgxk_multiaxpy_norm_f32(hipStream_t st, size_t len, int nv, const float* V, size_t ldv, const double* h, int from_vnext, double* w,
-                             float* vnext, double* partials, double* out, int wide = 8);
+bool pgxk_multiaxpy_norm(hipStream_t st, size_t len, int nv, const double* V, size_t ldv, const double* h, double* w,
+                         double* partials, double* out, int wide = 8, PgxTicket* tk = nullptr);
+bool pgxk_multiaxpy_norm_f32(hipStream_t st, size_t len, int nv, const float* V, size_t ldv, const double* h, int from_vnext, double* w,
+                             float* vnext, double* partials, double* out, int wide = 8, PgxTicket* tk = nullptr);
 void pgxk_f_pack_d(hipStream_t st, const GridLevel& L);
 void pgxk_f_smooth(hipStream_t st, int K, int first, const GridLevel& L, double alpha, const float2* xf, const double* b64u,
                    const double* b64p, const GridLevel* C, const float2* cf, const double* cdu, const double* cdp, double omega,
diff --git a/proximalgalerkin_amd/csrc/pgx_kernels.hip b/proximalgalerkin_amd/csrc/pgx_kernels.hip
--- a/proximalgalerkin_amd/csrc/pgx_kernels.hip
+++ b/proximalgalerkin_amd/csrc/pgx_kernels.hip
@@ -1248,10 +1248,105 @@
   *(vf*)p = v;
 }
 
-template <int NV, class VT, class WT>
+__global__ void __launch_bounds__(PGX_BLOCK) k_fill_hash(size_t len, unsigned long long seed, double* __restrict__ y, float* __restrict__ yf) {
+  for (size_t i = blockIdx.x * (size_t)blockDim.x + threadIdx.x; i < len; i += (size_t)gridDim.x * blockDim.x) {
+    unsigned long long z = seed * 0x9E3779B97F4A7C15ull + (i + 1) * 0xD1B54A32D192ED03ull;
+    z = (z ^ (z >> 30)) * 0xBF58476D1CE4E5B9ull;
+    z = (z ^ (z >> 27)) * 0x94D049BB133111EBull;
+    z ^= z >> 31;
+    const double v = (double)(z >> 11) * (2.0 / 9007199254740992.0) - 1.0;
+    if (yf)
+      yf[i] = (float)v;
+    else
+      y[i] = v;
+  }
+}
+void pgxk_fill_hash(hipStream_t st, size_t len, unsigned long long seed, double* y, float* yf) {
+  hipLaunchKernelGGL(k_fill_hash, stream_grid(len), dim3(PGX_BLOCK), 0, st, len, seed, y, yf);
+}
+
+__device__ __forceinline__ void tk_store(double* p, double v) { __hip_atomic_store(p, v, __ATOMIC_RELAXED, __HIP_MEMORY_SCOPE_AGENT); }
+__device__ __forceinline__ double tk_load(const double* p) {
+  return __hip_atomic_load(const_cast<double*>(p), __ATOMIC_RELAXED, __HIP_MEMORY_SCOPE_AGENT);
+}
+__device__ __forceinline__ bool tk_arrive(const PgxTicket& tk, double* sm) {
+  if (threadIdx.x == 0) {
+    asm volatile("s_waitcnt vmcnt(0)" ::: "memory");
+    const unsigned nb = gridDim.x, S = nb < PGX_TK_SHARDS ? nb : PGX_TK_SHARDS, sh = blockIdx.x % S;
+    const unsigned long long quota = nb / S + (sh < nb % S ? 1u : 0u);
+    unsigned long long* const shard = tk.ctr + (size_t)(1 + sh) * PGX_TK_STRIDE;
+    bool last = false;
+    if (__hip_atomic_fetch_add(shard, 1ull, __ATOMIC_RELAXED, __HIP_MEMORY_SCOPE_AGENT) == quota - 1) {
+      __hip_atomic_store(shard, 0ull, __ATOMIC_RELAXED, __HIP_MEMORY_SCOPE_AGENT);
+      if (__hip_atomic_fetch_add(tk.ctr, 1ull, __ATOMIC_RELAXED, __HIP_MEMORY_SCOPE_AGENT) == (unsigned long long)S - 1) {
+        __hip_atomic_store(tk.ctr, 0ull, __ATOMIC_RELAXED, __HIP_MEMORY_SCOPE_AGENT);
+        last = true;
+        __builtin_amdgcn_fence(__ATOMIC_ACQUIRE, "agent");
+        asm volatile("s_waitcnt vmcnt(0)" ::: "memory");
+      }
+    }
+    sm[0] = last ? 1.0 : 0.0;
+  }
+  __syncthreads();
+  return sm[0] != 0.0;
+}
+template <int D, int K>
+__device__ __forceinline__ void tk_finish(const PgxTicket& tk, int nb, const double* p, unsigned bs, unsigned rs, int nrows,
+                                          int scaled, const PgxDotScale& sc, double* out, double* sm) {
+  unsigned tid = threadIdx.x;
+  asm volatile("" : "+v"(tid));
+  for (int r0 = 0; r0 < nrows; r0 += D) {
+    double x[D][K];
+#pragma unroll
+    for (int d = 0; d < D; ++d) {
+      const unsigned r = min(r0 + d, nrows - 1);
+#pragma unroll
+      for (int k = 0; k < K; ++k) {
+        const unsigned b = min(tid + k * PGX_BLOCK, (unsigned)nb - 1u);
+        x[d][k] = tk_load((const double*)((const char*)p + (b * bs + r * rs) * (unsigned)sizeof(double)));
+      }
+    }
+#pragma unroll
+    for (int d = 0; d < D; ++d) {
+      const int r = r0 + d;
+      if (r >= nrows) break;
+      double s = 0.0;
+#pragma unroll
+      for (int k = 0; k < K; ++k)
+        if ((int)(tid + k * PGX_BLOCK) < nb) s += x[d][k];
+      double t = block_sum(s, sm);
+      if (threadIdx.x == 0) {
+        if (scaled) t *= sc.s[r];
+        out[r] = t;
+        if (tk.hout) __hip_atomic_store(tk.hout + r, t, __ATOMIC_RELAXED, __HIP_MEMORY_SCOPE_SYSTEM);
+      }
+    }
+  }
+  if (!tk.hout || threadIdx.x >= WAVE) return;
+  for (int i = threadIdx.x; i < tk.n1; i += WAVE) __hip_atomic_store(tk.dst1 + i, tk.src1[i], __ATOMIC_RELAXED, __HIP_MEMORY_SCOPE_SYSTEM);
+  __threadfence_system();
+  if (threadIdx.x == 0) __hip_atomic_store(tk.seqp, tk.seq, __ATOMIC_RELEASE, __HIP_MEMORY_SCOPE_SYSTEM);
+}
+template <int D, int K>
+__device__ __forceinline__ void tk_finish(const PgxTicket& tk, int nb, const double* p, unsigned bs, unsigned rs, int nrows, double* out,
+                                          double* sm) {
+  tk_finish<D, K>(tk, nb, p, bs, rs, nrows, 0, PgxDotScale(), out, sm);
+}
+
+#define PGX_TK_D 4
+template <class VT>
+static constexpr bool tk_fits(int nv) {
+  return std::is_same<VT, double>::value || nv <= 10;
+}
+template <class VT>
+static constexpr bool tk_dot_fits(int nv) {
+  return tk_fits<VT>(nv) && nv <= 4;
+}
+template <int NV, class VT, class WT, bool TK>
 __global__ void __launch_bounds__(PGX_BLOCK) k_multidot(size_t ng, int tail, const VT* __restrict__ V, size_t ldv,
                                                         const WT* __restrict__ w,
-                                                        double* __restrict__ partials, int pstride, int poff) {
+                                                        double* __restrict__ partials, int pstride, int poff, double* out, int scaled,
+                                                        PgxDotScale sc, PgxTicket tk) {
   constexpr int G = GsLane<VT>::G;
   __shared__ double sm[PGX_BLOCK / WAVE];
   double acc[NV];
@@ -1282,8 +1377,16 @@
 #pragma unroll
   for (int v = 0; v < NV; ++v) {
     const double r = block_sum(acc[v], sm);
-    if (threadIdx.x == 0) partials[(size_t)blockIdx.x * pstride + poff + v] = r;
-  }
+    if (threadIdx.x == 0) {
+      double* const pv = partials + (size_t)blockIdx.x * pstride + poff + v;
+      if (TK)
+        tk_store(pv, r);
+      else
+        *pv = r;
+    }
+  }
+  if constexpr (TK)
+    if (tk_arrive(tk, sm)) tk_finish<PGX_TK_D, PGX_RED_BLOCKS / PGX_BLOCK>(tk, (int)gridDim.x, partials, (unsigned)pstride, 1u, pstride, scaled, sc, out, sm);
 }
 
 __global__ void __launch_bounds__(PGX_BLOCK) k_reduce_partials(int nblocks, int nv, const double* __restrict__ p,
@@ -1312,8 +1415,8 @@
 }
 
 template <class VT, class WT>
-static void multidot_t(hipStream_t st, size_t len, int nv, const VT* V, size_t ldv, const WT* w, double* partials, double* out,
-                       const PgxDotScale* scale, int wide) {
+static bool multidot_t(hipStream_t st, size_t len, int nv, const VT* V, size_t ldv, const WT* w, double* partials, double* out,
+                       const PgxDotScale* scale, int wide, PgxTicket* tk) {
   constexpr int G = GsLane<VT>::G;
   const size_t ng = len / G;
   const int tail = (int)(len - G * ng);
@@ -1321,12 +1424,25 @@
   dim3 grid((unsigned)nb), block(PGX_BLOCK);
   const int cap = wide > 16 ? 16 : wide < 1 ? 1 : wide;
   int done = 0;
+  static const PgxDotScale no_scale = {};
+  const PgxDotScale& sc = scale ? *scale : no_scale;
+  const int last_take = nv % cap ? nv % cap : cap;
+  const bool ticketed = tk && out && nv > 0 && tk_dot_fits<VT>(last_take);
   while (done < nv) {
     const int rem = nv - done;
     const VT* Vp = V + (size_t)done * ldv;
+    PgxTicket t;
+    if (ticketed && rem <= cap) t = *tk;
 #define PGX_MD(N)                                                                                                          \
   case N:                                                                                                                  \
-    hipLaunchKernelGGL((k_multidot<N, VT, WT>), grid, block, 0, st, ng, tail, Vp, ldv, w, partials, nv, done);             \
+    if constexpr (tk_dot_fits<VT>(N))                                                                                      \
+      if (t.ctr) {                                                                                                         \
+        hipLaunchKernelGGL((k_multidot<N, VT, WT, true>), grid, block, 0, st, ng, tail, Vp, ldv, w, partials, nv, done, out,  \
+                           scale ? 1 : 0, sc, t);                                                                          \
+        break;                                                                                                             \
+      }                                                                                                                    \
+    hipLaunchKernelGGL((k_multidot<N, VT, WT, false>), grid, block, 0, st, ng, tail, Vp, ldv, w, partials, nv, done, out, 0,  \
+                       no_scale, t);                                                                                       \
     break
     const int take = rem >= cap ? cap : rem;
     switch (take) {
@@ -1350,22 +1466,21 @@
 #undef PGX_MD
     done += take;
   }
-  if (!out) return;
+  if (!out || ticketed) return ticketed;
   if (scale)
     hipLaunchKernelGGL(k_reduce_partials_scaled, dim3(nv), block, 0, st, (int)nb, nv, partials, *scale, out);
   else
     hipLaunchKernelGGL(k_reduce_partials, dim3(nv), block, 0, st, (int)nb, nv, partials, out);
-}
-void pgxk_multidot(hipStream_t st, size_t len, int nv, const double* V, size_t ldv, const double* w, double* partials,
-                   double* out, const PgxDotScale* scale, int wide) {
-  multidot_t(st, len, nv, V, ldv, w, partials, out, scale, wide);
-}
-void pgxk_multidot_f32(hipStream_t st, size_t len, int nv, const float* V, size_t ldv, const double* w, const float* wf,
-                       double* partials, double* out, const PgxDotScale* scale, int wide) {
-  if (w)
-    multidot_t(st, len, nv, V, ldv, w, partials, out, scale, wide);
-  else
-    multidot_t(st, len, nv, V, ldv, wf, partials, out, scale, wide);
+  return false;
+}
+bool pgxk_multidot(hipStream_t st, size_t len, int nv, const double* V, size_t ldv, const double* w, double* partials,
+                   double* out, const PgxDotScale* scale, int wide, PgxTicket* tk) {
+  return multidot_t(st, len, nv, V, ldv, w, partials, out, scale, wide, tk);
+}
+bool pgxk_multidot_f32(hipStream_t st, size_t len, int nv, const float* V, size_t ldv, const double* w, const float* wf,
+                       double* partials, double* out, const PgxDotScale* scale, int wide, PgxTicket* tk) {
+  if (w) return multidot_t(st, len, nv, V, ldv, w, partials, out, scale, wide, tk);
+  return multidot_t(st, len, nv, V, ldv, wf, partials, out, scale, wide, tk);
 }
 
 __global__ void __launch_bounds__(PGX_BLOCK) k_reduce_publish(int nb, const double* __restrict__ p, int nrows, double* out, double* hout,
@@ -1392,8 +1507,9 @@
   hipLaunchKernelGGL(k_reduce_publish, dim3(1), dim3(PGX_BLOCK), 0, st, nb, partials, nrows, out, hout, n1, src1, dst1, seq, seqp);
 }
 
+template <bool TK>
 __global__ void __launch_bounds__(PGX_BLOCK) k_axpy_norms(size_t len2, double a, const double2* __restrict__ x, double2* __restrict__ y,
-                                                          double* __restrict__ partials) {
+                                                          double* __restrict__ partials, double* out, PgxTicket tk) {
   __shared__ double sm[PGX_BLOCK / WAVE];
   double accx = 0.0, accy = 0.0;
   for (size_t i = blockIdx.x * (size_t)blockDim.x + threadIdx.x; i < len2; i += (size_t)gridDim.x * blockDim.x) {
@@ -1407,13 +1523,25 @@
   const double rx = block_sum(accx, sm);
   const double ry = block_sum(accy, sm);
   if (threadIdx.x == 0) {
-    partials[blockIdx.x] = rx;
-    partials[gridDim.x + blockIdx.x] = ry;
-  }
-}
-int pgxk_axpy_norms(hipStream_t st, size_t len, const double* x, double* y, double* partials) {
+    if (TK) {
+      tk_store(partials + blockIdx.x, rx);
+      tk_store(partials + gridDim.x + blockIdx.x, ry);
+    } else {
+      partials[blockIdx.x] = rx;
+      partials[gridDim.x + blockIdx.x] = ry;
+    }
+  }
+  if constexpr (TK)
+    if (tk_arrive(tk, sm)) tk_finish<2, PGX_RED_BLOCKS / PGX_BLOCK>(tk, (int)gridDim.x, partials, 1u, gridDim.x, 2, out, sm);
+}
+int pgxk_axpy_norms(hipStream_t st, size_t len, const double* x, double* y, double* partials, double* out, PgxTicket* tk) {
   const int nb = pgxk_multidot_blocks(len);
-  hipLaunchKernelGGL(k_axpy_norms, dim3(nb), dim3(PGX_BLOCK), 0, st, len / 2, 1.0, (const double2*)x, (double2*)y, partials);
+  PgxTicket t;
+  if (tk && out) t = *tk;
+  if (t.ctr)
+    hipLaunchKernelGGL(k_axpy_norms<true>, dim3(nb), dim3(PGX_BLOCK), 0, st, len / 2, 1.0, (const double2*)x, (double2*)y, partials, out, t);
+  else
+    hipLaunchKernelGGL(k_axpy_norms<false>, dim3(nb), dim3(PGX_BLOCK), 0, st, len / 2, 1.0, (const double2*)x, (double2*)y, partials, out, t);
   return nb;
 }
 
@@ -1553,11 +1681,11 @@
   }
 }
 
-template <int NV, bool NORM, class VT, class WT>
+template <int NV, bool NORM, class VT, class WT, bool TK = false>
 __global__ void __launch_bounds__(PGX_BLOCK) k_multiaxpy_norm(size_t ng, int tail, const VT* __restrict__ V, size_t ldv,
                                                               const double* __restrict__ h, const WT* __restrict__ win,
                                                               typename std::conditional<NORM && std::is_same<VT, float>::value, float, double>::type* __restrict__ wout,
-                                                              double* __restrict__ partials) {
+                                                              double* __restrict__ partials, double* out, PgxTicket tk) {
   typedef typename std::conditional<NORM && std::is_same<VT, float>::value, float, double>::type OT;
   constexpr int G = GsLane<VT>::G;
   const WT* const wi = std::is_same<WT, OT>::value ? (const WT*)wout : win;
@@ -1598,46 +1726,69 @@
   }
   if (NORM) {
     const double r = block_sum(acc, sm);
-    if (threadIdx.x == 0) partials[blockIdx.x] = r;
+    if (threadIdx.x == 0) {
+      if (TK)
+        tk_store(partials + blockIdx.x, r);
+      else
+        partials[blockIdx.x] = r;
+    }
+    if constexpr (TK)
+      if (tk_arrive(tk, sm)) tk_finish<1, 16>(tk, (int)gridDim.x, partials, 1u, gridDim.x, 1, out, sm);
   }
 }
 int pgxk_stream_blocks(size_t len) { return (int)stream_grid(len / 2).x; }
 template <int N, class VT>
 static void launch_multiaxpy_norm(hipStream_t st, dim3 grid, size_t ng, int tail, const VT* Vp, size_t ldv, const double* h, bool last,
-                                  bool inf, double* w, float* wf, double* partials) {
+                                  bool inf, double* w, float* wf, double* partials, double* out, const PgxTicket& tk) {
   const dim3 block(PGX_BLOCK);
   if constexpr (std::is_same<VT, double>::value) {
-    if (last)
-      hipLaunchKernelGGL((k_multiaxpy_norm<N, true, double, double>), grid, block, 0, st, ng, tail, Vp, ldv, h, (const double*)nullptr, w, partials);
+    if (last && tk.ctr)
+      hipLaunchKernelGGL((k_multiaxpy_norm<N, true, double, double, true>), grid, block, 0, st, ng, tail, Vp, ldv, h, (const double*)nullptr, w, partials, out, tk);
+    else if (last)
+      hipLaunchKernelGGL((k_multiaxpy_norm<N, true, double, double>), grid, block, 0, st, ng, tail, Vp, ldv, h, (const double*)nullptr, w, partials, out, tk);
     else
-      hipLaunchKernelGGL((k_multiaxpy_norm<N, false, double, double>), grid, block, 0, st, ng, tail, Vp, ldv, h, (const double*)nullptr, w, partials);
+      hipLaunchKernelGGL((k_multiaxpy_norm<N, false, double, double>), grid, block, 0, st, ng, tail, Vp, ldv, h, (const double*)nullptr, w, partials, out, tk);
   } else {
+    if constexpr (tk_fits<VT>(N))
+      if (last && tk.ctr) {
+        if (inf)
+          hipLaunchKernelGGL((k_multiaxpy_norm<N, true, float, float, true>), grid, block, 0, st, ng, tail, Vp, ldv, h, (const float*)nullptr, wf, partials, out, tk);
+        else
+          hipLaunchKernelGGL((k_multiaxpy_norm<N, true, float, double, true>), grid, block, 0, st, ng, tail, Vp, ldv, h, (const double*)w, wf, partials, out, tk);
+        return;
+      }
     if (last && inf)
-      hipLaunchKernelGGL((k_multiaxpy_norm<N, true, float, float>), grid, block, 0, st, ng, tail, Vp, ldv, h, (const float*)nullptr, wf, partials);
+      hipLaunchKernelGGL((k_multiaxpy_norm<N, true, float, float>), grid, block, 0, st, ng, tail, Vp, ldv, h, (const float*)nullptr, wf, partials, out, tk);
     else if (last)
-      hipLaunchKernelGGL((k_multiaxpy_norm<N, true, float, double>), grid, block, 0, st, ng, tail, Vp, ldv, h, (const double*)w, wf, partials);
+      hipLaunchKernelGGL((k_multiaxpy_norm<N, true, float, double>), grid, block, 0, st, ng, tail, Vp, ldv, h, (const double*)w, wf, partials, out, tk);
     else if (inf)
-      hipLaunchKernelGGL((k_multiaxpy_norm<N, false, float, float>), grid, block, 0, st, ng, tail, Vp, ldv, h, (const float*)wf, w, partials);
+      hipLaunchKernelGGL((k_multiaxpy_norm<N, false, float, float>), grid, block, 0, st, ng, tail, Vp, ldv, h, (const float*)wf, w, partials, out, tk);
     else
-      hipLaunchKernelGGL((k_multiaxpy_norm<N, false, float, double>), grid, block, 0, st, ng, tail, Vp, ldv, h, (const double*)nullptr, w, partials);
+      hipLaunchKernelGGL((k_multiaxpy_norm<N, false, float, double>), grid, block, 0, st, ng, tail, Vp, ldv, h, (const double*)nullptr, w, partials, out, tk);
   }
 }
 template <class VT>
-static void multiaxpy_norm_t(hipStream_t st, size_t len, int nv, const VT* V, size_t ldv, const double* h, bool inf, double* w, float* wf,
-                             double* partials, double* out, int wide) {
+static bool multiaxpy_norm_t(hipStream_t st, size_t len, int nv, const VT* V, size_t ldv, const double* h, bool inf, double* w, float* wf,
+                             double* partials, double* out, int wide, PgxTicket* tk) {
   constexpr int G = GsLane<VT>::G;
   const size_t ng = len / G;
   const int tail = (int)(len - G * ng);
   dim3 grid = stream_grid(len / 2);
   const int cap = wide > 16 ? 16 : wide < 1 ? 1 : wide;
   int done = 0;
+  bool ticketed = false;
   while (done < nv) {
     const int step = std::min(cap, nv - done);
     const bool last = done + step == nv;
     const VT* Vp = V + (size_t)done * ldv;
+    PgxTicket t;
+    if (tk && out && last && tk_fits<VT>(step)) {
+      ticketed = true;
+      t = *tk;
+    }
 #define PGX_MAN(N)                                                                                                     \
   case N:                                                                                                              \
-    launch_multiaxpy_norm<N>(st, grid, ng, tail, Vp, ldv, h + done, last, inf && done == 0, w, wf, partials);          \
+    launch_multiaxpy_norm<N>(st, grid, ng, tail, Vp, ldv, h + done, last, inf && done == 0, w, wf, partials, out, t);  \
     break
     switch (step) {
       PGX_MAN(16);
@@ -1655,20 +1806,21 @@
       PGX_MAN(4);
       PGX_MAN(3);
       PGX_MAN(2);
-      default: launch_multiaxpy_norm<1>(st, grid, ng, tail, Vp, ldv, h + done, last, inf && done == 0, w, wf, partials); break;
+      default: launch_multiaxpy_norm<1>(st, grid, ng, tail, Vp, ldv, h + done, last, inf && done == 0, w, wf, partials, out, t); break;
     }
 #undef PGX_MAN
     done += step;
   }
-  if (out) hipLaunchKernelGGL(k_reduce_rows, dim3(1), dim3(PGX_BLOCK), 0, st, (int)grid.x, partials, out);
-}
-void pgxk_multiaxpy_norm(hipStream_t st, size_t len, int nv, const double* V, size_t ldv, const double* h, double* w,
-                         double* partials, double* out, int wide) {
-  multiaxpy_norm_t(st, len, nv, V, ldv, h, false, w, nullptr, partials, out, wide);
-}
-void pgxk_multiaxpy_norm_f32(hipStream_t st, size_t len, int nv, const float* V, size_t ldv, const double* h, int from_vnext, double* w,
-                             float* vnext, double* partials, double* out, int wide) {
-  multiaxpy_norm_t(st, len, nv, V, ldv, h, from_vnext != 0, w, vnext, partials, out, wide);
+  if (out && !tk) hipLaunchKernelGGL(k_reduce_rows, dim3(1), dim3(PGX_BLOCK), 0, st, (int)grid.x, partials, out);
+  return ticketed;
+}
+bool pgxk_multiaxpy_norm(hipStream_t st, size_t len, int nv, const double* V, size_t ldv, const double* h, double* w,
+                         double* partials, double* out, int wide, PgxTicket* tk) {
+  return multiaxpy_norm_t(st, len, nv, V, ldv, h, false, w, nullptr, partials, out, wide, tk);
+}
+bool pgxk_multiaxpy_norm_f32(hipStream_t st, size_t len, int nv, const float* V, size_t ldv, const double* h, int from_vnext, double* w,
+                             float* vnext, double* partials, double* out, int wide, PgxTicket* tk) {
+  return multiaxpy_norm_t(st, len, nv, V, ldv, h, from_vnext != 0, w, vnext, partials, out, wide, tk);
 }
 
 void pgxk_multiaxpy(hipStream_t st, size_t len, int nv, const double* V, size_t ldv, const double* h, double* w) {
@@ -1694,28 +1846,30 @@
   }
 }
 
+template <bool BYVAL>
 __global__ void __launch_bounds__(PGX_BLOCK) k_lincomb(size_t len2, int nv, const double2* __restrict__ Z,
-                                                       size_t ldz2, const double* __restrict__ y,
+                                                       size_t ldz2, const double* __restrict__ y, PgxDotScale yc,
                                                        double2* __restrict__ x, int accumulate) {
   for (size_t i = blockIdx.x * (size_t)blockDim.x + threadIdx.x; i < len2; i += (size_t)gridDim.x * blockDim.x) {
     double2 s = accumulate ? x[i] : make_double2(0.0, 0.0);
     for (int v = 0; v < nv; ++v) {
       const double2 a = Z[v * ldz2 + i];
-      const double yv = y[v];
+      const double yv = BYVAL ? yc.s[v] : y[v];
       s.x += yv * a.x;
       s.y += yv * a.y;
     }
     x[i] = s;
   }
 }
+template <bool BYVAL>
 __global__ void __launch_bounds__(PGX_BLOCK) k_lincomb_f2(size_t n, int nv, const float2* __restrict__ Zf, size_t ldz,
-                                                          const double* __restrict__ y, double* __restrict__ xu, double* __restrict__ xp,
-                                                          int accumulate) {
+                                                          const double* __restrict__ y, PgxDotScale yc, double* __restrict__ xu,
+                                                          double* __restrict__ xp, int accumulate) {
   for (size_t i = blockIdx.x * (size_t)blockDim.x + threadIdx.x; i < n; i += (size_t)gridDim.x * blockDim.x) {
     double su = accumulate ? xu[i] : 0.0, sp = accumulate ? xp[i] : 0.0;
     for (int v = 0; v < nv; ++v) {
       const float2 a = Zf[v * ldz + i];
-      const double yv = y[v];
+      const double yv = BYVAL ? yc.s[v] : y[v];
       su += yv * (double)a.x;
       sp += yv * (double)a.y;
     }
@@ -1723,16 +1877,32 @@
     xp[i] = sp;
   }
 }
+static PgxDotScale coef_arg(int nv, const double* yhost) {
+  PgxDotScale yc = {};
+  if (yhost) std::copy(yhost, yhost + nv, yc.s);
+  return yc;
+}
 void pgxk_lincomb_f2(hipStream_t st, size_t n, int nv, const float2* Zf, size_t ldz, const double* y, double* xu, double* xp,
-                     int accumulate) {
+                     int accumulate, const double* yhost) {
   const unsigned grid = (unsigned)std::min<size_t>((n + PGX_BLOCK - 1) / PGX_BLOCK, 256 * 32);
-  hipLaunchKernelGGL(k_lincomb_f2, dim3(grid), dim3(PGX_BLOCK), 0, st, n, nv, Zf, ldz, y, xu, xp, accumulate);
+  if (yhost && nv > PGX_DOT_SCALE_MAX) yhost = nullptr;
+  const PgxDotScale yc = coef_arg(nv, yhost);
+  if (yhost)
+    hipLaunchKernelGGL(k_lincomb_f2<true>, dim3(grid), dim3(PGX_BLOCK), 0, st, n, nv, Zf, ldz, y, yc, xu, xp, accumulate);
+  else
+    hipLaunchKernelGGL(k_lincomb_f2<false>, dim3(grid), dim3(PGX_BLOCK), 0, st, n, nv, Zf, ldz, y, yc, xu, xp, accumulate);
 }
 
 void pgxk_lincomb(hipStream_t st, size_t len, int nv, const double* Z, size_t ldz, const double* y, double* x,
-                  int accumulate) {
-  hipLaunchKernelGGL(k_lincomb, stream_grid(len / 2), dim3(PGX_BLOCK), 0, st, len / 2, nv, (const double2*)Z,
-                     ldz / 2, y, (double2*)x, accumulate);
+                  int accumulate, const double* yhost) {
+  if (yhost && nv > PGX_DOT_SCALE_MAX) yhost = nullptr;
+  const PgxDotScale yc = coef_arg(nv, yhost);
+  if (yhost)
+    hipLaunchKernelGGL(k_lincomb<true>, stream_grid(len / 2), dim3(PGX_BLOCK), 0, st, len / 2, nv, (const double2*)Z, ldz / 2, y, yc,
+                       (double2*)x, accumulate);
+  else
+    hipLaunchKernelGGL(k_lincomb<false>, stream_grid(len / 2), dim3(PGX_BLOCK), 0, st, len / 2, nv, (const double2*)Z, ldz / 2, y, yc,
+                       (double2*)x, accumulate);
 }
 
 __device__ __forceinline__ constexpr double pw(int dx, int dy) {
diff --git a/proximalgalerkin_amd/csrc/pgx_mg32.hip b/proximalgalerkin_amd/csrc/pgx_mg32.hip
--- a/proximalgalerkin_amd/csrc/pgx_mg32.hip
+++ b/proximalgalerkin_amd/csrc/pgx_mg32.hip
@@ -1012,7 +1012,8 @@
   __syncthreads();
   if (wave < CY && lane < CX) {
     const int q = (2 * wave + 1) * W + 2 * lane + 2;
-    F_LDS7(rimg, q, W, r0, r1, r2, r3, r4, r5, r6)
+    const float2 r0 = rimg[q], r1 = rimg[q + 1], r2 = rimg[q - 1], r3 = rimg[q + W], r4 = rimg[q - W], r5 = rimg[q + W + 1],
+                 r6 = rimg[q - W - 1];
     const float su = r0.x + 0.5f * (((r1.x + r2.x) + (r3.x + r4.x)) + (r5.x + r6.x));
     const float sp = r0.y + 0.5f * (((r1.y + r2.y) + (r3.y + r4.y)) + (r5.y + r6.y));
     const int C = (J0 + wave) * sxc + I0 + lane;
@@ -1086,7 +1087,8 @@
     const int I = I0 + lane, J = J0 + wave;
     if (I <= A.nxc && J <= A.nyc) {
       const int q = (2 * wave + 1) * W + 2 * lane + 2;
-      F_LDS7(rimg, q, W, r0, r1, r2, r3, r4, r5, r6)
+      const float2 r0 = rimg[q], r1 = rimg[q + 1], r2 = rimg[q - 1], r3 = rimg[q + W], r4 = rimg[q - W], r5 = rimg[q + W + 1],
+                   r6 = rimg[q - W - 1];
       float su = r0.x + 0.5f * (((r1.x + r2.x) + (r3.x + r4.x)) + (r5.x + r6.x));
       const float sp = r0.y + 0.5f * (((r1.y + r2.y) + (r3.y + r4.y)) + (r5.y + r6.y));
       const int C = J * sxc + I;
diff --git a/proximalgalerkin_amd/problem.py b/proximalgalerkin_amd/problem.py
--- a/proximalgalerkin_amd/problem.py
+++ b/proximalgalerkin_amd/problem.py
@@ -360,6 +360,12 @@
         _lib.check(self._lib, self._h, self._lib.pgx_observables(self._h, _lib.dptr(out)), "pgx_observables")
         return out
 
+    def reduce_selfcheck(self, nv, length, basis_f32=False, reps=1, seed=0):
+        bad = C.c_int64(-1)
+        _lib.check(self._lib, self._h, self._lib.pgx_reduce_selfcheck(self._h, int(nv), int(length), int(bool(basis_f32)), int(reps),
+                                                                      int(seed), C.byref(bad)), "pgx_reduce_selfcheck")
+        return bad.value
+
     def owned_edge_range(self):
         off, cnt = C.c_int64(0), C.c_int64(0)
         _lib.check(self._lib, self._h, self._lib.pgx_owned_edge_range(self._h, C.byref(off), C.byref(cnt)),
```

Result: faster. 160.0 Newton iterations/s (median of 6 runs) (+1.2%).
